# KimmiShi/TorchDistPackage

Measured on AMD Instinct MI355X. Metric: tokens_per_second, higher is better.
Workload: dtype bf16; 1 GPU; model=gpt2_1.3b, global_batch=16, seq_len=1024, parallelism=dp1_pp1_tp1

## Files before the change

torchdistpackage_amd/ops/__init__.py:

```python

from __future__ import annotations

import contextlib
import math
import os
from typing import Optional

import torch

_EXT = None
_EXT_ERR: Optional[str] = None


def _load_extension():
    global _EXT, _EXT_ERR
    if _EXT is not None or _EXT_ERR is not None:
        return _EXT
    import glob
    import importlib.util
    here = os.path.dirname(os.path.abspath(__file__))
    cands = glob.glob(os.path.join(here, "_tdpa_hip*.so"))
    if not cands:
        _EXT_ERR = (f"in-tree HIP extension not found under {here}; "
                    "run `python -m torchdistpackage_amd.ops.build` "
                    "(or __graft_entry__.build())")
        return None
    spec = importlib.util.spec_from_file_location("_tdpa_hip", cands[0])
    mod = importlib.util.module_from_spec(spec)
    try:
        spec.loader.exec_module(mod)
    except Exception as e:
        _EXT_ERR = f"failed to load {cands[0]}: {e}"
        return None
    _EXT = mod
    return _EXT


def ext(required_for: str = "op"):
    m = _load_extension()
    if m is None:
        raise RuntimeError(
            f"HIP extension required for {required_for} on GPU but "
            f"unavailable: {_EXT_ERR}")
    return m


def extension_available() -> bool:
    return _load_extension() is not None



class _RMSNormFn(torch.autograd.Function):
    @staticmethod
    def forward(ctx, x, weight, eps):
        if x.is_cuda:
            y, rstd = ext("rms_norm").rmsnorm_fwd(x.contiguous(), weight, eps)
        else:
            xf = x.float()
            rstd = torch.rsqrt(xf.pow(2).mean(-1, keepdim=True) + eps)
            y = (xf * rstd * weight.float()).to(x.dtype)
            rstd = rstd.squeeze(-1)
        ctx.save_for_backward(x, weight, rstd)
        ctx.eps = eps
        return y

    @staticmethod
    def backward(ctx, dy):
        x, weight, rstd = ctx.saved_tensors
        if x.is_cuda:
            dx, dw = ext("rms_norm").rmsnorm_bwd(
                dy.contiguous(), x.contiguous(), weight, rstd)
        else:
            xf, dyf, wf = x.float(), dy.float(), weight.float()
            r = rstd.unsqueeze(-1)
            xhat = xf * r
            wdy = dyf * wf
            m = (wdy * xhat).mean(-1, keepdim=True)
            dx = (r * (wdy - xhat * m)).to(x.dtype)
            dw = (dyf * xhat).reshape(-1, x.shape[-1]).sum(0).to(weight.dtype)
        return dx, dw, None


def rms_norm(x: torch.Tensor, weight: torch.Tensor, eps: float = 1e-6):
    return _RMSNormFn.apply(x, weight, eps)


class RMSNorm(torch.nn.Module):
    def __init__(self, dim: int, eps: float = 1e-6, device=None, dtype=None):
        super().__init__()
        self.eps = eps
        self.weight = torch.nn.Parameter(
            torch.ones(dim, device=device, dtype=dtype))

    def forward(self, x):
        return rms_norm(x, self.weight, self.eps)



class _LayerNormFn(torch.autograd.Function):
    @staticmethod
    def forward(ctx, x, weight, bias, eps):
        if x.is_cuda:
            y, mean, rstd = ext("layer_norm").layernorm_fwd(
                x.contiguous(), weight, bias, eps)
        else:
            xf = x.float()
            mean = xf.mean(-1, keepdim=True)
            var = xf.var(-1, unbiased=False, keepdim=True)
            off = ~(mean * mean <= var)
            if off.any():
                mean2 = mean + (xf - mean).mean(-1, keepdim=True)
                var2 = (xf - mean2).pow(2).mean(-1, keepdim=True)
                mean = torch.where(off, mean2, mean)
                var = torch.where(off, var2, var)
            rstd = torch.rsqrt(var + eps)
            y = ((xf - mean) * rstd * weight.float() + bias.float()).to(x.dtype)
            mean, rstd = mean.squeeze(-1), rstd.squeeze(-1)
        ctx.save_for_backward(x, weight, mean, rstd)
        return y

    @staticmethod
    def backward(ctx, dy):
        x, weight, mean, rstd = ctx.saved_tensors
        if x.is_cuda:
            dx, dw, db = ext("layer_norm").layernorm_bwd(
                dy.contiguous(), x.contiguous(), weight, mean, rstd)
        else:
            xf, dyf, wf = x.float(), dy.float(), weight.float()
            mu, r = mean.unsqueeze(-1), rstd.unsqueeze(-1)
            xhat = (xf - mu) * r
            wdy = dyf * wf
            m1 = wdy.mean(-1, keepdim=True)
            m2 = (wdy * xhat).mean(-1, keepdim=True)
            dx = (r * (wdy - m1 - xhat * m2)).to(x.dtype)
            dw = (dyf * xhat).reshape(-1, x.shape[-1]).sum(0).to(weight.dtype)
            db = dyf.reshape(-1, x.shape[-1]).sum(0).to(weight.dtype)
        return dx, dw, db, None


def layer_norm(x, weight, bias, eps: float = 1e-5):
    return _LayerNormFn.apply(x, weight, bias, eps)


class LayerNorm(torch.nn.Module):
    def __init__(self, dim: int, eps: float = 1e-5, device=None, dtype=None):
        super().__init__()
        self.eps = eps
        kw = {"device": device, "dtype": dtype}
        self.weight = torch.nn.Parameter(torch.ones(dim, **kw))
        self.bias = torch.nn.Parameter(torch.zeros(dim, **kw))

    def forward(self, x):
        return layer_norm(x, self.weight, self.bias, self.eps)



_GELU_C = math.sqrt(2.0 / math.pi)


def _gelu_tanh(u):
    return 0.5 * u * (1.0 + torch.tanh(_GELU_C * (u + 0.044715 * u.pow(3))))


class _BiasGeluFn(torch.autograd.Function):
    @staticmethod
    def forward(ctx, x, bias):
        ctx.has_bias = bias is not None
        if x.is_cuda:
            y = ext("bias_gelu").bias_gelu_fwd(
                x.contiguous(),
                bias if bias is not None else torch.empty(
                    0, dtype=x.dtype, device=x.device))
            ctx.save_for_backward(x, bias if bias is not None else
                                  torch.empty(0, dtype=x.dtype, device=x.device))
        else:
            u = x.float() + (bias.float() if bias is not None else 0.0)
            y = _gelu_tanh(u).to(x.dtype)
            ctx.save_for_backward(x, bias if bias is not None else
                                  torch.empty(0, dtype=x.dtype))
        return y

    @staticmethod
    def backward(ctx, dy):
        x, bias = ctx.saved_tensors
        if x.is_cuda:
            dx = ext("bias_gelu").bias_gelu_bwd(dy.contiguous(),
                                                x.contiguous(), bias)
        else:
            u = x.float() + (bias.float() if ctx.has_bias else 0.0)
            t = torch.tanh(_GELU_C * (u + 0.044715 * u.pow(3)))
            du = 0.5 * (1 + t) + 0.5 * u * (1 - t * t) * _GELU_C * \
                (1 + 3 * 0.044715 * u.pow(2))
            dx = (dy.float() * du).to(x.dtype)
        dbias = None
        if ctx.has_bias:
            dbias = dx.reshape(-1, x.shape[-1]).sum(0).to(x.dtype)
        return dx, dbias


def bias_gelu(x, bias=None):
    return _BiasGeluFn.apply(x, bias)



class _FlashAttentionFn(torch.autograd.Function):

    @staticmethod
    def forward(ctx, q, k, v, causal, scale):
        if scale is None:
            scale = 1.0 / math.sqrt(q.shape[-1])
        rep = q.shape[1] // k.shape[1]
        if q.is_cuda:
            o = torch.empty(q.shape, dtype=q.dtype, device=q.device)
            o, lse = ext("flash_attention").attn_fwd(
                q, k, v, o, bool(causal), float(scale))
        else:
            kf = k.float() if rep == 1 else \
                k.float().repeat_interleave(rep, 1)
            vf = v.float() if rep == 1 else \
                v.float().repeat_interleave(rep, 1)
            qf = q.float()
            s = torch.matmul(qf, kf.transpose(-1, -2)) * scale
            if causal:
                S = q.shape[-2]
                mask = torch.ones(S, k.shape[-2], dtype=torch.bool,
                                  device=q.device).tril_()
                s = s.masked_fill(~mask, float("-inf"))
            lse = torch.logsumexp(s, dim=-1)
            p = torch.softmax(s, dim=-1)
            o = torch.matmul(p, vf).to(q.dtype)
        ctx.save_for_backward(q, k, v, o, lse)
        ctx.causal = causal
        ctx.scale = scale
        return o

    @staticmethod
    def backward(ctx, do):
        q, k, v, o, lse = ctx.saved_tensors
        H, Hkv = q.shape[1], k.shape[1]
        rep = H // Hkv
        if q.is_cuda:
            dq = torch.empty(q.shape, dtype=q.dtype, device=q.device)
            dk = torch.empty(q.shape, dtype=k.dtype, device=k.device)
            dv = torch.empty(q.shape, dtype=v.dtype, device=v.device)
            dq, dk, dv = ext("flash_attention").attn_bwd(
                do.contiguous(), q, k, v, o, lse, dq, dk, dv,
                ctx.causal, ctx.scale)
            if rep > 1:
                B, _, S, D = q.shape
                dk = dk.view(B, Hkv, rep, S, D).sum(2).to(k.dtype)
                dv = dv.view(B, Hkv, rep, S, D).sum(2).to(v.dtype)
        else:
            qf = q.float()
            kf = k.float() if rep == 1 else \
                k.float().repeat_interleave(rep, 1)
            vf = v.float() if rep == 1 else \
                v.float().repeat_interleave(rep, 1)
            dof = do.float()
            s = torch.matmul(qf, kf.transpose(-1, -2)) * ctx.scale
            if ctx.causal:
                S = q.shape[-2]
                mask = torch.ones(S, k.shape[-2], dtype=torch.bool,
                                  device=q.device).tril_()
                s = s.masked_fill(~mask, float("-inf"))
            p = torch.softmax(s, dim=-1)
            dv = torch.matmul(p.transpose(-1, -2), dof)
            dp = torch.matmul(dof, vf.transpose(-1, -2))
            d = (dp * p).sum(-1, keepdim=True)
            ds = p * (dp - d) * ctx.scale
            dq = torch.matmul(ds, kf)
            dk = torch.matmul(ds.transpose(-1, -2), qf)
            if rep > 1:
                B, _, S, D = q.shape
                dk = dk.view(B, Hkv, rep, S, D).sum(2)
                dv = dv.view(B, Hkv, rep, S, D).sum(2)
            dq, dk, dv = dq.to(q.dtype), dk.to(k.dtype), dv.to(v.dtype)
        return dq, dk, dv, None, None


_ATTN_KNOBS = ("dq_recompute", "no_tr16", "pstore", "force_v1",
               "max_ds_bytes")


def attention_knobs() -> dict:
    return dict(zip(_ATTN_KNOBS, ext("attention_knobs").attn_knobs()))


@contextlib.contextmanager
def attention_route(**knobs):
    unknown = set(knobs) - set(_ATTN_KNOBS)
    if unknown:
        raise TypeError(f"unknown attention knob(s) {sorted(unknown)}; "
                        f"known: {_ATTN_KNOBS}")
    e = ext("attention_knobs")
    cur = attention_knobs()
    cur.update(knobs)
    prev = e.attn_set_knobs(*(cur[n] for n in _ATTN_KNOBS))
    try:
        yield
    finally:
        e.attn_set_knobs(*prev)


_warned_hd = set()


def flash_attention(q, k, v, causal: bool = True, scale: float = None):
    D = q.shape[-1]
    if q.is_cuda and D not in (64, 128):
        if D not in _warned_hd:
            _warned_hd.add(D)
            print(f"[tdpa.ops] flash_attention: head_dim {D} has no HIP "
                  f"kernel (64/128 do); using composite SDPA for it")
        rep = q.shape[1] // k.shape[1]
        kk = k if rep == 1 else k.repeat_interleave(rep, 1)
        vv = v if rep == 1 else v.repeat_interleave(rep, 1)
        if scale is None:
            scale = 1.0 / math.sqrt(D)
        return torch.nn.functional.scaled_dot_product_attention(
            q, kk, vv, is_causal=causal, scale=scale)
    return _FlashAttentionFn.apply(q, k, v, causal, scale)



def fused_adamw_(param: torch.Tensor, grad: torch.Tensor,
                 exp_avg: torch.Tensor, exp_avg_sq: torch.Tensor,
                 step: int, lr: float, beta1: float, beta2: float,
                 eps: float, weight_decay: float):
    if param.is_cuda:
        ext("fused_adamw").adamw_step(param, grad, exp_avg, exp_avg_sq,
                                      step, lr, beta1, beta2, eps,
                                      weight_decay)
        return
    bc1 = 1 - beta1 ** step
    bc2 = 1 - beta2 ** step
    param.mul_(1 - lr * weight_decay)
    exp_avg.mul_(beta1).add_(grad, alpha=1 - beta1)
    exp_avg_sq.mul_(beta2).addcmul_(grad, grad, value=1 - beta2)
    denom = (exp_avg_sq / bc2).sqrt_().add_(eps)
    param.addcdiv_(exp_avg, denom, value=-lr / bc1)


def ema_update_(ema: torch.Tensor, param: torch.Tensor, decay: float):
    if ema.is_cuda:
        ext("ema_update").ema_update(ema, param.contiguous(), decay)
        return
    ema.lerp_(param.to(ema.dtype), 1.0 - decay)


def l2norm_sq(t: torch.Tensor) -> torch.Tensor:
    if t.is_cuda:
        return ext("l2norm").l2norm_sq(t)
    return t.float().pow(2).sum()


def scale_(t: torch.Tensor, scale: float):
    if t.is_cuda:
        ext("scale").scale_inplace(t, scale)
        return
    t.mul_(scale)


class _FusedQKVAttentionFn(torch.autograd.Function):

    @staticmethod
    def forward(ctx, qkv, n_head, causal, scale):
        S, B, three_d = qkv.shape
        d_local = three_d // 3
        hd = d_local // n_head
        if scale is None:
            scale = 1.0 / math.sqrt(hd)

        def view4(t, off):
            return t.narrow(-1, off, d_local) \
                .view(S, B, n_head, hd).permute(1, 2, 0, 3)

        q, k, v = view4(qkv, 0), view4(qkv, d_local), view4(qkv, 2 * d_local)
        if qkv.is_cuda:
            o_buf = torch.empty(S, B, d_local, dtype=qkv.dtype,
                                device=qkv.device)
            o4 = o_buf.view(S, B, n_head, hd).permute(1, 2, 0, 3)
            _, lse = ext("flash_attention").attn_fwd(
                q, k, v, o4, bool(causal), float(scale))
        else:
            qf = q.contiguous().float()
            kf = k.contiguous().float()
            vf = v.contiguous().float()
            sc = torch.matmul(qf, kf.transpose(-1, -2)) * scale
            if causal:
                mask = torch.ones(S, S, dtype=torch.bool).tril_()
                sc = sc.masked_fill(~mask, float("-inf"))
            lse = torch.logsumexp(sc, dim=-1)
            o4 = torch.matmul(torch.softmax(sc, -1), vf).to(qkv.dtype)
            o_buf = o4.permute(2, 0, 1, 3).reshape(S, B, d_local)
        ctx.save_for_backward(qkv, o_buf, lse)
        ctx.meta = (n_head, causal, scale)
        return o_buf

    @staticmethod
    def backward(ctx, do):
        qkv, o_buf, lse = ctx.saved_tensors
        n_head, causal, scale = ctx.meta
        S, B, three_d = qkv.shape
        d_local = three_d // 3
        hd = d_local // n_head

        def view4(t, off, width):
            return t.narrow(-1, off, width) \
                .view(S, B, n_head, hd).permute(1, 2, 0, 3)

        q = view4(qkv, 0, d_local)
        k = view4(qkv, d_local, d_local)
        v = view4(qkv, 2 * d_local, d_local)
        o4 = o_buf.view(S, B, n_head, hd).permute(1, 2, 0, 3)
        do = do.contiguous()
        do4 = do.view(S, B, n_head, hd).permute(1, 2, 0, 3)
        if qkv.is_cuda:
            dqkv = torch.empty_like(qkv)
            dq = view4(dqkv, 0, d_local)
            dk = view4(dqkv, d_local, d_local)
            dv = view4(dqkv, 2 * d_local, d_local)
            ext("flash_attention").attn_bwd(
                do4, q, k, v, o4, lse, dq, dk, dv, causal, scale)
        else:
            qc, kc, vc = q.contiguous(), k.contiguous(), v.contiguous()
            with torch.enable_grad():
                qf = qc.float().requires_grad_(True)
                kf = kc.float().requires_grad_(True)
                vf = vc.float().requires_grad_(True)
                s = torch.matmul(qf, kf.transpose(-1, -2)) * scale
                if causal:
                    Sq = q.shape[-2]
                    mask = torch.ones(Sq, Sq, dtype=torch.bool).tril_()
                    s = s.masked_fill(~mask, float("-inf"))
                ref = torch.matmul(torch.softmax(s, -1), vf)
                ref.backward(do4.float())
            dqkv = torch.cat([
                g.to(qkv.dtype).permute(2, 0, 1, 3).reshape(S, B, d_local)
                for g in (qf.grad, kf.grad, vf.grad)], dim=-1)
        return dqkv, None, None, None



def fused_qkv_attention(qkv, n_head: int, causal: bool = True,
                        scale: float = None):
    return _FusedQKVAttentionFn.apply(qkv, n_head, causal, scale)


class _GqaAttentionFn(torch.autograd.Function):

    @staticmethod
    def forward(ctx, q, k, v, causal, scale):
        B, H, S, D = q.shape
        o_buf = torch.empty(S, B, H * D, dtype=q.dtype, device=q.device)
        o4 = o_buf.view(S, B, H, D).permute(1, 2, 0, 3)
        _, lse = ext("flash_attention").attn_fwd(
            q, k, v, o4, bool(causal), float(scale))
        ctx.save_for_backward(q, k, v, o_buf, lse)
        ctx.meta = (causal, scale)
        return o_buf

    @staticmethod
    def backward(ctx, do):
        q, k, v, o_buf, lse = ctx.saved_tensors
        causal, scale = ctx.meta
        B, H, S, D = q.shape
        Hkv = k.shape[1]
        rep = H // Hkv
        o4 = o_buf.view(S, B, H, D).permute(1, 2, 0, 3)
        do = do.contiguous()
        do4 = do.view(S, B, H, D).permute(1, 2, 0, 3)
        dq_buf = torch.empty(S, B, H * D, dtype=q.dtype, device=q.device)
        dq = dq_buf.view(S, B, H, D).permute(1, 2, 0, 3)
        dk = torch.empty(B, H, S, D, dtype=k.dtype, device=k.device)
        dv = torch.empty(B, H, S, D, dtype=v.dtype, device=v.device)
        ext("flash_attention").attn_bwd(do4, q, k, v, o4, lse, dq, dk, dv,
                                        causal, scale)
        if rep > 1:
            dk = dk.view(B, Hkv, rep, S, D).sum(2)
            dv = dv.view(B, Hkv, rep, S, D).sum(2)
        return dq, dk, dv, None, None


def gqa_attention(q, k, v, causal: bool = True, scale: float = None):
    if scale is None:
        scale = 1.0 / math.sqrt(q.shape[-1])
    if q.is_cuda and q.dtype == torch.bfloat16 and q.shape[-1] in (64, 128):
        return _GqaAttentionFn.apply(q, k, v, causal, scale)
    o = flash_attention(q, k, v, causal=causal, scale=scale)
    B, H, S, D = q.shape
    return o.permute(2, 0, 1, 3).reshape(S, B, H * D)



_DECODE_MAX_ROWS = 16


def resolve_decode_attn_impl(attn_impl: Optional[str] = None) -> str:
    if attn_impl is None:
        attn_impl = "hip" if os.environ.get("TDPA_DECODE_ATTN", "0") == "1" \
            else "sdpa"
    if attn_impl not in ("sdpa", "hip"):
        raise ValueError(f"attn_impl must be 'sdpa' or 'hip', got "
                         f"{attn_impl!r}")
    return attn_impl


def _decode_attention_ref(q, k_cache, v_cache, pos0, scale):
    B, Hq, Sq, D = q.shape
    Hkv, Smax = k_cache.shape[1], k_cache.shape[2]
    G = Hq // Hkv
    if torch.is_tensor(pos0):
        pos = pos0.reshape(-1).to(device=q.device, dtype=torch.long)
        pos = pos.expand(B) if pos.numel() == 1 else pos
    else:
        if pos0 < 0 or pos0 + Sq > Smax:
            raise ValueError(f"decode_attention: pos0={pos0} with Sq={Sq} "
                             f"outside the cache (Smax={Smax})")
        pos = torch.full((B,), int(pos0), dtype=torch.long, device=q.device)
    pos = pos.clamp(0, Smax - Sq)
    L = int(pos.max()) + Sq
    kf = k_cache[:, :, :L].float()
    vf = v_cache[:, :, :L].float()
    j = torch.arange(L, device=q.device)
    live = j[None, :] < (pos[:, None] + Sq)
    vf = torch.where(live[:, None, :, None], vf, torch.zeros_like(vf))
    qf = q.float().reshape(B, Hkv, G * Sq, D)
    s = torch.matmul(qf, kf.transpose(-1, -2)) * scale
    row = torch.arange(G * Sq, device=q.device) % Sq
    vis = j[None, None, :] <= (pos[:, None, None] + row[None, :, None])
    s = s.masked_fill(~vis[:, None], float("-inf"))
    o = torch.matmul(torch.softmax(s, dim=-1), vf)
    return o.reshape(B, Hq, Sq, D).to(q.dtype)


def decode_attention(q: torch.Tensor, k_cache: torch.Tensor,
                     v_cache: torch.Tensor, pos0, scale: float = None,
                     split_kv: Optional[int] = None) -> torch.Tensor:
    B, Hq, Sq, D = q.shape
    Hkv = k_cache.shape[1]
    if Hq % Hkv != 0:
        raise ValueError(f"decode_attention: Hq={Hq} not a multiple of "
                         f"Hkv={Hkv}")
    if scale is None:
        scale = 1.0 / math.sqrt(D)
    if not q.is_cuda:
        o = _decode_attention_ref(q, k_cache, v_cache, pos0, scale)
        o_buf = o.permute(2, 0, 1, 3).contiguous()
        return o_buf.permute(1, 2, 0, 3)
    if q.dtype != torch.bfloat16:
        raise TypeError("decode_attention: the GPU kernel is bf16-only, got "
                        f"{q.dtype}")
    if D not in (64, 128):
        raise ValueError("decode_attention: the GPU kernel covers head dim "
                         f"64 and 128, got {D}")
    G = Hq // Hkv
    if G > _DECODE_MAX_ROWS:
        raise ValueError(f"decode_attention: Hq/Hkv={G} exceeds the "
                         f"kernel's {_DECODE_MAX_ROWS} rows per kv head")
    e = ext("decode_attention")
    o_buf = torch.empty(Sq, B, Hq * D, dtype=q.dtype, device=q.device)
    o4 = o_buf.view(Sq, B, Hq, D).permute(1, 2, 0, 3)
    skv = int(split_kv or 0)
    if torch.is_tensor(pos0):
        if G * Sq > _DECODE_MAX_ROWS:
            raise ValueError(
                f"decode_attention: (Hq/Hkv)*Sq={G * Sq} exceeds "
                f"{_DECODE_MAX_ROWS} rows per kv head; with a tensor pos0 "
                "the call cannot be split on the host — pass an int pos0 "
                "or fewer query rows")
        e.decode_attention(q, k_cache, v_cache, o4, pos0, 0, float(scale),
                           skv)
        return o4
    pos0 = int(pos0)
    rows = _DECODE_MAX_ROWS // G
    for r0 in range(0, Sq, rows):
        r1 = min(r0 + rows, Sq)
        e.decode_attention(q[:, :, r0:r1], k_cache, v_cache,
                           o4[:, :, r0:r1], None, pos0 + r0, float(scale),
                           skv)
    return o4


class _CrossEntropyFn(torch.autograd.Function):

    @staticmethod
    def forward(ctx, logits2d, targets):
        loss_vec, lse = ext("cross_entropy").ce_fwd(logits2d, targets)
        ctx.save_for_backward(logits2d, targets, lse)
        return loss_vec.mean()

    @staticmethod
    def backward(ctx, g):
        logits2d, targets, lse = ctx.saved_tensors
        dlogits = ext("cross_entropy").ce_bwd(
            logits2d, targets, lse, g.reshape(1).float().contiguous())
        return dlogits, None


def cross_entropy_loss(logits: torch.Tensor, targets: torch.Tensor):
    l2 = logits.reshape(-1, logits.size(-1))
    t = targets.reshape(-1)
    if l2.is_cuda and l2.dtype == torch.bfloat16:
        return _CrossEntropyFn.apply(l2.contiguous(), t)
    import torch.nn.functional as F
    return F.cross_entropy(l2.float(), t)



class _BatchedBiasGeluFn(torch.autograd.Function):

    @staticmethod
    def forward(ctx, x, bias):
        ctx.save_for_backward(x, bias)
        if x.is_cuda and x.dtype == torch.bfloat16:
            return ext("bgelu_b").bgelu_b_fwd(x.contiguous(),
                                              bias.contiguous())
        u = x.float() + bias.float().unsqueeze(1)
        return _gelu_tanh(u).to(x.dtype)

    @staticmethod
    def backward(ctx, dy):
        x, bias = ctx.saved_tensors
        if x.is_cuda and x.dtype == torch.bfloat16:
            dx = ext("bgelu_b").bgelu_b_bwd(dy.contiguous(), x.contiguous(),
                                            bias.contiguous())
        else:
            u = x.float() + bias.float().unsqueeze(1)
            t = torch.tanh(_GELU_C * (u + 0.044715 * u.pow(3)))
            du = 0.5 * (1 + t) + 0.5 * u * (1 - t * t) * _GELU_C * \
                (1 + 3 * 0.044715 * u.pow(2))
            dx = (dy.float() * du).to(x.dtype)
        dbias = dx.float().sum(1).to(bias.dtype)
        return dx, dbias


def batched_bias_gelu(x, bias):
    return _BatchedBiasGeluFn.apply(x, bias)


def _rope_rows(cos, sin, pos0, S):
    if cos.shape != sin.shape:
        raise ValueError("rope: sin must have the shape of cos")
    if pos0 < 0 or pos0 + S > cos.shape[0]:
        raise ValueError(f"rope: pos0={pos0} with S={S} outside the cos/sin "
                         f"table ({cos.shape[0]} rows)")
    return cos[pos0:pos0 + S].float(), sin[pos0:pos0 + S].float()


class _RopeFn(torch.autograd.Function):

    @staticmethod
    def forward(ctx, x, cos, sin, pos0):
        ctx.save_for_backward(cos, sin)
        ctx.pos0 = pos0
        if x.is_cuda and x.dtype == torch.bfloat16:
            return ext("rope").rope_apply(x, cos, sin, pos0, True)
        c, s = _rope_rows(cos, sin, pos0, x.shape[-2])
        hd = x.shape[-1]
        xf = x.float()
        x1, x2 = xf[..., :hd // 2], xf[..., hd // 2:]
        return torch.cat([x1 * c - x2 * s, x2 * c + x1 * s],
                         dim=-1).to(x.dtype)

    @staticmethod
    def backward(ctx, dy):
        cos, sin = ctx.saved_tensors
        if dy.is_cuda and dy.dtype == torch.bfloat16:
            if dy.stride(-1) != 1:
                dy = dy.contiguous()
            return (ext("rope").rope_apply(dy, cos, sin,
                                           ctx.pos0, False),
                    None, None, None)
        c, s = _rope_rows(cos, sin, ctx.pos0, dy.shape[-2])
        hd = dy.shape[-1]
        df = dy.float()
        d1, d2 = df[..., :hd // 2], df[..., hd // 2:]
        return (torch.cat([d1 * c + d2 * s, d2 * c - d1 * s],
                          dim=-1).to(dy.dtype),
                None, None, None)


def rope_rotate_half(x: torch.Tensor, cos: torch.Tensor, sin: torch.Tensor,
                     pos0=0) -> torch.Tensor:
    if torch.is_tensor(pos0):
        assert not torch.is_grad_enabled(), \
            "tensor pos0 is the no-grad decode path"
        if x.is_cuda and x.dtype == torch.bfloat16:
            return ext("rope").rope_apply_pos(x, cos, sin, pos0, True)
        return _RopeFn.apply(x, cos, sin, int(pos0.item()))
    return _RopeFn.apply(x, cos, sin, pos0)


class _SwiGluFn(torch.autograd.Function):
    @staticmethod
    def forward(ctx, a, b):
        ctx.save_for_backward(a, b)
        if a.is_cuda and a.dtype == torch.bfloat16:
            return ext("swiglu").swiglu_fwd(a.contiguous(), b.contiguous())
        af = a.float()
        return (af * torch.sigmoid(af) * b.float()).to(a.dtype)

    @staticmethod
    def backward(ctx, dy):
        a, b = ctx.saved_tensors
        if a.is_cuda and a.dtype == torch.bfloat16:
            da, db = ext("swiglu").swiglu_bwd(dy.contiguous(),
                                              a.contiguous(), b.contiguous())
            return da, db
        af, bf, dyf = a.float(), b.float(), dy.float()
        sig = torch.sigmoid(af)
        silu = af * sig
        da = dyf * bf * (sig + silu * (1 - sig))
        db = dyf * silu
        return da.to(a.dtype), db.to(b.dtype)


def swiglu(a: torch.Tensor, b: torch.Tensor) -> torch.Tensor:
    return _SwiGluFn.apply(a, b)



from .grouped import (GROUPED_GEMM_BM, grouped_gemm_eligible,
                      grouped_linear)
```

torchdistpackage_amd/ops/csrc/attention.hip:

```cpp

#include <torch/extension.h>
#include <ATen/hip/HIPContext.h>
#include "common.h"
#include "attn_knobs.h"
#include <cstdlib>
#include <string>
#include <tuple>

namespace {

typedef __attribute__((ext_vector_type(8))) __bf16 bf16x8_v;
typedef __attribute__((ext_vector_type(4))) float f32x4;

constexpr int WQ = 16;
constexpr int KT = 32;
constexpr int NW_FWD = 16;
constexpr int NW_DQ = 8;
constexpr int NW_DKDV = 8;

struct Strides {
  long b, h, s;
};

DEVINL bf16x8_v pack8(const unsigned short* p) {
  return *(const bf16x8_v*)p;
}

template <int D>
DEVINL int swzD(int row, int col) {
  return row * D + (col ^ ((row & (D / 8 - 1)) << 3));
}

DEVINL int swz32(int row, int col) {
  return row * KT + (col ^ (((row >> 2) & 3) << 3));
}


template <int D, bool CAUSAL, int NW>
__launch_bounds__(NW * 64)
__global__ void attn_fwd_kernel(const unsigned short* __restrict__ q,
                                const unsigned short* __restrict__ k,
                                const unsigned short* __restrict__ v,
                                unsigned short* __restrict__ o,
                                float* __restrict__ lse,
                                Strides qs, Strides ks, Strides vs, Strides os,
                                int B, int H, int S, float scale,
                                int q_per_kv) {
  constexpr int KC = D / 32;
  constexpr int DC = D / 16;
  __shared__ __attribute__((aligned(16))) unsigned short k_lds[KT * D];
  __shared__ __attribute__((aligned(16))) unsigned short vt_lds[D * KT];
  __shared__ __attribute__((aligned(16))) unsigned short p_lds[NW * 16 * KT];

  constexpr int QT = NW * WQ;
  const int bh = blockIdx.y;
  const int bb = bh / H, hh = bh % H;
  const int qbase = blockIdx.x * QT;
  if (qbase >= S) return;
  const int tid = threadIdx.x;
  const int wid = tid / WAVE;
  const int lane = tid % WAVE;
  const int l15 = lane & 15;
  const int lg = lane >> 4;

  const int hkv = hh / q_per_kv;
  const unsigned short* qp = q + bb * qs.b + hh * qs.h;
  const unsigned short* kp = k + bb * ks.b + hkv * ks.h;
  const unsigned short* vp = v + bb * vs.b + hkv * vs.h;

  const int qrow0 = qbase + wid * WQ;
  bf16x8_v a_q[KC];
  {
    int r = qrow0 + l15;
    long rr = (r < S ? r : S - 1) * qs.s;
#pragma unroll
    for (int c = 0; c < KC; ++c)
      a_q[c] = pack8(qp + rr + c * 32 + lg * 8);
  }

  float m_run[4], l_run[4];
#pragma unroll
  for (int i = 0; i < 4; ++i) { m_run[i] = -1e30f; l_run[i] = 0.f; }
  f32x4 acc_o[DC];
#pragma unroll
  for (int d = 0; d < DC; ++d) acc_o[d] = (f32x4)(0.f);

  const int kv_end = CAUSAL ? min(S, qbase + QT) : S;

  const int st_idx = tid * 8;
  const int st_key = st_idx / D;
  const int st_col = st_idx % D;
  const bool st_own = st_idx < KT * D;
  bf16x8_v k_reg, v_reg;

  auto stage_load = [&](int kt0) {
    if (!st_own) return;
    int gkey = kt0 + st_key;
    if (gkey < S) {
      k_reg = pack8(kp + (long)gkey * ks.s + st_col);
      v_reg = pack8(vp + (long)gkey * vs.s + st_col);
    } else {
      k_reg = (bf16x8_v)(__bf16)0.f;
      v_reg = (bf16x8_v)(__bf16)0.f;
    }
  };

  stage_load(0);

  for (int kt0 = 0; kt0 < kv_end; kt0 += KT) {
    __syncthreads();
    if (st_own) {
      *(bf16x8_v*)&k_lds[swzD<D>(st_key, st_col)] = k_reg;
      const unsigned short* vsrc = (const unsigned short*)&v_reg;
#pragma unroll
      for (int j = 0; j < 8; ++j)
        vt_lds[swz32(st_col + j, st_key)] = vsrc[j];
    }
    __syncthreads();
    if (kt0 + KT < kv_end) stage_load(kt0 + KT);

    f32x4 s_acc[KT / 16];
#pragma unroll
    for (int kg = 0; kg < KT / 16; ++kg) {
      s_acc[kg] = (f32x4)(0.f);
#pragma unroll
      for (int c = 0; c < KC; ++c) {
        bf16x8_v b_k = pack8(&k_lds[swzD<D>(kg * 16 + l15, c * 32 + lg * 8)]);
        s_acc[kg] = __builtin_amdgcn_mfma_f32_16x16x32_bf16(
            a_q[c], b_k, s_acc[kg], 0, 0, 0);
      }
    }

    float p_val[KT / 16][4];
    float alpha[4];
    {
      float tile_max[4];
#pragma unroll
      for (int rr = 0; rr < 4; ++rr) tile_max[rr] = -1e30f;
#pragma unroll
      for (int kg = 0; kg < KT / 16; ++kg) {
#pragma unroll
        for (int rr = 0; rr < 4; ++rr) {
          int qrow = qrow0 + lg * 4 + rr;
          int key = kt0 + kg * 16 + l15;
          float sv = s_acc[kg][rr] * scale;
          bool valid = key < S && (!CAUSAL || key <= qrow);
          sv = valid ? sv : -1e30f;
          s_acc[kg][rr] = sv;
          tile_max[rr] = fmaxf(tile_max[rr], sv);
        }
      }
#pragma unroll
      for (int rr = 0; rr < 4; ++rr) {
        tile_max[rr] = group16_max(tile_max[rr]);
        float m_new = fmaxf(m_run[rr], tile_max[rr]);
        alpha[rr] = __expf(m_run[rr] - m_new);
        m_run[rr] = m_new;
        float psum = 0.f;
#pragma unroll
        for (int kg = 0; kg < KT / 16; ++kg) {
          float pv = __expf(s_acc[kg][rr] - m_new);
          p_val[kg][rr] = pv;
          psum += pv;
        }
        psum = group16_sum(psum);
        l_run[rr] = l_run[rr] * alpha[rr] + psum;
      }
    }

#pragma unroll
    for (int d = 0; d < DC; ++d)
#pragma unroll
      for (int rr = 0; rr < 4; ++rr) acc_o[d][rr] *= alpha[rr];

    unsigned short* pw = &p_lds[wid * 16 * KT];
#pragma unroll
    for (int kg = 0; kg < KT / 16; ++kg)
#pragma unroll
      for (int rr = 0; rr < 4; ++rr)
        pw[swz32(lg * 4 + rr, kg * 16 + l15)] = f2bf(p_val[kg][rr]);

    bf16x8_v a_p = pack8(&pw[swz32(l15, lg * 8)]);
#pragma unroll
    for (int d = 0; d < DC; ++d) {
      bf16x8_v b_v = pack8(&vt_lds[swz32(d * 16 + l15, lg * 8)]);
      acc_o[d] = __builtin_amdgcn_mfma_f32_16x16x32_bf16(
          a_p, b_v, acc_o[d], 0, 0, 0);
    }
  }

  unsigned short* op = o + bb * os.b + hh * os.h;
  float* lsep = lse + ((long)bh) * S;
#pragma unroll
  for (int rr = 0; rr < 4; ++rr) {
    int qrow = qrow0 + lg * 4 + rr;
    if (qrow >= S) continue;
    float inv_l = l_run[rr] > 0.f ? 1.f / l_run[rr] : 0.f;
#pragma unroll
    for (int d = 0; d < DC; ++d)
      op[(long)qrow * os.s + d * 16 + l15] = f2bf(acc_o[d][rr] * inv_l);
    if (l15 == 0)
      lsep[qrow] = m_run[rr] + __logf(l_run[rr] > 0.f ? l_run[rr] : 1.f);
  }
}


__global__ void attn_delta_kernel(const unsigned short* __restrict__ o,
                                  const unsigned short* __restrict__ dout,
                                  float* __restrict__ delta,
                                  Strides os, Strides ds,
                                  int B, int H, int S, int D) {
  const long rows = (long)B * H * S;
  const int wpb = blockDim.x / WAVE;
  const int lane = threadIdx.x % WAVE;
  const long stride = (long)gridDim.x * wpb;
  for (long row = (long)blockIdx.x * wpb + threadIdx.x / WAVE; row < rows;
       row += stride) {
    int s = row % S;
    int h = (row / S) % H;
    int b = row / ((long)S * H);
    const unsigned short* orow = o + b * os.b + h * os.h + (long)s * os.s;
    const unsigned short* drow = dout + b * ds.b + h * ds.h + (long)s * ds.s;
    float acc = 0.f;
    for (int i = lane * 8; i < D; i += WAVE * 8) {
      bf16x8_v ov = pack8(orow + i);
      bf16x8_v dv = pack8(drow + i);
      const unsigned short* op = (const unsigned short*)&ov;
      const unsigned short* dp = (const unsigned short*)&dv;
#pragma unroll
      for (int j = 0; j < 8; ++j) acc += bf2f(op[j]) * bf2f(dp[j]);
    }
    acc = wave_sum(acc);
    if (lane == 0) delta[row] = acc;
  }
}

template <int D, bool CAUSAL, int NW>
__launch_bounds__(NW * 64)
__global__ void attn_bwd_dq_kernel(const unsigned short* __restrict__ q,
                                   const unsigned short* __restrict__ k,
                                   const unsigned short* __restrict__ v,
                                   const unsigned short* __restrict__ dout,
                                   const float* __restrict__ lse,
                                   const float* __restrict__ delta,
                                   unsigned short* __restrict__ dq,
                                   Strides qs, Strides ks, Strides vs,
                                   Strides dos, Strides dqs,
                                   int B, int H, int S, float scale,
                                   int q_per_kv) {
  constexpr int KC = D / 32;
  constexpr int DC = D / 16;
  __shared__ __attribute__((aligned(16))) unsigned short k_lds[KT * D];
  __shared__ __attribute__((aligned(16))) unsigned short kt_lds[D * KT];
  __shared__ __attribute__((aligned(16))) unsigned short v_lds[KT * D];
  __shared__ __attribute__((aligned(16))) unsigned short ds_lds[NW * 16 * KT];

  constexpr int QT = NW * WQ;
  const int bh = blockIdx.y;
  const int bb = bh / H, hh = bh % H;
  const int qbase = blockIdx.x * QT;
  if (qbase >= S) return;
  const int tid = threadIdx.x;
  const int wid = tid / WAVE;
  const int lane = tid % WAVE;
  const int l15 = lane & 15;
  const int lg = lane >> 4;

  const int hkv = hh / q_per_kv;
  const unsigned short* qp = q + bb * qs.b + hh * qs.h;
  const unsigned short* kp = k + bb * ks.b + hkv * ks.h;
  const unsigned short* vp = v + bb * vs.b + hkv * vs.h;
  const unsigned short* dop = dout + bb * dos.b + hh * dos.h;
  const float* lsep = lse + (long)bh * S;
  const float* delp = delta + (long)bh * S;

  const int qrow0 = qbase + wid * WQ;
  bf16x8_v a_q[KC], a_do[KC];
  float my_lse[4], my_delta[4];
  {
    int r = qrow0 + l15;
    int rc = r < S ? r : S - 1;
#pragma unroll
    for (int c = 0; c < KC; ++c) {
      a_q[c] = pack8(qp + (long)rc * qs.s + c * 32 + lg * 8);
      a_do[c] = pack8(dop + (long)rc * dos.s + c * 32 + lg * 8);
    }
#pragma unroll
    for (int rr4 = 0; rr4 < 4; ++rr4) {
      int row = qrow0 + lg * 4 + rr4;
      my_lse[rr4] = row < S ? lsep[row] : 0.f;
      my_delta[rr4] = row < S ? delp[row] : 0.f;
    }
  }

  f32x4 acc_dq[DC];
#pragma unroll
  for (int d = 0; d < DC; ++d) acc_dq[d] = (f32x4)(0.f);

  const int kv_end = CAUSAL ? min(S, qbase + QT) : S;

  const int st_idx = tid * 8;
  const int st_key = st_idx / D;
  const int st_col = st_idx % D;
  const bool st_own = st_idx < KT * D;
  bf16x8_v k_reg, v_reg;

  auto stage_load = [&](int kt0) {
    if (!st_own) return;
    int gkey = kt0 + st_key;
    if (gkey < S) {
      k_reg = pack8(kp + (long)gkey * ks.s + st_col);
      v_reg = pack8(vp + (long)gkey * vs.s + st_col);
    } else {
      k_reg = (bf16x8_v)(__bf16)0.f;
      v_reg = (bf16x8_v)(__bf16)0.f;
    }
  };

  stage_load(0);

  for (int kt0 = 0; kt0 < kv_end; kt0 += KT) {
    __syncthreads();
    if (st_own) {
      *(bf16x8_v*)&k_lds[swzD<D>(st_key, st_col)] = k_reg;
      *(bf16x8_v*)&v_lds[swzD<D>(st_key, st_col)] = v_reg;
      const unsigned short* ksrc = (const unsigned short*)&k_reg;
#pragma unroll
      for (int j = 0; j < 8; ++j)
        kt_lds[swz32(st_col + j, st_key)] = ksrc[j];
    }
    __syncthreads();
    if (kt0 + KT < kv_end) stage_load(kt0 + KT);

    f32x4 s_acc[KT / 16], dp_acc[KT / 16];
#pragma unroll
    for (int kg = 0; kg < KT / 16; ++kg) {
      s_acc[kg] = (f32x4)(0.f);
      dp_acc[kg] = (f32x4)(0.f);
#pragma unroll
      for (int c = 0; c < KC; ++c) {
        bf16x8_v b_k = pack8(&k_lds[swzD<D>(kg * 16 + l15, c * 32 + lg * 8)]);
        s_acc[kg] = __builtin_amdgcn_mfma_f32_16x16x32_bf16(
            a_q[c], b_k, s_acc[kg], 0, 0, 0);
        bf16x8_v b_v = pack8(&v_lds[swzD<D>(kg * 16 + l15, c * 32 + lg * 8)]);
        dp_acc[kg] = __builtin_amdgcn_mfma_f32_16x16x32_bf16(
            a_do[c], b_v, dp_acc[kg], 0, 0, 0);
      }
    }

    unsigned short* dsw = &ds_lds[wid * 16 * KT];
#pragma unroll
    for (int kg = 0; kg < KT / 16; ++kg) {
#pragma unroll
      for (int rr = 0; rr < 4; ++rr) {
        int qrow = qrow0 + lg * 4 + rr;
        int key = kt0 + kg * 16 + l15;
        bool valid = key < S && qrow < S && (!CAUSAL || key <= qrow);
        float p = valid ?
            __expf(s_acc[kg][rr] * scale - my_lse[rr]) : 0.f;
        float ds = p * (dp_acc[kg][rr] - my_delta[rr]) * scale;
        dsw[swz32(lg * 4 + rr, kg * 16 + l15)] = f2bf(ds);
      }
    }

    bf16x8_v a_ds = pack8(&dsw[swz32(l15, lg * 8)]);
#pragma unroll
    for (int d = 0; d < DC; ++d) {
      bf16x8_v b_kt = pack8(&kt_lds[swz32(d * 16 + l15, lg * 8)]);
      acc_dq[d] = __builtin_amdgcn_mfma_f32_16x16x32_bf16(
          a_ds, b_kt, acc_dq[d], 0, 0, 0);
    }
  }

  unsigned short* dqp = dq + bb * dqs.b + hh * dqs.h;
#pragma unroll
  for (int rr = 0; rr < 4; ++rr) {
    int qrow = qrow0 + lg * 4 + rr;
    if (qrow >= S) continue;
#pragma unroll
    for (int d = 0; d < DC; ++d)
      dqp[(long)qrow * dqs.s + d * 16 + l15] = f2bf(acc_dq[d][rr]);
  }
}

template <int D, bool CAUSAL, int NW>
__launch_bounds__(NW * 64)
__global__ void attn_bwd_dkdv_kernel(const unsigned short* __restrict__ q,
                                     const unsigned short* __restrict__ k,
                                     const unsigned short* __restrict__ v,
                                     const unsigned short* __restrict__ dout,
                                     const float* __restrict__ lse,
                                     const float* __restrict__ delta,
                                     unsigned short* __restrict__ dk,
                                     unsigned short* __restrict__ dv,
                                     Strides qs, Strides ks, Strides vs,
                                     Strides dos, Strides dks, Strides dvs,
                                     int B, int H, int S, float scale,
                                     int q_per_kv) {
  constexpr int KC = D / 32;
  constexpr int DC = D / 16;
  __shared__ __attribute__((aligned(16))) unsigned short q_lds[KT * D];
  __shared__ __attribute__((aligned(16))) unsigned short qt_lds[D * KT];
  __shared__ __attribute__((aligned(16))) unsigned short do_lds[KT * D];
  __shared__ __attribute__((aligned(16))) unsigned short dot_lds[D * KT];
  __shared__ __attribute__((aligned(16))) unsigned short st_lds[NW * 16 * KT];
  __shared__ __attribute__((aligned(16))) float lse_lds[KT];
  __shared__ __attribute__((aligned(16))) float del_lds[KT];

  constexpr int QT = NW * WQ;
  const int bh = blockIdx.y;
  const int bb = bh / H, hh = bh % H;
  const int kbase = blockIdx.x * QT;
  if (kbase >= S) return;
  const int tid = threadIdx.x;
  const int wid = tid / WAVE;
  const int lane = tid % WAVE;
  const int l15 = lane & 15;
  const int lg = lane >> 4;

  const int hkv = hh / q_per_kv;
  const unsigned short* qp = q + bb * qs.b + hh * qs.h;
  const unsigned short* kp = k + bb * ks.b + hkv * ks.h;
  const unsigned short* vp = v + bb * vs.b + hkv * vs.h;
  const unsigned short* dop = dout + bb * dos.b + hh * dos.h;
  const float* lsep = lse + (long)bh * S;
  const float* delp = delta + (long)bh * S;

  const int key0 = kbase + wid * WQ;
  bf16x8_v a_k[KC], a_v[KC];
  {
    int r = key0 + l15;
    long rc = (long)(r < S ? r : S - 1);
#pragma unroll
    for (int c = 0; c < KC; ++c) {
      a_k[c] = pack8(kp + rc * ks.s + c * 32 + lg * 8);
      a_v[c] = pack8(vp + rc * vs.s + c * 32 + lg * 8);
    }
  }

  f32x4 acc_dk[DC], acc_dv[DC];
#pragma unroll
  for (int d = 0; d < DC; ++d) {
    acc_dk[d] = (f32x4)(0.f);
    acc_dv[d] = (f32x4)(0.f);
  }

  const int qt_start = CAUSAL ? kbase : 0;

  const int st_idx = tid * 8;
  const int st_row = st_idx / D;
  const int st_col = st_idx % D;
  const bool st_own = st_idx < KT * D;
  bf16x8_v q_reg, do_reg;
  float lse_reg = 0.f, del_reg = 0.f;

  auto stage_load = [&](int qt0) {
    if (st_own) {
      int grow = qt0 + st_row;
      if (grow < S) {
        q_reg = pack8(qp + (long)grow * qs.s + st_col);
        do_reg = pack8(dop + (long)grow * dos.s + st_col);
      } else {
        q_reg = (bf16x8_v)(__bf16)0.f;
        do_reg = (bf16x8_v)(__bf16)0.f;
      }
    }
    if (tid < KT) {
      int grow = qt0 + tid;
      lse_reg = grow < S ? lsep[grow] : 0.f;
      del_reg = grow < S ? delp[grow] : 0.f;
    }
  };

  stage_load(qt_start);

  for (int qt0 = qt_start; qt0 < S; qt0 += KT) {
    __syncthreads();
    if (st_own) {
      *(bf16x8_v*)&q_lds[swzD<D>(st_row, st_col)] = q_reg;
      *(bf16x8_v*)&do_lds[swzD<D>(st_row, st_col)] = do_reg;
      const unsigned short* qsrc = (const unsigned short*)&q_reg;
      const unsigned short* dsrc = (const unsigned short*)&do_reg;
#pragma unroll
      for (int j = 0; j < 8; ++j) {
        qt_lds[swz32(st_col + j, st_row)] = qsrc[j];
        dot_lds[swz32(st_col + j, st_row)] = dsrc[j];
      }
    }
    if (tid < KT) {
      lse_lds[tid] = lse_reg;
      del_lds[tid] = del_reg;
    }
    __syncthreads();
    if (qt0 + KT < S) stage_load(qt0 + KT);

    f32x4 st_acc[KT / 16], dpt_acc[KT / 16];
#pragma unroll
    for (int qg = 0; qg < KT / 16; ++qg) {
      st_acc[qg] = (f32x4)(0.f);
      dpt_acc[qg] = (f32x4)(0.f);
#pragma unroll
      for (int c = 0; c < KC; ++c) {
        bf16x8_v b_q = pack8(&q_lds[swzD<D>(qg * 16 + l15, c * 32 + lg * 8)]);
        st_acc[qg] = __builtin_amdgcn_mfma_f32_16x16x32_bf16(
            a_k[c], b_q, st_acc[qg], 0, 0, 0);
        bf16x8_v b_do = pack8(&do_lds[swzD<D>(qg * 16 + l15, c * 32 + lg * 8)]);
        dpt_acc[qg] = __builtin_amdgcn_mfma_f32_16x16x32_bf16(
            a_v[c], b_do, dpt_acc[qg], 0, 0, 0);
      }
    }

    unsigned short* stw = &st_lds[wid * 16 * KT];
#pragma unroll
    for (int qg = 0; qg < KT / 16; ++qg) {
#pragma unroll
      for (int rr = 0; rr < 4; ++rr) {
        int key = key0 + lg * 4 + rr;
        int qrow = qt0 + qg * 16 + l15;
        bool valid = key < S && qrow < S && (!CAUSAL || key <= qrow);
        float p = valid ?
            __expf(st_acc[qg][rr] * scale - lse_lds[qg * 16 + l15]) : 0.f;
        st_acc[qg][rr] = p;
        stw[swz32(lg * 4 + rr, qg * 16 + l15)] =
            f2bf(p < kAttnPFlush ? 0.f : p);
      }
    }

    bf16x8_v a_pt = pack8(&stw[swz32(l15, lg * 8)]);
#pragma unroll
    for (int d = 0; d < DC; ++d) {
      bf16x8_v b_dot = pack8(&dot_lds[swz32(d * 16 + l15, lg * 8)]);
      acc_dv[d] = __builtin_amdgcn_mfma_f32_16x16x32_bf16(
          a_pt, b_dot, acc_dv[d], 0, 0, 0);
    }

#pragma unroll
    for (int qg = 0; qg < KT / 16; ++qg) {
#pragma unroll
      for (int rr = 0; rr < 4; ++rr) {
        float ds = st_acc[qg][rr] *
            (dpt_acc[qg][rr] - del_lds[qg * 16 + l15]) * scale;
        stw[swz32(lg * 4 + rr, qg * 16 + l15)] = f2bf(ds);
      }
    }

    bf16x8_v a_dst = pack8(&stw[swz32(l15, lg * 8)]);
#pragma unroll
    for (int d = 0; d < DC; ++d) {
      bf16x8_v b_qt = pack8(&qt_lds[swz32(d * 16 + l15, lg * 8)]);
      acc_dk[d] = __builtin_amdgcn_mfma_f32_16x16x32_bf16(
          a_dst, b_qt, acc_dk[d], 0, 0, 0);
    }
  }

  unsigned short* dkp = dk + bb * dks.b + hh * dks.h;
  unsigned short* dvp = dv + bb * dvs.b + hh * dvs.h;
#pragma unroll
  for (int rr = 0; rr < 4; ++rr) {
    int key = key0 + lg * 4 + rr;
    if (key >= S) continue;
#pragma unroll
    for (int d = 0; d < DC; ++d) {
      dkp[(long)key * dks.s + d * 16 + l15] = f2bf(acc_dk[d][rr]);
      dvp[(long)key * dvs.s + d * 16 + l15] = f2bf(acc_dv[d][rr]);
    }
  }
}

Strides get_strides(const torch::Tensor& t) {
  TORCH_CHECK(t.dim() == 4 && t.stride(3) == 1,
              "attention tensors must be 4D (B,H,S,D) with contiguous D");
  return Strides{t.stride(0), t.stride(1), t.stride(2)};
}

void check_operand(const char* fn, const char* name, const torch::Tensor& t,
                   const torch::Tensor& q, int64_t B, int64_t Hh, int64_t S,
                   int64_t D) {
  TORCH_CHECK(t.is_cuda() && t.device() == q.device(), fn, ": ", name,
              " must be on q's device ", q.device(), ", got ", t.device());
  TORCH_CHECK(t.scalar_type() == torch::kBFloat16, fn, ": ", name,
              " must be bf16, got ", t.scalar_type());
  TORCH_CHECK(t.dim() == 4 && t.size(0) == B && t.size(1) == Hh &&
                  t.size(2) == S && t.size(3) == D,
              fn, ": ", name, " must be (", B, ", ", Hh, ", ", S, ", ", D,
              "), got ", t.sizes());
  TORCH_CHECK(t.stride(3) == 1, fn, ": ", name,
              " must have a contiguous last dim, got stride ", t.stride(3));
  for (int d = 0; d < 3; ++d)
    TORCH_CHECK(t.size(d) == 1 || t.stride(d) % 8 == 0, fn, ": ", name,
                " stride ", t.stride(d), " of dim ", d, " is not a multiple "
                "of 8 elements: the kernels use 16-byte vector accesses");
  TORCH_CHECK(reinterpret_cast<uintptr_t>(t.data_ptr()) % 16 == 0, fn, ": ",
              name, " is not 16-byte aligned: the kernels use 16-byte vector "
              "accesses");
}

std::tuple<int64_t, int64_t, int64_t, int64_t, int64_t> check_qkv(
    const char* fn, const torch::Tensor& q, const torch::Tensor& k,
    const torch::Tensor& v) {
  TORCH_CHECK(q.is_cuda() && q.scalar_type() == torch::kBFloat16, fn,
              ": bf16 CUDA tensors required");
  TORCH_CHECK(q.dim() == 4, fn, ": q must be (B, H, S, D), got ", q.sizes());
  const int64_t B = q.size(0), H = q.size(1), S = q.size(2), D = q.size(3);
  TORCH_CHECK(D == 64 || D == 128, fn, ": head_dim must be 64 or 128, got ",
              D);
  TORCH_CHECK(B >= 1 && H >= 1 && S >= 1, fn,
              ": empty problem (S = 0?), q is ", q.sizes());
  TORCH_CHECK(k.dim() == 4 && v.dim() == 4, fn,
              ": k and v must be (B, Hkv, S, D), got ", k.sizes(), " and ",
              v.sizes());
  const int64_t Hkv = k.size(1);
  TORCH_CHECK(Hkv >= 1 && H % Hkv == 0, fn,
              ": n_head must be a multiple of n_kv_head, got ", H, " and ",
              Hkv);
  TORCH_CHECK(k.size(2) == S, fn,
              ": cross-attention S_kv != S_q not supported yet (k has ",
              k.size(2), " keys, q ", S, " rows)");
  check_operand(fn, "q", q, q, B, H, S, D);
  check_operand(fn, "k", k, q, B, Hkv, S, D);
  check_operand(fn, "v", v, q, B, Hkv, S, D);
  return {B, H, Hkv, S, D};
}

}

AttnKnobs& attn_knobs_ref() {
  static AttnKnobs k{
      std::getenv("TDPA_DQ_RECOMPUTE") != nullptr,
      std::getenv("TDPA_NO_TR16") != nullptr,
      std::getenv("TDPA_PSTORE") != nullptr,
      std::getenv("TDPA_ATTN_V1") != nullptr,
      (int64_t)4 << 30};
  return k;
}

using KnobTuple = std::tuple<bool, bool, bool, bool, int64_t>;

KnobTuple attn_knobs() {
  const AttnKnobs& k = attn_knobs_ref();
  return {k.dq_recompute, k.no_tr16, k.pstore, k.force_v1, k.max_ds_bytes};
}

KnobTuple attn_set_knobs(bool dq_recompute, bool no_tr16, bool pstore,
                         bool force_v1, int64_t max_ds_bytes) {
  KnobTuple prev = attn_knobs();
  attn_knobs_ref() =
      AttnKnobs{dq_recompute, no_tr16, pstore, force_v1, max_ds_bytes};
  return prev;
}

std::string attn_bwd_route(int64_t B, int64_t H, int64_t S, int64_t D) {
  const AttnBwdRoute r = attn_bwd_select(attn_knobs_ref(), B, H, S, D);
  if (r.v1) return "v1";
  if (r.recompute) return "v2_recompute";
  std::string name = "v2_workspace";
  if (r.pstore) name += "+pstore";
  if (r.no_tr16) name += "+no_tr16";
  return name;
}

void attn_fwd_v2(torch::Tensor q, torch::Tensor k, torch::Tensor v,
                 torch::Tensor o, torch::Tensor lse, bool causal,
                 double scale);
void attn_bwd_dq_v2(torch::Tensor dout, torch::Tensor q, torch::Tensor k,
                    torch::Tensor v, torch::Tensor lse, torch::Tensor delta,
                    torch::Tensor dq, bool causal, double scale);
void attn_bwd_v2_all(torch::Tensor dout, torch::Tensor q, torch::Tensor k,
                     torch::Tensor v, torch::Tensor lse, torch::Tensor delta,
                     torch::Tensor dq, torch::Tensor dk, torch::Tensor dv,
                     bool causal, double scale, const AttnBwdRoute& route);
void attn_bwd_dkdv_v2(torch::Tensor dout, torch::Tensor q, torch::Tensor k,
                      torch::Tensor v, torch::Tensor lse, torch::Tensor delta,
                      torch::Tensor dk, torch::Tensor dv, bool causal,
                      double scale);

std::vector<torch::Tensor> attn_fwd(torch::Tensor q, torch::Tensor k,
                                    torch::Tensor v, torch::Tensor o,
                                    bool causal, double scale) {
  auto [B_, H_, Hkv_, S_, D_] = check_qkv("attn_fwd", q, k, v);
  check_operand("attn_fwd", "o", o, q, B_, H_, S_, D_);
  const int B = B_, H = H_, S = S_, D = D_, Hkv = Hkv_;
  const int q_per_kv = H / Hkv;
  auto lse = torch::empty({B, H, S}, q.options().dtype(torch::kFloat));
  const bool force_v1 = attn_knobs_ref().force_v1;
  if (D == 128 && !force_v1) {
    attn_fwd_v2(q, k, v, o, lse, causal, scale);
    return {o, lse};
  }
  auto stream = at::cuda::getCurrentHIPStream();
  constexpr int QT = NW_FWD * WQ;
  dim3 grid((S + QT - 1) / QT, B * H), block(NW_FWD * 64);
  Strides qs = get_strides(q), ks = get_strides(k), vs = get_strides(v),
          os = get_strides(o);
  const unsigned short* qp = (const unsigned short*)q.data_ptr();
  const unsigned short* kp = (const unsigned short*)k.data_ptr();
  const unsigned short* vp = (const unsigned short*)v.data_ptr();
  unsigned short* op = (unsigned short*)o.data_ptr();
  float* lp = lse.data_ptr<float>();
#define LAUNCH(DD, CC)                                                        \
  hipLaunchKernelGGL((attn_fwd_kernel<DD, CC, NW_FWD>), grid, block, 0,       \
                     stream, qp, kp, vp, op, lp, qs, ks, vs, os, B, H, S,     \
                     (float)scale, q_per_kv)
  if (D == 128) { if (causal) LAUNCH(128, true); else LAUNCH(128, false); }
  else          { if (causal) LAUNCH(64, true);  else LAUNCH(64, false);  }
#undef LAUNCH
  HIP_CHECK_LAST();
  return {o, lse};
}

std::vector<torch::Tensor> attn_bwd(torch::Tensor dout, torch::Tensor q,
                                    torch::Tensor k, torch::Tensor v,
                                    torch::Tensor o, torch::Tensor lse,
                                    torch::Tensor dq, torch::Tensor dk,
                                    torch::Tensor dv,
                                    bool causal, double scale) {
  auto [B_, H_, Hkv_, S_, D_] = check_qkv("attn_bwd", q, k, v);
  const int B = B_, H = H_, S = S_, D = D_, Hkv = Hkv_;
  const int q_per_kv = H / Hkv;
  check_operand("attn_bwd", "dout", dout, q, B, H, S, D);
  check_operand("attn_bwd", "o", o, q, B, H, S, D);
  check_operand("attn_bwd", "dq", dq, q, B, H, S, D);
  TORCH_CHECK(dk.dim() == 4 && dv.dim() == 4 && dk.size(1) == H &&
                  dv.size(1) == H,
              "attn_bwd: dk/dv must be expanded to H q-heads for GQA, got ",
              dk.sizes(), " and ", dv.sizes(), " for H = ", H);
  check_operand("attn_bwd", "dk", dk, q, B, H, S, D);
  check_operand("attn_bwd", "dv", dv, q, B, H, S, D);
  TORCH_CHECK(lse.is_cuda() && lse.device() == q.device() &&
                  lse.scalar_type() == torch::kFloat && lse.dim() == 3 &&
                  lse.size(0) == B && lse.size(1) == H && lse.size(2) == S &&
                  lse.is_contiguous(),
              "attn_bwd: lse must be a contiguous fp32 (", B, ", ", H, ", ",
              S, ") tensor on q's device, got ", lse.scalar_type(), " ",
              lse.sizes(), " strides ", lse.strides(), " on ", lse.device());
  auto delta = torch::empty({B, H, S}, q.options().dtype(torch::kFloat));
  auto stream = at::cuda::getCurrentHIPStream();
  Strides qs = get_strides(q), ks = get_strides(k), vs = get_strides(v),
          os = get_strides(o), dos = get_strides(dout),
          dqs = get_strides(dq), dks = get_strides(dk), dvs = get_strides(dv);

  {
    long rows = (long)B * H * S;
    long blocks = (rows + 3) / 4;
    if (blocks > 2048) blocks = 2048;
    hipLaunchKernelGGL(attn_delta_kernel, dim3((unsigned)blocks), dim3(256),
                       0, stream, (const unsigned short*)o.data_ptr(),
                       (const unsigned short*)dout.data_ptr(),
                       delta.data_ptr<float>(), os, dos, B, H, S, D);
  }

  const AttnBwdRoute route = attn_bwd_select(attn_knobs_ref(), B, H, S, D);
  if (!route.v1) {
    attn_bwd_v2_all(dout, q, k, v, lse, delta, dq, dk, dv, causal, scale,
                    route);
    HIP_CHECK_LAST();
    return {dq, dk, dv};
  }
  constexpr int QT_DQ = NW_DQ * WQ;
  constexpr int QT_KV = NW_DKDV * WQ;
  dim3 grid_dq((S + QT_DQ - 1) / QT_DQ, B * H), block_dq(NW_DQ * 64);
  dim3 grid_kv((S + QT_KV - 1) / QT_KV, B * H), block_kv(NW_DKDV * 64);
  const unsigned short* qp = (const unsigned short*)q.data_ptr();
  const unsigned short* kp = (const unsigned short*)k.data_ptr();
  const unsigned short* vp = (const unsigned short*)v.data_ptr();
  const unsigned short* dop = (const unsigned short*)dout.data_ptr();
  const float* lp = lse.data_ptr<float>();
  const float* delp = delta.data_ptr<float>();
#define LAUNCH_BWD(DD, CC)                                                    \
  do {                                                                        \
    hipLaunchKernelGGL((attn_bwd_dq_kernel<DD, CC, NW_DQ>), grid_dq,         \
                       block_dq, 0, stream, qp, kp, vp, dop, lp, delp,        \
                       (unsigned short*)dq.data_ptr(), qs, ks, vs, dos, dqs,  \
                       B, H, S, (float)scale, q_per_kv);                      \
    hipLaunchKernelGGL((attn_bwd_dkdv_kernel<DD, CC, NW_DKDV>), grid_kv,      \
                       block_kv, 0, stream, qp, kp, vp, dop, lp, delp,        \
                       (unsigned short*)dk.data_ptr(),                        \
                       (unsigned short*)dv.data_ptr(), qs, ks, vs, dos,       \
                       dks, dvs, B, H, S, (float)scale, q_per_kv);            \
  } while (0)
  if (D == 128) { if (causal) LAUNCH_BWD(128, true); else LAUNCH_BWD(128, false); }
  else          { if (causal) LAUNCH_BWD(64, true);  else LAUNCH_BWD(64, false);  }
#undef LAUNCH_BWD
  HIP_CHECK_LAST();
  return {dq, dk, dv};
}
```

torchdistpackage_amd/ops/csrc/bindings.cpp:

```cpp
#include <torch/extension.h>

#include "grouped_gemm_plan.h"

std::vector<torch::Tensor> rmsnorm_fwd(torch::Tensor x, torch::Tensor w,
                                       double eps);
std::vector<torch::Tensor> rmsnorm_bwd(torch::Tensor dy, torch::Tensor x,
                                       torch::Tensor w, torch::Tensor rstd);
std::vector<torch::Tensor> layernorm_fwd(torch::Tensor x, torch::Tensor w,
                                         torch::Tensor b, double eps);
std::vector<torch::Tensor> layernorm_bwd(torch::Tensor dy, torch::Tensor x,
                                         torch::Tensor w, torch::Tensor mean,
                                         torch::Tensor rstd);
torch::Tensor bias_gelu_fwd(torch::Tensor x, torch::Tensor bias);
torch::Tensor bias_gelu_bwd(torch::Tensor dy, torch::Tensor x,
                            torch::Tensor bias);
void adamw_step(torch::Tensor p, torch::Tensor g, torch::Tensor m,
                torch::Tensor v, long step, double lr, double beta1,
                double beta2, double eps, double wd);
void multi_adamw_step(torch::Tensor cpid, torch::Tensor coff,
                      torch::Tensor pptrs, torch::Tensor gptrs,
                      torch::Tensor mptrs, torch::Tensor moffs,
                      torch::Tensor numels,
                      torch::Tensor m, torch::Tensor v,
                      long step, double lr, double beta1, double beta2,
                      double eps, double wd, bool param_bf16, bool grad_bf16);
void adamw_step_dev(torch::Tensor p, torch::Tensor g, torch::Tensor m,
                    torch::Tensor v, torch::Tensor coef, double beta1,
                    double beta2, double eps);
void adamw_prelude(torch::Tensor step, torch::Tensor hyp, torch::Tensor coef);
void multi_adamw_step_dev(torch::Tensor cpid, torch::Tensor coff,
                          torch::Tensor pptrs, torch::Tensor gptrs,
                          torch::Tensor mptrs, torch::Tensor moffs,
                          torch::Tensor numels,
                          torch::Tensor m, torch::Tensor v,
                          torch::Tensor coef, double beta1, double beta2,
                          double eps, bool param_bf16, bool grad_bf16);
void ema_update(torch::Tensor ema, torch::Tensor p, double decay);
torch::Tensor l2norm_sq(torch::Tensor x);
void scale_inplace(torch::Tensor x, double s);
std::vector<torch::Tensor> attn_fwd(torch::Tensor q, torch::Tensor k,
                                    torch::Tensor v, torch::Tensor o,
                                    bool causal, double scale);
std::vector<torch::Tensor> attn_bwd(torch::Tensor dout, torch::Tensor q,
                                    torch::Tensor k, torch::Tensor v,
                                    torch::Tensor o, torch::Tensor lse,
                                    torch::Tensor dq, torch::Tensor dk,
                                    torch::Tensor dv,
                                    bool causal, double scale);
std::tuple<bool, bool, bool, bool, int64_t> attn_knobs();
std::tuple<bool, bool, bool, bool, int64_t> attn_set_knobs(
    bool dq_recompute, bool no_tr16, bool pstore, bool force_v1,
    int64_t max_ds_bytes);
std::string attn_bwd_route(int64_t B, int64_t H, int64_t S, int64_t D);
torch::Tensor mfma_probe_16x16x32(torch::Tensor a, torch::Tensor b);
torch::Tensor mfma_probe_32x32x16(torch::Tensor a, torch::Tensor b);
torch::Tensor tr16_probe(long addr_mode);
std::vector<torch::Tensor> ce_fwd(torch::Tensor logits, torch::Tensor targets);
torch::Tensor gemm_fprop(torch::Tensor x, torch::Tensor w,
                         c10::optional<torch::Tensor> bias);
torch::Tensor rope_apply(torch::Tensor x, torch::Tensor cs, torch::Tensor sn,
                         long pos0, bool fwd);
torch::Tensor swiglu_fwd(torch::Tensor a, torch::Tensor b);
torch::Tensor bgelu_b_fwd(torch::Tensor x, torch::Tensor bias);
torch::Tensor bgelu_b_bwd(torch::Tensor dy, torch::Tensor x,
                          torch::Tensor bias);
std::vector<torch::Tensor> swiglu_bwd(torch::Tensor dy, torch::Tensor a,
                                      torch::Tensor b);
torch::Tensor gemm_dgrad(torch::Tensor dy, torch::Tensor w, bool kswz);
torch::Tensor gemm_wgrad(torch::Tensor dy, torch::Tensor x, long splitk,
                         bool kswz);
torch::Tensor ce_bwd(torch::Tensor logits, torch::Tensor targets,
                     torch::Tensor lse, torch::Tensor grad_out);
std::vector<torch::Tensor> ce_partial_fwd(torch::Tensor logits,
                                          torch::Tensor targets);
torch::Tensor gemv_bf16(torch::Tensor x, torch::Tensor W,
                        c10::optional<torch::Tensor> bias);
torch::Tensor rope_apply_pos(torch::Tensor x, torch::Tensor cs,
                             torch::Tensor sn, torch::Tensor pos, bool fwd);
torch::Tensor decode_attention(torch::Tensor q, torch::Tensor k_cache,
                               torch::Tensor v_cache, torch::Tensor out,
                               c10::optional<torch::Tensor> pos_t, long pos0,
                               double scale, long split_kv);
torch::Tensor grouped_gemm_fprop(torch::Tensor x, torch::Tensor w,
                                 torch::Tensor offs,
                                 c10::optional<torch::Tensor> bias);
torch::Tensor grouped_gemm_dgrad(torch::Tensor dy, torch::Tensor w,
                                 torch::Tensor offs);
std::tuple<torch::Tensor, c10::optional<torch::Tensor>> grouped_gemm_wgrad(
    torch::Tensor dy, torch::Tensor x, torch::Tensor offs,
    bool want_bias_grad);
torch::Tensor grouped_gemm_plan(torch::Tensor offs_cpu, int64_t T);

PYBIND11_MODULE(TORCH_EXTENSION_NAME, m) {
  m.def("rmsnorm_fwd", &rmsnorm_fwd);
  m.def("rmsnorm_bwd", &rmsnorm_bwd);
  m.def("layernorm_fwd", &layernorm_fwd);
  m.def("layernorm_bwd", &layernorm_bwd);
  m.def("bias_gelu_fwd", &bias_gelu_fwd);
  m.def("bias_gelu_bwd", &bias_gelu_bwd);
  m.def("adamw_step", &adamw_step);
  m.def("multi_adamw_step", &multi_adamw_step);
  m.def("adamw_step_dev", &adamw_step_dev);
  m.def("adamw_prelude", &adamw_prelude);
  m.def("multi_adamw_step_dev", &multi_adamw_step_dev);
  m.def("ema_update", &ema_update);
  m.def("l2norm_sq", &l2norm_sq);
  m.def("scale_inplace", &scale_inplace);
  m.def("attn_fwd", &attn_fwd);
  m.def("attn_bwd", &attn_bwd);
  m.def("attn_knobs", &attn_knobs,
        "(dq_recompute, no_tr16, pstore, force_v1, max_ds_bytes)");
  m.def("attn_set_knobs", &attn_set_knobs,
        "set the five attention knobs; returns the previous five");
  m.def("attn_bwd_route", &attn_bwd_route,
        "name of the backward route for (B, H, S, D) under the current knobs");
  m.def("mfma_probe_16x16x32", &mfma_probe_16x16x32);
  m.def("mfma_probe_32x32x16", &mfma_probe_32x32x16);
  m.def("tr16_probe", &tr16_probe);
  m.def("ce_fwd", &ce_fwd);
  m.def("gemm_fprop", &gemm_fprop);
  m.def("rope_apply", &rope_apply);
  m.def("swiglu_fwd", &swiglu_fwd);
  m.def("bgelu_b_fwd", &bgelu_b_fwd);
  m.def("bgelu_b_bwd", &bgelu_b_bwd);
  m.def("swiglu_bwd", &swiglu_bwd);
  m.def("gemm_dgrad", &gemm_dgrad);
  m.def("gemm_wgrad", &gemm_wgrad);
  m.def("ce_bwd", &ce_bwd);
  m.def("ce_partial_fwd", &ce_partial_fwd);
  m.def("gemv_bf16", &gemv_bf16);
  m.def("rope_apply_pos", &rope_apply_pos);
  m.def("decode_attention", &decode_attention);
  m.def("grouped_gemm_fprop", &grouped_gemm_fprop);
  m.def("grouped_gemm_dgrad", &grouped_gemm_dgrad);
  m.def("grouped_gemm_wgrad", &grouped_gemm_wgrad);
  m.def("grouped_gemm_plan", &grouped_gemm_plan,
        "(offs_cpu, T) -> (row-tile bound, 3) int64: (expert, first row, "
        "row count) per block, expert -1 = idle");
  m.attr("GROUPED_GEMM_BM") = GG_BM;
}
```

torchdistpackage_amd/ops/csrc/elementwise.hip:

```cpp

#include <torch/extension.h>
#include <ATen/hip/HIPContext.h>
#include "common.h"

namespace {

constexpr int BLOCK = 256;
constexpr float GELU_C = 0.7978845608028654f;
constexpr float GELU_A = 0.044715f;

DEVINL float tanh_fast(float x) {
  float e = __builtin_amdgcn_exp2f(x * 2.885390082f);
  return 1.f - 2.f / (e + 1.f);
}

DEVINL float gelu_f(float u) {
  float t = tanh_fast(GELU_C * (u + GELU_A * u * u * u));
  return 0.5f * u * (1.f + t);
}

DEVINL float gelu_df(float u) {
  float u2 = u * u;
  float t = tanh_fast(GELU_C * (u + GELU_A * u * u2));
  return 0.5f * (1.f + t) +
         0.5f * u * (1.f - t * t) * GELU_C * (1.f + 3.f * GELU_A * u2);
}


__global__ void bias_gelu_fwd_bf16(const unsigned short* __restrict__ x,
                                   const unsigned short* __restrict__ bias,
                                   unsigned short* __restrict__ y,
                                   long n, int D, int has_bias) {
  long i0 = ((long)blockIdx.x * BLOCK + threadIdx.x) * 8;
  long stride = (long)gridDim.x * BLOCK * 8;
  for (long i = i0; i < n; i += stride) {
    if (i + 8 <= n) {
      bf16x8 xv = *(const bf16x8*)(x + i);
      bf16x8 bv;
      if (has_bias) bv = *(const bf16x8*)(bias + (int)(i % D));
      const unsigned short* xs = (const unsigned short*)&xv;
      const unsigned short* bs = (const unsigned short*)&bv;
      bf16x8 out;
      unsigned short* os = (unsigned short*)&out;
#pragma unroll
      for (int j = 0; j < 8; ++j) {
        float b = has_bias ? bf2f(bs[j]) : 0.f;
        os[j] = f2bf(gelu_f(bf2f(xs[j]) + b));
      }
      *(bf16x8*)(y + i) = out;
    } else {
      for (long j = i; j < n; ++j) {
        float b = has_bias ? bf2f(bias[j % D]) : 0.f;
        y[j] = f2bf(gelu_f(bf2f(x[j]) + b));
      }
    }
  }
}

__global__ void bias_gelu_bwd_bf16(const unsigned short* __restrict__ dy,
                                   const unsigned short* __restrict__ x,
                                   const unsigned short* __restrict__ bias,
                                   unsigned short* __restrict__ dx,
                                   long n, int D, int has_bias) {
  long i0 = ((long)blockIdx.x * BLOCK + threadIdx.x) * 8;
  long stride = (long)gridDim.x * BLOCK * 8;
  for (long i = i0; i < n; i += stride) {
    if (i + 8 <= n) {
      bf16x8 xv = *(const bf16x8*)(x + i);
      bf16x8 gv = *(const bf16x8*)(dy + i);
      bf16x8 bv;
      if (has_bias) bv = *(const bf16x8*)(bias + (int)(i % D));
      const unsigned short* xs = (const unsigned short*)&xv;
      const unsigned short* gs = (const unsigned short*)&gv;
      const unsigned short* bs = (const unsigned short*)&bv;
      bf16x8 out;
      unsigned short* os = (unsigned short*)&out;
#pragma unroll
      for (int j = 0; j < 8; ++j) {
        float b = has_bias ? bf2f(bs[j]) : 0.f;
        os[j] = f2bf(bf2f(gs[j]) * gelu_df(bf2f(xs[j]) + b));
      }
      *(bf16x8*)(dx + i) = out;
    } else {
      for (long j = i; j < n; ++j) {
        float b = has_bias ? bf2f(bias[j % D]) : 0.f;
        dx[j] = f2bf(bf2f(dy[j]) * gelu_df(bf2f(x[j]) + b));
      }
    }
  }
}

__global__ void bias_gelu_fwd_f32(const float* __restrict__ x,
                                  const float* __restrict__ bias,
                                  float* __restrict__ y,
                                  long n, int D, int has_bias) {
  long i0 = (long)blockIdx.x * BLOCK + threadIdx.x;
  long stride = (long)gridDim.x * BLOCK;
  for (long i = i0; i < n; i += stride) {
    float b = has_bias ? bias[i % D] : 0.f;
    y[i] = gelu_f(x[i] + b);
  }
}

__global__ void bias_gelu_bwd_f32(const float* __restrict__ dy,
                                  const float* __restrict__ x,
                                  const float* __restrict__ bias,
                                  float* __restrict__ dx,
                                  long n, int D, int has_bias) {
  long i0 = (long)blockIdx.x * BLOCK + threadIdx.x;
  long stride = (long)gridDim.x * BLOCK;
  for (long i = i0; i < n; i += stride) {
    float b = has_bias ? bias[i % D] : 0.f;
    dx[i] = dy[i] * gelu_df(x[i] + b);
  }
}


struct AdamCoef {
  float omb1;
  float omb2;
  float bc2;
  float step_size;
  float decay;
};
constexpr int ADAM_NCOEF = 5;
constexpr int ADAM_NHYP = 4;

DEVINL AdamCoef adam_coef_load(AdamCoef c, const float* __restrict__ cdev) {
  if (cdev != nullptr) {
    c.omb1 = cdev[0];
    c.omb2 = cdev[1];
    c.bc2 = cdev[2];
    c.step_size = cdev[3];
    c.decay = cdev[4];
  }
  return c;
}

DEVINL void adam_elem(float& p, float& m, float& v, float g, float beta1,
                      float beta2, float eps, const AdamCoef& c) {
  float mi = m * beta1 + g * c.omb1;
  float vi = v * beta2 + g * g * c.omb2;
  m = mi;
  v = vi;
  p = p * c.decay - c.step_size * mi / (sqrtf(vi / c.bc2) + eps);
}

__global__ void adam_prelude_kernel(long* __restrict__ step,
                                    const double* __restrict__ hyp,
                                    float* __restrict__ coef, int ngroups) {
  const long t = *step + 1;
  __syncthreads();
  for (int g = threadIdx.x; g < ngroups; g += blockDim.x) {
    const double lr = hyp[g * ADAM_NHYP + 0];
    const double b1 = hyp[g * ADAM_NHYP + 1];
    const double b2 = hyp[g * ADAM_NHYP + 2];
    const double wd = hyp[g * ADAM_NHYP + 3];
    const double bc1 = 1.0 - pow(b1, (double)t);
    const double bc2 = 1.0 - pow(b2, (double)t);
    float* c = coef + g * ADAM_NCOEF;
    c[0] = (float)(1.0 - b1);
    c[1] = (float)(1.0 - b2);
    c[2] = (float)bc2;
    c[3] = (float)(lr / bc1);
    c[4] = (float)(1.0 - lr * wd);
  }
  if (threadIdx.x == 0) *step = t;
}

__global__ void adamw_kernel(float* __restrict__ p, const float* __restrict__ g,
                             float* __restrict__ m, float* __restrict__ v,
                             long n, float beta1, float beta2, float eps,
                             AdamCoef ch, const float* __restrict__ cdev) {
  const AdamCoef c = adam_coef_load(ch, cdev);
  long i0 = (long)blockIdx.x * BLOCK + threadIdx.x;
  long stride = (long)gridDim.x * BLOCK;
  for (long i = i0; i < n; i += stride) {
    float pi = p[i], mi = m[i], vi = v[i];
    adam_elem(pi, mi, vi, g[i], beta1, beta2, eps, c);
    m[i] = mi;
    v[i] = vi;
    p[i] = pi;
  }
}


__global__ void ema_kernel(float* __restrict__ ema, const float* __restrict__ p,
                           long n, float decay, float omd, int vec4) {
  const long n4 = vec4 ? (n >> 2) : 0;
  long i0 = (long)blockIdx.x * BLOCK + threadIdx.x;
  long stride = (long)gridDim.x * BLOCK;
  for (long i = i0; i < n4; i += stride) {
    float4 e = *(const float4*)(ema + i * 4);
    float4 v = *(const float4*)(p + i * 4);
    e.x = decay * e.x + omd * v.x;
    e.y = decay * e.y + omd * v.y;
    e.z = decay * e.z + omd * v.z;
    e.w = decay * e.w + omd * v.w;
    *(float4*)(ema + i * 4) = e;
  }
  for (long i = n4 * 4 + i0; i < n; i += stride)
    ema[i] = decay * ema[i] + omd * p[i];
}


template <typename T>
__global__ void l2norm_kernel(const T* __restrict__ x,
                              float* __restrict__ partial, long n) {
  __shared__ float lds[BLOCK / WAVE];
  long i0 = (long)blockIdx.x * BLOCK + threadIdx.x;
  long stride = (long)gridDim.x * BLOCK;
  float acc = 0.f;
  for (long i = i0; i < n; i += stride) {
    float v;
    if constexpr (sizeof(T) == 2) v = bf2f(((const unsigned short*)x)[i]);
    else v = ((const float*)x)[i];
    acc += v * v;
  }
  acc = block_sum<BLOCK>(acc, lds);
  if (threadIdx.x == 0) partial[blockIdx.x] = acc;
}

__global__ void l2norm_final_kernel(const float* __restrict__ partial,
                                    float* __restrict__ out, int nparts) {
  __shared__ float lds[BLOCK / WAVE];
  float acc = 0.f;
  for (int i = threadIdx.x; i < nparts; i += BLOCK) acc += partial[i];
  acc = block_sum<BLOCK>(acc, lds);
  if (threadIdx.x == 0) *out = acc;
}

template <typename T>
__global__ void scale_kernel(T* __restrict__ x, long n, float s) {
  long i0 = (long)blockIdx.x * BLOCK + threadIdx.x;
  long stride = (long)gridDim.x * BLOCK;
  for (long i = i0; i < n; i += stride) {
    if constexpr (sizeof(T) == 2) {
      unsigned short* p = (unsigned short*)x;
      p[i] = f2bf(bf2f(p[i]) * s);
    } else {
      ((float*)x)[i] *= s;
    }
  }
}

int ew_grid(long n, int per_thread = 1) {
  long blocks = (n + (long)BLOCK * per_thread - 1) / ((long)BLOCK * per_thread);
  return (int)(blocks > 2048 ? 2048 : (blocks > 0 ? blocks : 1));
}

AdamCoef adam_coef_host(long step, double lr, double beta1, double beta2,
                        double wd) {
  const double bc1 = 1.0 - std::pow(beta1, (double)step);
  const double bc2 = 1.0 - std::pow(beta2, (double)step);
  AdamCoef c;
  c.omb1 = (float)(1.0 - beta1);
  c.omb2 = (float)(1.0 - beta2);
  c.bc2 = (float)bc2;
  c.step_size = (float)(lr / bc1);
  c.decay = (float)(1.0 - lr * wd);
  return c;
}

void check_adamw_flat(const torch::Tensor& p, const torch::Tensor& g,
                      const torch::Tensor& m, const torch::Tensor& v) {
  const torch::Tensor* ts[4] = {&p, &g, &m, &v};
  const char* names[4] = {"p", "g", "m", "v"};
  for (int i = 0; i < 4; ++i) {
    TORCH_CHECK(ts[i]->is_cuda() && ts[i]->scalar_type() == torch::kFloat,
                "adamw_step: ", names[i], " must be an fp32 device tensor");
    TORCH_CHECK(ts[i]->is_contiguous(), "adamw_step: ", names[i],
                " must be contiguous");
    TORCH_CHECK(ts[i]->numel() == p.numel(), "adamw_step: ", names[i],
                " has ", ts[i]->numel(), " elements, p has ", p.numel());
    TORCH_CHECK(ts[i]->get_device() == p.get_device(), "adamw_step: ",
                names[i], " is on another device than p");
  }
}

void check_adam_coef(const torch::Tensor& coef, const torch::Tensor& like) {
  TORCH_CHECK(coef.is_cuda() && coef.scalar_type() == torch::kFloat &&
              coef.is_contiguous() && coef.numel() == ADAM_NCOEF &&
              coef.get_device() == like.get_device(),
              "adamw: coef must be ", ADAM_NCOEF,
              " contiguous fp32 values on the params' device");
}

}


torch::Tensor bias_gelu_fwd(torch::Tensor x, torch::Tensor bias) {
  TORCH_CHECK(x.is_cuda() && x.is_contiguous());
  auto y = torch::empty_like(x);
  long n = x.numel();
  int D = x.size(-1);
  int has_bias = bias.numel() > 0 ? 1 : 0;
  auto stream = at::cuda::getCurrentHIPStream();
  if (x.scalar_type() == torch::kBFloat16) {
    TORCH_CHECK(!has_bias || (D % 8 == 0), "D must be multiple of 8");
    hipLaunchKernelGGL(bias_gelu_fwd_bf16, dim3(ew_grid(n, 8)), dim3(BLOCK), 0,
                       stream, (const unsigned short*)x.data_ptr(),
                       (const unsigned short*)bias.data_ptr(),
                       (unsigned short*)y.data_ptr(), n, D, has_bias);
  } else {
    hipLaunchKernelGGL(bias_gelu_fwd_f32, dim3(ew_grid(n)), dim3(BLOCK), 0,
                       stream, x.data_ptr<float>(), bias.data_ptr<float>(),
                       y.data_ptr<float>(), n, D, has_bias);
  }
  HIP_CHECK_LAST();
  return y;
}

torch::Tensor bias_gelu_bwd(torch::Tensor dy, torch::Tensor x,
                            torch::Tensor bias) {
  auto dx = torch::empty_like(x);
  long n = x.numel();
  int D = x.size(-1);
  int has_bias = bias.numel() > 0 ? 1 : 0;
  auto stream = at::cuda::getCurrentHIPStream();
  if (x.scalar_type() == torch::kBFloat16) {
    TORCH_CHECK(!has_bias || (D % 8 == 0), "D must be multiple of 8");
    hipLaunchKernelGGL(bias_gelu_bwd_bf16, dim3(ew_grid(n, 8)), dim3(BLOCK), 0,
                       stream, (const unsigned short*)dy.data_ptr(),
                       (const unsigned short*)x.data_ptr(),
                       (const unsigned short*)bias.data_ptr(),
                       (unsigned short*)dx.data_ptr(), n, D, has_bias);
  } else {
    hipLaunchKernelGGL(bias_gelu_bwd_f32, dim3(ew_grid(n)), dim3(BLOCK), 0,
                       stream, dy.data_ptr<float>(), x.data_ptr<float>(),
                       bias.data_ptr<float>(), dx.data_ptr<float>(),
                       n, D, has_bias);
  }
  HIP_CHECK_LAST();
  return dx;
}

void adamw_step(torch::Tensor p, torch::Tensor g, torch::Tensor m,
                torch::Tensor v, long step, double lr, double beta1,
                double beta2, double eps, double wd) {
  check_adamw_flat(p, g, m, v);
  long n = p.numel();
  auto stream = at::cuda::getCurrentHIPStream();
  hipLaunchKernelGGL(adamw_kernel, dim3(ew_grid(n)), dim3(BLOCK), 0, stream,
                     p.data_ptr<float>(), g.data_ptr<float>(),
                     m.data_ptr<float>(), v.data_ptr<float>(), n,
                     (float)beta1, (float)beta2, (float)eps,
                     adam_coef_host(step, lr, beta1, beta2, wd),
                     (const float*)nullptr);
  HIP_CHECK_LAST();
}

void adamw_step_dev(torch::Tensor p, torch::Tensor g, torch::Tensor m,
                    torch::Tensor v, torch::Tensor coef, double beta1,
                    double beta2, double eps) {
  check_adamw_flat(p, g, m, v);
  check_adam_coef(coef, p);
  long n = p.numel();
  auto stream = at::cuda::getCurrentHIPStream();
  hipLaunchKernelGGL(adamw_kernel, dim3(ew_grid(n)), dim3(BLOCK), 0, stream,
                     p.data_ptr<float>(), g.data_ptr<float>(),
                     m.data_ptr<float>(), v.data_ptr<float>(), n,
                     (float)beta1, (float)beta2, (float)eps, AdamCoef{},
                     (const float*)coef.data_ptr<float>());
  HIP_CHECK_LAST();
}

void adamw_prelude(torch::Tensor step, torch::Tensor hyp, torch::Tensor coef) {
  TORCH_CHECK(step.is_cuda() && step.scalar_type() == torch::kLong &&
              step.numel() == 1, "adamw_prelude: step must be a device int64");
  TORCH_CHECK(hyp.is_cuda() && hyp.scalar_type() == torch::kDouble &&
              hyp.is_contiguous() && hyp.dim() == 2 &&
              hyp.size(1) == ADAM_NHYP,
              "adamw_prelude: hyp must be a contiguous device double (G, 4)");
  TORCH_CHECK(coef.is_cuda() && coef.scalar_type() == torch::kFloat &&
              coef.is_contiguous() && coef.dim() == 2 &&
              coef.size(0) == hyp.size(0) && coef.size(1) == ADAM_NCOEF,
              "adamw_prelude: coef must be a contiguous device float (G, 5)");
  TORCH_CHECK(step.get_device() == hyp.get_device() &&
              step.get_device() == coef.get_device());
  auto stream = at::cuda::getCurrentHIPStream();
  hipLaunchKernelGGL(adam_prelude_kernel, dim3(1), dim3(WAVE), 0, stream,
                     (long*)step.data_ptr<int64_t>(), hyp.data_ptr<double>(),
                     coef.data_ptr<float>(), (int)hyp.size(0));
  HIP_CHECK_LAST();
}

namespace {
__global__ void ema_bf16_kernel(float* __restrict__ ema,
                                const unsigned short* __restrict__ p, long n,
                                float decay, float omd, int vec4) {
  const long n4 = vec4 ? (n >> 2) : 0;
  const long i0 = (long)blockIdx.x * blockDim.x + threadIdx.x;
  const long stride = (long)gridDim.x * blockDim.x;
  for (long i = i0; i < n4; i += stride) {
    float4 e = *(const float4*)(ema + i * 4);
    ushort4 v = *(const ushort4*)(p + i * 4);
    e.x = decay * e.x + omd * bf2f(v.x);
    e.y = decay * e.y + omd * bf2f(v.y);
    e.z = decay * e.z + omd * bf2f(v.z);
    e.w = decay * e.w + omd * bf2f(v.w);
    *(float4*)(ema + i * 4) = e;
  }
  for (long i = n4 * 4 + i0; i < n; i += stride)
    ema[i] = decay * ema[i] + omd * bf2f(p[i]);
}
}

void ema_update(torch::Tensor ema, torch::Tensor p, double decay) {
  TORCH_CHECK(ema.is_cuda() && ema.scalar_type() == torch::kFloat);
  TORCH_CHECK(p.is_cuda() && p.get_device() == ema.get_device(),
              "ema_update: p must be on ema's device");
  TORCH_CHECK(p.scalar_type() == torch::kFloat ||
              p.scalar_type() == torch::kBFloat16,
              "ema_update: p must be fp32 or bf16");
  TORCH_CHECK(p.numel() == ema.numel(), "ema_update: p has ", p.numel(),
              " elements, ema has ", ema.numel());
  TORCH_CHECK(ema.is_contiguous() && p.is_contiguous(),
              "ema_update: ema and p must be contiguous");
  long n = ema.numel();
  const float omd = (float)(1.0 - decay);
  auto stream = at::cuda::getCurrentHIPStream();
  const int vec4 = (((unsigned long long)ema.data_ptr() & 15) == 0 &&
                    ((unsigned long long)p.data_ptr() &
                     (p.scalar_type() == torch::kBFloat16 ? 7 : 15)) == 0)
                   ? 1 : 0;
  if (p.scalar_type() == torch::kBFloat16) {
    hipLaunchKernelGGL(ema_bf16_kernel, dim3(ew_grid(n, 4)), dim3(BLOCK), 0,
                       stream, ema.data_ptr<float>(),
                       (const unsigned short*)p.data_ptr(), n, (float)decay,
                       omd, vec4);
  } else {
    hipLaunchKernelGGL(ema_kernel, dim3(ew_grid(n, 4)), dim3(BLOCK), 0,
                       stream, ema.data_ptr<float>(), p.data_ptr<float>(), n,
                       (float)decay, omd, vec4);
  }
  HIP_CHECK_LAST();
}

torch::Tensor l2norm_sq(torch::Tensor x) {
  TORCH_CHECK(x.is_cuda() && x.is_contiguous());
  auto out = torch::empty({}, x.options().dtype(torch::kFloat));
  long n = x.numel();
  const int grid = ew_grid(n);
  auto partial = grid == 1 ? out
      : torch::empty({grid}, x.options().dtype(torch::kFloat));
  auto stream = at::cuda::getCurrentHIPStream();
  if (x.scalar_type() == torch::kBFloat16) {
    hipLaunchKernelGGL(l2norm_kernel<bf16_t>, dim3(grid), dim3(BLOCK), 0,
                       stream, (const bf16_t*)x.data_ptr(),
                       partial.data_ptr<float>(), n);
  } else {
    hipLaunchKernelGGL(l2norm_kernel<float>, dim3(grid), dim3(BLOCK), 0,
                       stream, x.data_ptr<float>(), partial.data_ptr<float>(),
                       n);
  }
  HIP_CHECK_LAST();
  if (grid > 1) {
    hipLaunchKernelGGL(l2norm_final_kernel, dim3(1), dim3(BLOCK), 0, stream,
                       (const float*)partial.data_ptr<float>(),
                       out.data_ptr<float>(), grid);
    HIP_CHECK_LAST();
  }
  return out;
}

void scale_inplace(torch::Tensor x, double s) {
  TORCH_CHECK(x.is_cuda() && x.is_contiguous());
  long n = x.numel();
  auto stream = at::cuda::getCurrentHIPStream();
  if (x.scalar_type() == torch::kBFloat16) {
    hipLaunchKernelGGL(scale_kernel<bf16_t>, dim3(ew_grid(n)), dim3(BLOCK), 0,
                       stream, (bf16_t*)x.data_ptr(), n, (float)s);
  } else {
    hipLaunchKernelGGL(scale_kernel<float>, dim3(ew_grid(n)), dim3(BLOCK), 0,
                       stream, x.data_ptr<float>(), n, (float)s);
  }
  HIP_CHECK_LAST();
}


namespace {

constexpr long MT_CHUNK = 1 << 16;

__global__ void multi_adamw_kernel(const int* __restrict__ cpid,
                                   const long* __restrict__ coff,
                                   const long* __restrict__ pptrs,
                                   const long* __restrict__ gptrs,
                                   const long* __restrict__ mptrs,
                                   const long* __restrict__ moffs,
                                   const long* __restrict__ numels,
                                   int nchunks,
                                   float* __restrict__ m,
                                   float* __restrict__ v,
                                   float beta1, float beta2, float eps,
                                   AdamCoef ch,
                                   const float* __restrict__ cdev,
                                   int param_bf16, int grad_bf16) {
  const int c = blockIdx.x;
  if (c >= nchunks) return;
  const AdamCoef cf = adam_coef_load(ch, cdev);
  const int pid = cpid[c];
  const long off = coff[c];
  const long n = numels[pid];
  const long end = off + MT_CHUNK < n ? off + MT_CHUNK : n;
  const long mvbase = moffs[pid];
  float* master = (float*)mptrs[pid];
  void* pp = (void*)pptrs[pid];
  const void* gp = (const void*)gptrs[pid];
  if (gp == nullptr) return;
  const bool vec4 = ((off | mvbase) & 3) == 0 &&
      (((long)master | (long)pp | (long)gp) & 15) == 0;
  if (vec4) {
    const long nv = (end - off) >> 2;
    for (long g = threadIdx.x; g < nv; g += blockDim.x) {
      const long i = off + g * 4;
      const long k = mvbase + i;
      float4 gi4;
      if (gp == nullptr) gi4 = make_float4(0.f, 0.f, 0.f, 0.f);
      else if (grad_bf16) {
        ushort4 gu = *(const ushort4*)((const unsigned short*)gp + i);
        gi4 = make_float4(bf2f(gu.x), bf2f(gu.y), bf2f(gu.z), bf2f(gu.w));
      } else {
        gi4 = *(const float4*)((const float*)gp + i);
      }
      float4 p4 = *(const float4*)(master + i);
      float4 m4 = *(const float4*)(m + k);
      float4 v4 = *(const float4*)(v + k);
      float* pi = (float*)&p4;
      float* mi = (float*)&m4;
      float* vi = (float*)&v4;
      const float* gi = (const float*)&gi4;
      ushort4 pb;
      unsigned short* pbs = (unsigned short*)&pb;
#pragma unroll
      for (int j = 0; j < 4; ++j) {
        adam_elem(pi[j], mi[j], vi[j], gi[j], beta1, beta2, eps, cf);
        pbs[j] = f2bf(pi[j]);
      }
      *(float4*)(m + k) = m4;
      *(float4*)(v + k) = v4;
      *(float4*)(master + i) = p4;
      if (param_bf16) *(ushort4*)((unsigned short*)pp + i) = pb;
    }
    for (long i = off + nv * 4 + threadIdx.x; i < end; i += blockDim.x) {
      float gi;
      if (gp == nullptr) gi = 0.f;
      else if (grad_bf16) gi = bf2f(((const unsigned short*)gp)[i]);
      else gi = ((const float*)gp)[i];
      const long k = mvbase + i;
      float pi = master[i], mi = m[k], vi = v[k];
      adam_elem(pi, mi, vi, gi, beta1, beta2, eps, cf);
      m[k] = mi;
      v[k] = vi;
      master[i] = pi;
      if (param_bf16) ((unsigned short*)pp)[i] = f2bf(pi);
    }
    return;
  }
  for (long i = off + threadIdx.x; i < end; i += blockDim.x) {
    float gi;
    if (gp == nullptr) gi = 0.f;
    else if (grad_bf16) gi = bf2f(((const unsigned short*)gp)[i]);
    else gi = ((const float*)gp)[i];
    const long k = mvbase + i;
    float pi = master[i], mi = m[k], vi = v[k];
    adam_elem(pi, mi, vi, gi, beta1, beta2, eps, cf);
    m[k] = mi;
    v[k] = vi;
    master[i] = pi;
    if (param_bf16) ((unsigned short*)pp)[i] = f2bf(pi);
  }
}

}

namespace {
void launch_multi_adamw(const torch::Tensor& cpid, const torch::Tensor& coff,
                        const torch::Tensor& pptrs, const torch::Tensor& gptrs,
                        const torch::Tensor& mptrs, const torch::Tensor& moffs,
                        const torch::Tensor& numels, const torch::Tensor& m,
                        const torch::Tensor& v, double beta1, double beta2,
                        double eps, AdamCoef ch, const float* cdev,
                        bool param_bf16, bool grad_bf16) {
  TORCH_CHECK(m.is_cuda() && m.scalar_type() == torch::kFloat);
  int nchunks = cpid.numel();
  auto stream = at::cuda::getCurrentHIPStream();
  hipLaunchKernelGGL(multi_adamw_kernel, dim3(nchunks), dim3(BLOCK), 0,
                     stream, cpid.data_ptr<int>(), coff.data_ptr<long>(),
                     pptrs.data_ptr<long>(), gptrs.data_ptr<long>(),
                     mptrs.data_ptr<long>(), moffs.data_ptr<long>(),
                     numels.data_ptr<long>(),
                     nchunks, m.data_ptr<float>(),
                     v.data_ptr<float>(), (float)beta1, (float)beta2,
                     (float)eps, ch, cdev,
                     param_bf16 ? 1 : 0, grad_bf16 ? 1 : 0);
  HIP_CHECK_LAST();
}
}

void multi_adamw_step(torch::Tensor cpid, torch::Tensor coff,
                      torch::Tensor pptrs, torch::Tensor gptrs,
                      torch::Tensor mptrs, torch::Tensor moffs,
                      torch::Tensor numels,
                      torch::Tensor m, torch::Tensor v,
                      long step, double lr, double beta1, double beta2,
                      double eps, double wd, bool param_bf16,
                      bool grad_bf16) {
  launch_multi_adamw(cpid, coff, pptrs, gptrs, mptrs, moffs, numels, m, v,
                     beta1, beta2, eps,
                     adam_coef_host(step, lr, beta1, beta2, wd), nullptr,
                     param_bf16, grad_bf16);
}

void multi_adamw_step_dev(torch::Tensor cpid, torch::Tensor coff,
                          torch::Tensor pptrs, torch::Tensor gptrs,
                          torch::Tensor mptrs, torch::Tensor moffs,
                          torch::Tensor numels,
                          torch::Tensor m, torch::Tensor v,
                          torch::Tensor coef, double beta1, double beta2,
                          double eps, bool param_bf16, bool grad_bf16) {
  check_adam_coef(coef, m);
  launch_multi_adamw(cpid, coff, pptrs, gptrs, mptrs, moffs, numels, m, v,
                     beta1, beta2, eps, AdamCoef{}, coef.data_ptr<float>(),
                     param_bf16, grad_bf16);
}
```

torchdistpackage_amd/ops/csrc/norms.hip:

```cpp

#include <torch/extension.h>
#include <ATen/hip/HIPContext.h>
#include "common.h"

namespace {

constexpr int BLOCK = 256;
constexpr int MAX_D = 16384;


template <typename T>
DEVINL float load_as_f32(const T* p, int i);
template <> DEVINL float load_as_f32<bf16_t>(const bf16_t* p, int i) {
  return bf2f(((const unsigned short*)p)[i]);
}
template <> DEVINL float load_as_f32<float>(const float* p, int i) {
  return p[i];
}
template <typename T>
DEVINL void store_from_f32(T* p, int i, float v);
template <> DEVINL void store_from_f32<bf16_t>(bf16_t* p, int i, float v) {
  ((unsigned short*)p)[i] = f2bf(v);
}
template <> DEVINL void store_from_f32<float>(float* p, int i, float v) {
  p[i] = v;
}

template <typename T>
__global__ void rmsnorm_fwd_kernel(const T* __restrict__ x,
                                   const T* __restrict__ w,
                                   T* __restrict__ y,
                                   float* __restrict__ rstd,
                                   int rows, int D, float eps) {
  __shared__ float lds[BLOCK / WAVE];
  for (int row = blockIdx.x; row < rows; row += gridDim.x) {
    const T* xr = x + (long)row * D;
    T* yr = y + (long)row * D;
    float ss = 0.f;
    for (int i = threadIdx.x; i < D; i += BLOCK) {
      float v = load_as_f32(xr, i);
      ss += v * v;
    }
    ss = block_sum<BLOCK>(ss, lds);
    float r = rsqrtf(ss / D + eps);
    if (threadIdx.x == 0) rstd[row] = r;
    for (int i = threadIdx.x; i < D; i += BLOCK) {
      float v = load_as_f32(xr, i);
      float wv = load_as_f32(w, i);
      store_from_f32(yr, i, v * r * wv);
    }
    __syncthreads();
  }
}

template <typename T>
__global__ void rmsnorm_bwd_kernel(const T* __restrict__ dy,
                                   const T* __restrict__ x,
                                   const T* __restrict__ w,
                                   const float* __restrict__ rstd,
                                   T* __restrict__ dx,
                                   int rows, int D) {
  __shared__ float scratch[BLOCK / WAVE];
  for (int row = blockIdx.x; row < rows; row += gridDim.x) {
    const T* dyr = dy + (long)row * D;
    const T* xr = x + (long)row * D;
    T* dxr = dx + (long)row * D;
    float r = rstd[row];
    float dot = 0.f;
    for (int i = threadIdx.x; i < D; i += BLOCK) {
      float xhat = load_as_f32(xr, i) * r;
      float wdy = load_as_f32(w, i) * load_as_f32(dyr, i);
      dot += wdy * xhat;
    }
    dot = block_sum<BLOCK>(dot, scratch) / D;
    for (int i = threadIdx.x; i < D; i += BLOCK) {
      float xhat = load_as_f32(xr, i) * r;
      float dyv = load_as_f32(dyr, i);
      float wdy = load_as_f32(w, i) * dyv;
      store_from_f32(dxr, i, r * (wdy - xhat * dot));
    }
    __syncthreads();
  }
}

constexpr int DW_COLS = 16;
constexpr int DW_LANES = BLOCK / DW_COLS;

template <typename T, bool MEAN>
__global__ void norm_bwd_dwdb_kernel(const T* __restrict__ dy,
                                     const T* __restrict__ x,
                                     const float* __restrict__ mean,
                                     const float* __restrict__ rstd,
                                     float* __restrict__ dw,
                                     float* __restrict__ db,
                                     int rows, int D) {
  __shared__ float lds_w[DW_LANES][DW_COLS];
  __shared__ float lds_b[DW_LANES][DW_COLS];
  const int c = threadIdx.x % DW_COLS;
  const int lane = threadIdx.x / DW_COLS;
  const int col = blockIdx.x * DW_COLS + c;
  float aw = 0.f, ab = 0.f;
  if (col < D) {
    for (int row = lane; row < rows; row += DW_LANES) {
      const long off = (long)row * D;
      float xv = load_as_f32(x + off, col);
      float dyv = load_as_f32(dy + off, col);
      float xhat = MEAN ? (xv - mean[row]) * rstd[row] : xv * rstd[row];
      aw += dyv * xhat;
      ab += dyv;
    }
  }
  lds_w[lane][c] = aw;
  lds_b[lane][c] = ab;
  __syncthreads();
  if (lane == 0 && col < D) {
    float sw = 0.f, sb = 0.f;
    for (int l = 0; l < DW_LANES; ++l) {
      sw += lds_w[l][c];
      sb += lds_b[l][c];
    }
    dw[col] = sw;
    if (MEAN) db[col] = sb;
  }
}


DEVINL bool ln_one_pass_ok(float mu, float var) { return mu * mu <= var; }

DEVINL void ln_finish_stats(float mu0, float d1, float d2, int D, float eps,
                            float& mu, float& r) {
  const float c = d1 / D;
  mu = mu0 + c;
  const float var = fmaxf(d2 / D - c * c, 0.f);
  r = rsqrtf(var + eps);
}

template <typename T>
__global__ void layernorm_fwd_kernel(const T* __restrict__ x,
                                     const T* __restrict__ w,
                                     const T* __restrict__ b,
                                     T* __restrict__ y,
                                     float* __restrict__ mean,
                                     float* __restrict__ rstd,
                                     int rows, int D, float eps) {
  __shared__ float lds[3 * BLOCK / WAVE];
  for (int row = blockIdx.x; row < rows; row += gridDim.x) {
    const T* xr = x + (long)row * D;
    T* yr = y + (long)row * D;
    float s = 0.f, ss = 0.f;
    for (int i = threadIdx.x; i < D; i += BLOCK) {
      float v = load_as_f32(xr, i);
      s += v;
      ss += v * v;
    }
    s = block_sum<BLOCK>(s, lds);
    __syncthreads();
    ss = block_sum<BLOCK>(ss, lds);
    float mu = s / D;
    float var = ss / D - mu * mu;
    float r = rsqrtf(var + eps);
    if (!ln_one_pass_ok(mu, var)) {
      const float mu0 = mu;
      float d1 = 0.f, d2 = 0.f;
      for (int i = threadIdx.x; i < D; i += BLOCK) {
        float d = load_as_f32(xr, i) - mu0;
        d1 += d;
        d2 += d * d;
      }
      d1 = block_sum<BLOCK>(d1, lds + BLOCK / WAVE);
      d2 = block_sum<BLOCK>(d2, lds + 2 * BLOCK / WAVE);
      ln_finish_stats(mu0, d1, d2, D, eps, mu, r);
    }
    if (threadIdx.x == 0) { mean[row] = mu; rstd[row] = r; }
    for (int i = threadIdx.x; i < D; i += BLOCK) {
      float v = load_as_f32(xr, i);
      float wv = load_as_f32(w, i);
      float bv = load_as_f32(b, i);
      store_from_f32(yr, i, (v - mu) * r * wv + bv);
    }
    __syncthreads();
  }
}

template <typename T>
__global__ void layernorm_bwd_kernel(const T* __restrict__ dy,
                                     const T* __restrict__ x,
                                     const T* __restrict__ w,
                                     const float* __restrict__ mean,
                                     const float* __restrict__ rstd,
                                     T* __restrict__ dx,
                                     int rows, int D) {
  __shared__ float scratch[BLOCK / WAVE];
  for (int row = blockIdx.x; row < rows; row += gridDim.x) {
    const T* dyr = dy + (long)row * D;
    const T* xr = x + (long)row * D;
    T* dxr = dx + (long)row * D;
    float mu = mean[row], r = rstd[row];
    float m1 = 0.f, m2 = 0.f;
    for (int i = threadIdx.x; i < D; i += BLOCK) {
      float xhat = (load_as_f32(xr, i) - mu) * r;
      float wdy = load_as_f32(w, i) * load_as_f32(dyr, i);
      m1 += wdy;
      m2 += wdy * xhat;
    }
    m1 = block_sum<BLOCK>(m1, scratch);
    __syncthreads();
    m2 = block_sum<BLOCK>(m2, scratch);
    m1 /= D;
    m2 /= D;
    for (int i = threadIdx.x; i < D; i += BLOCK) {
      float xhat = (load_as_f32(xr, i) - mu) * r;
      float dyv = load_as_f32(dyr, i);
      float wdy = load_as_f32(w, i) * dyv;
      store_from_f32(dxr, i, r * (wdy - m1 - xhat * m2));
    }
    __syncthreads();
  }
}

int pick_grid(long rows) {
  long g = rows < 2048 ? rows : 2048;
  return (int)(g > 0 ? g : 1);
}


typedef ushort4 u4;
struct f8 { float v[8]; };

DEVINL f8 load8f(const unsigned short* p) {
  u4 a = *(const u4*)p;
  u4 b = *(const u4*)(p + 4);
  f8 r;
  r.v[0] = bf2f(a.x); r.v[1] = bf2f(a.y); r.v[2] = bf2f(a.z); r.v[3] = bf2f(a.w);
  r.v[4] = bf2f(b.x); r.v[5] = bf2f(b.y); r.v[6] = bf2f(b.z); r.v[7] = bf2f(b.w);
  return r;
}

DEVINL void store8f(unsigned short* p, const f8& r) {
  u4 a, b;
  a.x = f2bf(r.v[0]); a.y = f2bf(r.v[1]); a.z = f2bf(r.v[2]); a.w = f2bf(r.v[3]);
  b.x = f2bf(r.v[4]); b.y = f2bf(r.v[5]); b.z = f2bf(r.v[6]); b.w = f2bf(r.v[7]);
  *(u4*)p = a;
  *(u4*)(p + 4) = b;
}

__global__ void rmsnorm_fwd_bf16v8(const unsigned short* __restrict__ x,
                                   const unsigned short* __restrict__ w,
                                   unsigned short* __restrict__ y,
                                   float* __restrict__ rstd,
                                   int rows, int D, float eps) {
  __shared__ float lds[BLOCK / WAVE];
  for (int row = blockIdx.x; row < rows; row += gridDim.x) {
    const unsigned short* xr = x + (long)row * D;
    unsigned short* yr = y + (long)row * D;
    float ss = 0.f;
    for (int i = threadIdx.x * 8; i < D; i += BLOCK * 8) {
      f8 v = load8f(xr + i);
#pragma unroll
      for (int j = 0; j < 8; ++j) ss += v.v[j] * v.v[j];
    }
    ss = block_sum<BLOCK>(ss, lds);
    float r = rsqrtf(ss / D + eps);
    if (threadIdx.x == 0) rstd[row] = r;
    for (int i = threadIdx.x * 8; i < D; i += BLOCK * 8) {
      f8 v = load8f(xr + i);
      f8 wv = load8f(w + i);
      f8 out;
#pragma unroll
      for (int j = 0; j < 8; ++j) out.v[j] = v.v[j] * r * wv.v[j];
      store8f(yr + i, out);
    }
    __syncthreads();
  }
}

__global__ void rmsnorm_bwd_bf16v8(const unsigned short* __restrict__ dy,
                                   const unsigned short* __restrict__ x,
                                   const unsigned short* __restrict__ w,
                                   const float* __restrict__ rstd,
                                   unsigned short* __restrict__ dx,
                                   int rows, int D) {
  __shared__ float scratch[BLOCK / WAVE];
  for (int row = blockIdx.x; row < rows; row += gridDim.x) {
    const unsigned short* dyr = dy + (long)row * D;
    const unsigned short* xr = x + (long)row * D;
    unsigned short* dxr = dx + (long)row * D;
    float r = rstd[row];
    float dot = 0.f;
    for (int i = threadIdx.x * 8; i < D; i += BLOCK * 8) {
      f8 xv = load8f(xr + i), dyv = load8f(dyr + i), wv = load8f(w + i);
#pragma unroll
      for (int j = 0; j < 8; ++j)
        dot += wv.v[j] * dyv.v[j] * xv.v[j] * r;
    }
    dot = block_sum<BLOCK>(dot, scratch) / D;
    for (int i = threadIdx.x * 8; i < D; i += BLOCK * 8) {
      f8 xv = load8f(xr + i), dyv = load8f(dyr + i), wv = load8f(w + i);
      f8 out;
#pragma unroll
      for (int j = 0; j < 8; ++j) {
        float xhat = xv.v[j] * r;
        out.v[j] = r * (wv.v[j] * dyv.v[j] - xhat * dot);
      }
      store8f(dxr + i, out);
    }
    __syncthreads();
  }
}

template <int NC>
__global__ void __launch_bounds__(BLOCK)
layernorm_fwd_bf16v8(const unsigned short* __restrict__ x,
                     const unsigned short* __restrict__ w,
                     const unsigned short* __restrict__ b,
                     unsigned short* __restrict__ y,
                     float* __restrict__ mean,
                     float* __restrict__ rstd,
                     int rows, int D, float eps) {
  __shared__ float lds[4 * BLOCK / WAVE];
  const int wid = threadIdx.x / WAVE;
  for (int row = blockIdx.x; row < rows; row += gridDim.x) {
    const unsigned short* xr = x + (long)row * D;
    unsigned short* yr = y + (long)row * D;
    f8 xv[NC];
    float s = 0.f, ss = 0.f;
#pragma unroll
    for (int c = 0; c < NC; ++c) {
      int i = threadIdx.x * 8 + c * BLOCK * 8;
      if (i < D) {
        xv[c] = load8f(xr + i);
#pragma unroll
        for (int j = 0; j < 8; ++j) {
          s += xv[c].v[j];
          ss += xv[c].v[j] * xv[c].v[j];
        }
      }
    }
    {
      float sw = wave_sum(s), ssw = wave_sum(ss);
      if ((threadIdx.x & (WAVE - 1)) == 0) {
        lds[wid] = sw;
        lds[BLOCK / WAVE + wid] = ssw;
      }
      __syncthreads();
      s = 0.f; ss = 0.f;
#pragma unroll
      for (int i = 0; i < BLOCK / WAVE; ++i) {
        s += lds[i];
        ss += lds[BLOCK / WAVE + i];
      }
    }
    float mu = s / D;
    float var = ss / D - mu * mu;
    float r = rsqrtf(var + eps);
    if (!ln_one_pass_ok(mu, var)) {
      const float mu0 = mu;
      float d1 = 0.f, d2 = 0.f;
#pragma unroll
      for (int c = 0; c < NC; ++c) {
        int i = threadIdx.x * 8 + c * BLOCK * 8;
        if (i < D) {
#pragma unroll
          for (int j = 0; j < 8; ++j) {
            float d = xv[c].v[j] - mu0;
            d1 += d;
            d2 += d * d;
          }
        }
      }
      float a = wave_sum(d1), q = wave_sum(d2);
      if ((threadIdx.x & (WAVE - 1)) == 0) {
        lds[2 * BLOCK / WAVE + wid] = a;
        lds[3 * BLOCK / WAVE + wid] = q;
      }
      __syncthreads();
      d1 = 0.f; d2 = 0.f;
#pragma unroll
      for (int i = 0; i < BLOCK / WAVE; ++i) {
        d1 += lds[2 * BLOCK / WAVE + i];
        d2 += lds[3 * BLOCK / WAVE + i];
      }
      ln_finish_stats(mu0, d1, d2, D, eps, mu, r);
    }
    if (threadIdx.x == 0) { mean[row] = mu; rstd[row] = r; }
#pragma unroll
    for (int c = 0; c < NC; ++c) {
      int i = threadIdx.x * 8 + c * BLOCK * 8;
      if (i < D) {
        f8 wv = load8f(w + i), bv = load8f(b + i);
        f8 out;
#pragma unroll
        for (int j = 0; j < 8; ++j)
          out.v[j] = (xv[c].v[j] - mu) * r * wv.v[j] + bv.v[j];
        store8f(yr + i, out);
      }
    }
    __syncthreads();
  }
}

__global__ void layernorm_bwd_bf16v8(const unsigned short* __restrict__ dy,
                                     const unsigned short* __restrict__ x,
                                     const unsigned short* __restrict__ w,
                                     const float* __restrict__ mean,
                                     const float* __restrict__ rstd,
                                     unsigned short* __restrict__ dx,
                                     int rows, int D) {
  __shared__ float scratch[2 * BLOCK / WAVE];
  for (int row = blockIdx.x; row < rows; row += gridDim.x) {
    const unsigned short* dyr = dy + (long)row * D;
    const unsigned short* xr = x + (long)row * D;
    unsigned short* dxr = dx + (long)row * D;
    float mu = mean[row], r = rstd[row];
    float m1 = 0.f, m2 = 0.f;
    for (int i = threadIdx.x * 8; i < D; i += BLOCK * 8) {
      f8 xv = load8f(xr + i), dyv = load8f(dyr + i), wv = load8f(w + i);
#pragma unroll
      for (int j = 0; j < 8; ++j) {
        float xhat = (xv.v[j] - mu) * r;
        float wdy = wv.v[j] * dyv.v[j];
        m1 += wdy;
        m2 += wdy * xhat;
      }
    }
    {
      const int wid = threadIdx.x / WAVE;
      float a = wave_sum(m1), c = wave_sum(m2);
      if ((threadIdx.x & (WAVE - 1)) == 0) {
        scratch[wid] = a;
        scratch[BLOCK / WAVE + wid] = c;
      }
      __syncthreads();
      m1 = 0.f; m2 = 0.f;
#pragma unroll
      for (int i = 0; i < BLOCK / WAVE; ++i) {
        m1 += scratch[i];
        m2 += scratch[BLOCK / WAVE + i];
      }
    }
    m1 /= D;
    m2 /= D;
    for (int i = threadIdx.x * 8; i < D; i += BLOCK * 8) {
      f8 xv = load8f(xr + i), dyv = load8f(dyr + i), wv = load8f(w + i);
      f8 out;
#pragma unroll
      for (int j = 0; j < 8; ++j) {
        float xhat = (xv.v[j] - mu) * r;
        out.v[j] = r * (wv.v[j] * dyv.v[j] - m1 - xhat * m2);
      }
      store8f(dxr + i, out);
    }
    __syncthreads();
  }
}

template <int NC>
__global__ void rmsnorm_bwd_bf16_reg(const unsigned short* __restrict__ dy,
                                     const unsigned short* __restrict__ x,
                                     const unsigned short* __restrict__ w,
                                     const float* __restrict__ rstd,
                                     unsigned short* __restrict__ dx,
                                     float* __restrict__ dw_partial,
                                     int rows, int D) {
  __shared__ float scratch[BLOCK / WAVE];
  float acc_dw[NC][8];
#pragma unroll
  for (int c = 0; c < NC; ++c)
#pragma unroll
    for (int j = 0; j < 8; ++j) acc_dw[c][j] = 0.f;

  for (int row = blockIdx.x; row < rows; row += gridDim.x) {
    const unsigned short* dyr = dy + (long)row * D;
    const unsigned short* xr = x + (long)row * D;
    unsigned short* dxr = dx + (long)row * D;
    float r = rstd[row];
    float dot = 0.f;
    f8 xv[NC], dyv[NC], wv[NC];
#pragma unroll
    for (int c = 0; c < NC; ++c) {
      int i = threadIdx.x * 8 + c * BLOCK * 8;
      if (i < D) {
        xv[c] = load8f(xr + i);
        dyv[c] = load8f(dyr + i);
        wv[c] = load8f(w + i);
#pragma unroll
        for (int j = 0; j < 8; ++j)
          dot += wv[c].v[j] * dyv[c].v[j] * xv[c].v[j] * r;
      }
    }
    dot = block_sum<BLOCK>(dot, scratch) / D;
#pragma unroll
    for (int c = 0; c < NC; ++c) {
      int i = threadIdx.x * 8 + c * BLOCK * 8;
      if (i < D) {
        f8 out;
#pragma unroll
        for (int j = 0; j < 8; ++j) {
          float xhat = xv[c].v[j] * r;
          out.v[j] = r * (wv[c].v[j] * dyv[c].v[j] - xhat * dot);
          acc_dw[c][j] += dyv[c].v[j] * xhat;
        }
        store8f(dxr + i, out);
      }
    }
    __syncthreads();
  }
  float* dwp = dw_partial + (long)blockIdx.x * D;
#pragma unroll
  for (int c = 0; c < NC; ++c) {
    int i = threadIdx.x * 8 + c * BLOCK * 8;
    if (i < D)
#pragma unroll
      for (int j = 0; j < 8; ++j) dwp[i + j] = acc_dw[c][j];
  }
}

template <int NC>
__global__ void layernorm_bwd_bf16_reg(const unsigned short* __restrict__ dy,
                                       const unsigned short* __restrict__ x,
                                       const unsigned short* __restrict__ w,
                                       const float* __restrict__ mean,
                                       const float* __restrict__ rstd,
                                       unsigned short* __restrict__ dx,
                                       float* __restrict__ dw_partial,
                                       float* __restrict__ db_partial,
                                       int rows, int D) {
  __shared__ float scratch[2 * BLOCK / WAVE];
  float acc_dw[NC][8], acc_db[NC][8];
#pragma unroll
  for (int c = 0; c < NC; ++c)
#pragma unroll
    for (int j = 0; j < 8; ++j) { acc_dw[c][j] = 0.f; acc_db[c][j] = 0.f; }

  for (int row = blockIdx.x; row < rows; row += gridDim.x) {
    const unsigned short* dyr = dy + (long)row * D;
    const unsigned short* xr = x + (long)row * D;
    unsigned short* dxr = dx + (long)row * D;
    float mu = mean[row], r = rstd[row];
    float m1 = 0.f, m2 = 0.f;
    f8 xv[NC], dyv[NC], wv[NC];
#pragma unroll
    for (int c = 0; c < NC; ++c) {
      int i = threadIdx.x * 8 + c * BLOCK * 8;
      if (i < D) {
        xv[c] = load8f(xr + i);
        dyv[c] = load8f(dyr + i);
        wv[c] = load8f(w + i);
#pragma unroll
        for (int j = 0; j < 8; ++j) {
          float xhat = (xv[c].v[j] - mu) * r;
          float wdy = wv[c].v[j] * dyv[c].v[j];
          m1 += wdy;
          m2 += wdy * xhat;
        }
      }
    }
    {
      const int wid = threadIdx.x / WAVE;
      float a = wave_sum(m1), cgr = wave_sum(m2);
      if ((threadIdx.x & (WAVE - 1)) == 0) {
        scratch[wid] = a;
        scratch[BLOCK / WAVE + wid] = cgr;
      }
      __syncthreads();
      m1 = 0.f; m2 = 0.f;
#pragma unroll
      for (int i = 0; i < BLOCK / WAVE; ++i) {
        m1 += scratch[i];
        m2 += scratch[BLOCK / WAVE + i];
      }
    }
    m1 /= D;
    m2 /= D;
#pragma unroll
    for (int c = 0; c < NC; ++c) {
      int i = threadIdx.x * 8 + c * BLOCK * 8;
      if (i < D) {
        f8 out;
#pragma unroll
        for (int j = 0; j < 8; ++j) {
          float xhat = (xv[c].v[j] - mu) * r;
          out.v[j] = r * (wv[c].v[j] * dyv[c].v[j] - m1 - xhat * m2);
          acc_dw[c][j] += dyv[c].v[j] * xhat;
          acc_db[c][j] += dyv[c].v[j];
        }
        store8f(dxr + i, out);
      }
    }
    __syncthreads();
  }
  float* dwp = dw_partial + (long)blockIdx.x * D;
  float* dbp = db_partial + (long)blockIdx.x * D;
#pragma unroll
  for (int c = 0; c < NC; ++c) {
    int i = threadIdx.x * 8 + c * BLOCK * 8;
    if (i < D)
#pragma unroll
      for (int j = 0; j < 8; ++j) {
        dwp[i + j] = acc_dw[c][j];
        dbp[i + j] = acc_db[c][j];
      }
  }
}

}


std::vector<torch::Tensor> rmsnorm_fwd(torch::Tensor x, torch::Tensor w,
                                       double eps) {
  TORCH_CHECK(x.is_cuda() && x.is_contiguous());
  const int D = x.size(-1);
  TORCH_CHECK(D <= MAX_D, "D too large");
  const long rows = x.numel() / D;
  auto y = torch::empty_like(x);
  auto rstd = torch::empty({rows}, x.options().dtype(torch::kFloat));
  auto stream = at::cuda::getCurrentHIPStream();
  dim3 grid(pick_grid(rows)), block(BLOCK);
  if (x.scalar_type() == torch::kBFloat16 && D % 8 == 0) {
    hipLaunchKernelGGL(rmsnorm_fwd_bf16v8, grid, block, 0, stream,
                       (const unsigned short*)x.data_ptr(),
                       (const unsigned short*)w.data_ptr(),
                       (unsigned short*)y.data_ptr(), rstd.data_ptr<float>(),
                       (int)rows, D, (float)eps);
  } else if (x.scalar_type() == torch::kBFloat16) {
    hipLaunchKernelGGL(rmsnorm_fwd_kernel<bf16_t>, grid, block, 0, stream,
                       (const bf16_t*)x.data_ptr(), (const bf16_t*)w.data_ptr(),
                       (bf16_t*)y.data_ptr(), rstd.data_ptr<float>(),
                       (int)rows, D, (float)eps);
  } else {
    TORCH_CHECK(x.scalar_type() == torch::kFloat, "bf16/f32 only");
    hipLaunchKernelGGL(rmsnorm_fwd_kernel<float>, grid, block, 0, stream,
                       x.data_ptr<float>(), w.data_ptr<float>(),
                       y.data_ptr<float>(), rstd.data_ptr<float>(),
                       (int)rows, D, (float)eps);
  }
  HIP_CHECK_LAST();
  return {y, rstd};
}

std::vector<torch::Tensor> rmsnorm_bwd(torch::Tensor dy, torch::Tensor x,
                                       torch::Tensor w, torch::Tensor rstd) {
  const int D = x.size(-1);
  const long rows = x.numel() / D;
  auto dx = torch::empty_like(x);
  auto stream = at::cuda::getCurrentHIPStream();
  dim3 grid(pick_grid(rows)), block(BLOCK);
  const bool reg_path = x.scalar_type() == torch::kBFloat16 &&
      D % 8 == 0 && D <= 4 * BLOCK * 8;
  if (reg_path) {
    auto dw_partial = torch::empty({(long)grid.x, (long)D},
                                   x.options().dtype(torch::kFloat));
    int nc = (D + BLOCK * 8 - 1) / (BLOCK * 8);
#define RMS_REG(NC)                                                          \
    hipLaunchKernelGGL(rmsnorm_bwd_bf16_reg<NC>, grid, block, 0, stream,     \
                       (const unsigned short*)dy.data_ptr(),                 \
                       (const unsigned short*)x.data_ptr(),                  \
                       (const unsigned short*)w.data_ptr(),                  \
                       rstd.data_ptr<float>(),                               \
                       (unsigned short*)dx.data_ptr(),                       \
                       dw_partial.data_ptr<float>(), (int)rows, D)
    if (nc == 1) RMS_REG(1); else if (nc == 2) RMS_REG(2);
    else if (nc == 3) RMS_REG(3); else RMS_REG(4);
#undef RMS_REG
    HIP_CHECK_LAST();
    return {dx, dw_partial.sum(0).to(w.scalar_type())};
  }
  auto dw = torch::empty({D}, x.options().dtype(torch::kFloat));
  dim3 grid_dw((D + DW_COLS - 1) / DW_COLS);
  if (x.scalar_type() == torch::kBFloat16) {
    if (D % 8 == 0) {
      hipLaunchKernelGGL(rmsnorm_bwd_bf16v8, grid, block, 0, stream,
                         (const unsigned short*)dy.data_ptr(),
                         (const unsigned short*)x.data_ptr(),
                         (const unsigned short*)w.data_ptr(),
                         rstd.data_ptr<float>(),
                         (unsigned short*)dx.data_ptr(), (int)rows, D);
    } else {
      hipLaunchKernelGGL(rmsnorm_bwd_kernel<bf16_t>, grid, block, 0, stream,
                         (const bf16_t*)dy.data_ptr(),
                         (const bf16_t*)x.data_ptr(),
                         (const bf16_t*)w.data_ptr(), rstd.data_ptr<float>(),
                         (bf16_t*)dx.data_ptr(), (int)rows, D);
    }
    hipLaunchKernelGGL((norm_bwd_dwdb_kernel<bf16_t, false>), grid_dw, block,
                       0, stream, (const bf16_t*)dy.data_ptr(),
                       (const bf16_t*)x.data_ptr(), (const float*)nullptr,
                       rstd.data_ptr<float>(), dw.data_ptr<float>(),
                       (float*)nullptr, (int)rows, D);
  } else {
    TORCH_CHECK(x.scalar_type() == torch::kFloat, "bf16/f32 only");
    hipLaunchKernelGGL(rmsnorm_bwd_kernel<float>, grid, block, 0, stream,
                       dy.data_ptr<float>(), x.data_ptr<float>(),
                       w.data_ptr<float>(), rstd.data_ptr<float>(),
                       dx.data_ptr<float>(), (int)rows, D);
    hipLaunchKernelGGL((norm_bwd_dwdb_kernel<float, false>), grid_dw, block,
                       0, stream, dy.data_ptr<float>(), x.data_ptr<float>(),
                       (const float*)nullptr, rstd.data_ptr<float>(),
                       dw.data_ptr<float>(), (float*)nullptr, (int)rows, D);
  }
  HIP_CHECK_LAST();
  return {dx, dw.to(w.scalar_type())};
}

std::vector<torch::Tensor> layernorm_fwd(torch::Tensor x, torch::Tensor w,
                                         torch::Tensor b, double eps) {
  TORCH_CHECK(x.is_cuda() && x.is_contiguous());
  const int D = x.size(-1);
  TORCH_CHECK(D <= MAX_D, "D too large");
  const long rows = x.numel() / D;
  auto y = torch::empty_like(x);
  auto mean = torch::empty({rows}, x.options().dtype(torch::kFloat));
  auto rstd = torch::empty({rows}, x.options().dtype(torch::kFloat));
  auto stream = at::cuda::getCurrentHIPStream();
  dim3 grid(pick_grid(rows)), block(BLOCK);
  if (x.scalar_type() == torch::kBFloat16 && D % 8 == 0) {
    const int nc = (D + BLOCK * 8 - 1) / (BLOCK * 8);
#define LN_FWD(NC)                                                           \
    hipLaunchKernelGGL(layernorm_fwd_bf16v8<NC>, grid, block, 0, stream,     \
                       (const unsigned short*)x.data_ptr(),                  \
                       (const unsigned short*)w.data_ptr(),                  \
                       (const unsigned short*)b.data_ptr(),                  \
                       (unsigned short*)y.data_ptr(),                        \
                       mean.data_ptr<float>(), rstd.data_ptr<float>(),       \
                       (int)rows, D, (float)eps)
    if (nc == 1) LN_FWD(1); else if (nc == 2) LN_FWD(2);
    else if (nc <= 4) LN_FWD(4); else LN_FWD(8);
#undef LN_FWD
  } else if (x.scalar_type() == torch::kBFloat16) {
    hipLaunchKernelGGL(layernorm_fwd_kernel<bf16_t>, grid, block, 0, stream,
                       (const bf16_t*)x.data_ptr(), (const bf16_t*)w.data_ptr(),
                       (const bf16_t*)b.data_ptr(), (bf16_t*)y.data_ptr(),
                       mean.data_ptr<float>(), rstd.data_ptr<float>(),
                       (int)rows, D, (float)eps);
  } else {
    TORCH_CHECK(x.scalar_type() == torch::kFloat, "bf16/f32 only");
    hipLaunchKernelGGL(layernorm_fwd_kernel<float>, grid, block, 0, stream,
                       x.data_ptr<float>(), w.data_ptr<float>(),
                       b.data_ptr<float>(), y.data_ptr<float>(),
                       mean.data_ptr<float>(), rstd.data_ptr<float>(),
                       (int)rows, D, (float)eps);
  }
  HIP_CHECK_LAST();
  return {y, mean, rstd};
}

std::vector<torch::Tensor> layernorm_bwd(torch::Tensor dy, torch::Tensor x,
                                         torch::Tensor w, torch::Tensor mean,
                                         torch::Tensor rstd) {
  const int D = x.size(-1);
  const long rows = x.numel() / D;
  auto dx = torch::empty_like(x);
  auto stream = at::cuda::getCurrentHIPStream();
  dim3 grid(pick_grid(rows)), block(BLOCK);
  const bool reg_path = x.scalar_type() == torch::kBFloat16 &&
      D % 8 == 0 && D <= 4 * BLOCK * 8;
  if (reg_path) {
    auto dw_partial = torch::empty({(long)grid.x, (long)D},
                                   x.options().dtype(torch::kFloat));
    auto db_partial = torch::empty({(long)grid.x, (long)D},
                                   x.options().dtype(torch::kFloat));
    int nc = (D + BLOCK * 8 - 1) / (BLOCK * 8);
#define LN_REG(NC)                                                           \
    hipLaunchKernelGGL(layernorm_bwd_bf16_reg<NC>, grid, block, 0, stream,   \
                       (const unsigned short*)dy.data_ptr(),                 \
                       (const unsigned short*)x.data_ptr(),                  \
                       (const unsigned short*)w.data_ptr(),                  \
                       mean.data_ptr<float>(), rstd.data_ptr<float>(),       \
                       (unsigned short*)dx.data_ptr(),                       \
                       dw_partial.data_ptr<float>(),                         \
                       db_partial.data_ptr<float>(), (int)rows, D)
    if (nc == 1) LN_REG(1); else if (nc == 2) LN_REG(2);
    else if (nc == 3) LN_REG(3); else LN_REG(4);
#undef LN_REG
    HIP_CHECK_LAST();
    return {dx, dw_partial.sum(0).to(w.scalar_type()),
            db_partial.sum(0).to(w.scalar_type())};
  }
  auto dw = torch::empty({D}, x.options().dtype(torch::kFloat));
  auto db = torch::empty({D}, x.options().dtype(torch::kFloat));
  dim3 grid_dw((D + DW_COLS - 1) / DW_COLS);
  if (x.scalar_type() == torch::kBFloat16) {
    if (D % 8 == 0) {
      hipLaunchKernelGGL(layernorm_bwd_bf16v8, grid, block, 0, stream,
                         (const unsigned short*)dy.data_ptr(),
                         (const unsigned short*)x.data_ptr(),
                         (const unsigned short*)w.data_ptr(),
                         mean.data_ptr<float>(), rstd.data_ptr<float>(),
                         (unsigned short*)dx.data_ptr(), (int)rows, D);
    } else {
      hipLaunchKernelGGL(layernorm_bwd_kernel<bf16_t>, grid, block, 0, stream,
                         (const bf16_t*)dy.data_ptr(),
                         (const bf16_t*)x.data_ptr(),
                         (const bf16_t*)w.data_ptr(), mean.data_ptr<float>(),
                         rstd.data_ptr<float>(), (bf16_t*)dx.data_ptr(),
                         (int)rows, D);
    }
    hipLaunchKernelGGL((norm_bwd_dwdb_kernel<bf16_t, true>), grid_dw, block,
                       0, stream, (const bf16_t*)dy.data_ptr(),
                       (const bf16_t*)x.data_ptr(), mean.data_ptr<float>(),
                       rstd.data_ptr<float>(), dw.data_ptr<float>(),
                       db.data_ptr<float>(), (int)rows, D);
  } else {
    TORCH_CHECK(x.scalar_type() == torch::kFloat, "bf16/f32 only");
    hipLaunchKernelGGL(layernorm_bwd_kernel<float>, grid, block, 0, stream,
                       dy.data_ptr<float>(), x.data_ptr<float>(),
                       w.data_ptr<float>(), mean.data_ptr<float>(),
                       rstd.data_ptr<float>(), dx.data_ptr<float>(),
                       (int)rows, D);
    hipLaunchKernelGGL((norm_bwd_dwdb_kernel<float, true>), grid_dw, block,
                       0, stream, dy.data_ptr<float>(), x.data_ptr<float>(),
                       mean.data_ptr<float>(), rstd.data_ptr<float>(),
                       dw.data_ptr<float>(), db.data_ptr<float>(),
                       (int)rows, D);
  }
  HIP_CHECK_LAST();
  return {dx, dw.to(w.scalar_type()), db.to(w.scalar_type())};
}
```

torchdistpackage_amd/parallel/tensor/attn.py:

```python

from __future__ import annotations

from typing import Optional

import torch
import torch.nn as nn
import torch.nn.functional as F

from ...ops import (decode_attention, fused_qkv_attention,
                    resolve_decode_attn_impl)
from .tp_utils import (ColParallelLinear, RowParallelLinear, TpLinear,
                       copy_to_tp_region, gather_from_sequence_parallel_region,
                       get_tp_size, is_sequence_parallel)


def _cached_sdpa(q: torch.Tensor, k_cache: torch.Tensor,
                 v_cache: torch.Tensor, pos0: int,
                 causal: bool) -> torch.Tensor:
    S = q.shape[2]
    ka = k_cache[:, :, :pos0 + S]
    va = v_cache[:, :, :pos0 + S]
    if not causal or S == 1:
        return F.scaled_dot_product_attention(q, ka, va)
    if pos0 == 0:
        return F.scaled_dot_product_attention(q, ka, va, is_causal=True)
    mask = torch.arange(pos0 + S, device=q.device)[None, :] <= \
        (pos0 + torch.arange(S, device=q.device))[:, None]
    return F.scaled_dot_product_attention(q, ka, va, attn_mask=mask)


def _sdpa(x_qkv: torch.Tensor, n_head: int, causal: bool) -> torch.Tensor:
    return fused_qkv_attention(x_qkv.contiguous(), n_head, causal=causal)


class Attention(nn.Module):

    def __init__(self, dim: int, n_head: int, bias: bool = True,
                 causal: bool = True, device=None, dtype=None):
        super().__init__()
        assert dim % n_head == 0
        self.n_head = n_head
        self.causal = causal
        self.qkv = TpLinear(dim, 3 * dim, bias=bias, device=device, dtype=dtype)
        self.proj = TpLinear(dim, dim, bias=bias, device=device, dtype=dtype)

    def forward(self, x):
        return self.proj(_sdpa(self.qkv(x), self.n_head, self.causal))


class TpAttention(nn.Module):

    def __init__(self, dim: int, n_head: int, bias: bool = True,
                 causal: bool = True, sequence_parallel: bool = False,
                 device=None, dtype=None):
        super().__init__()
        tp = get_tp_size()
        assert dim % n_head == 0 and n_head % tp == 0, (dim, n_head, tp)
        self.n_head = n_head
        self.n_head_local = n_head // tp
        self.causal = causal
        self.qkv = ColParallelLinear(dim, 3 * dim, bias=bias,
                                     device=device, dtype=dtype)
        self.proj = RowParallelLinear(dim, dim, bias=bias,
                                      sequence_parallel=sequence_parallel,
                                      device=device, dtype=dtype)

    def forward(self, x):
        if is_sequence_parallel(x):
            x = gather_from_sequence_parallel_region(x)
        else:
            x = copy_to_tp_region(x)
        from ...ops.gemm import linear as fast_linear
        qkv = fast_linear(x, self.qkv.weight, self.qkv.bias)
        o = _sdpa(qkv, self.n_head_local, self.causal)
        return self.proj(o)

    @torch.no_grad()
    def decode_step(self, x: torch.Tensor, k_cache: torch.Tensor,
                    v_cache: torch.Tensor, pos0: int,
                    attn_impl: Optional[str] = None) -> torch.Tensor:
        from ...ops.gemm import linear as fast_linear
        S, B, D = x.shape
        hl = self.n_head_local
        hd = D // self.n_head
        qkv = fast_linear(x, self.qkv.weight, self.qkv.bias)
        q, k, v = qkv.split(hl * hd, dim=-1)

        def v4(t):
            return t.reshape(S, B, hl, hd).permute(1, 2, 0, 3)

        q, k, v = v4(q), v4(k), v4(v)
        k_cache[:, :, pos0:pos0 + S] = k
        v_cache[:, :, pos0:pos0 + S] = v
        if resolve_decode_attn_impl(attn_impl) == "hip":
            assert self.causal or S == 1, \
                "decode_attention is causal over the new rows"
            o = decode_attention(q, k_cache, v_cache, pos0)
        else:
            o = _cached_sdpa(q, k_cache, v_cache, pos0, self.causal)
        o = o.permute(2, 0, 1, 3).reshape(S, B, hl * hd)
        return self.proj(o)

    @torch.no_grad()
    def init_from_full(self, full_attn: Attention):
        self.qkv.init_qkv_weight_from_full(full_attn.qkv.weight,
                                           full_attn.qkv.bias, num_splits=3)
        self.proj.init_weight_from_full(full_attn.proj.weight,
                                        full_attn.proj.bias)
```

torchdistpackage_amd/parallel/tensor/mlp.py:

```python

from __future__ import annotations

import torch
import torch.nn as nn
import torch.nn.functional as F

from .tp_utils import (ColParallelLinear, RowParallelLinear, TpLinear,
                       get_tp_size, is_sequence_parallel,
                       maybe_gather_for_sequence_parallel)
from ...ops import bias_gelu


class Mlp(nn.Module):

    def __init__(self, dim: int, hidden_mult: int = 4, bias: bool = True,
                 device=None, dtype=None):
        super().__init__()
        self.fc1 = TpLinear(dim, dim * hidden_mult, bias=bias,
                            device=device, dtype=dtype)
        self.fc2 = TpLinear(dim * hidden_mult, dim, bias=bias,
                            device=device, dtype=dtype)

    def forward(self, x):
        return self.fc2(F.gelu(self.fc1(x), approximate="tanh"))


class TpMlp(nn.Module):

    def __init__(self, dim: int, hidden_mult: int = 4, bias: bool = True,
                 dropout: float = 0.0, sequence_parallel: bool = False,
                 device=None, dtype=None):
        super().__init__()
        self.dropout = dropout
        self.fc1 = ColParallelLinear(dim, dim * hidden_mult, bias=bias,
                                     device=device, dtype=dtype)
        self.fc2 = RowParallelLinear(dim * hidden_mult, dim, bias=bias,
                                     sequence_parallel=sequence_parallel,
                                     device=device, dtype=dtype)

    def forward(self, x):
        from .tp_utils import copy_to_tp_region, \
            gather_from_sequence_parallel_region
        if is_sequence_parallel(x):
            x = gather_from_sequence_parallel_region(x)
        else:
            x = copy_to_tp_region(x)
        from ...ops.gemm import linear as fast_linear
        h = fast_linear(x, self.fc1.weight)
        h = bias_gelu(h, self.fc1.bias)
        if self.dropout > 0 and self.training:
            h = F.dropout(h, p=self.dropout)
        return self.fc2(h)

    @torch.no_grad()
    def init_weight_from_full(self, full_mlp: Mlp):
        self.fc1.init_weight_from_full(full_mlp.fc1.weight,
                                       full_mlp.fc1.bias)
        self.fc2.init_weight_from_full(full_mlp.fc2.weight,
                                       full_mlp.fc2.bias)
```

torchdistpackage_amd/parallel/tensor/tp_utils.py:

```python

from __future__ import annotations

from typing import Optional

import torch
import torch.distributed as dist
import torch.nn as nn
import torch.nn.functional as F

from ...ops.gemm import linear as fast_linear

_TP_GROUP: Optional[dist.ProcessGroup] = None


def set_tp_group(group: Optional[dist.ProcessGroup]):
    global _TP_GROUP
    _TP_GROUP = group


def get_tp_group() -> Optional[dist.ProcessGroup]:
    global _TP_GROUP
    if _TP_GROUP is None:
        try:
            from ...dist.topo import tpc
            if tpc.is_mode_inited("tensor"):
                _TP_GROUP = tpc.get_group("tensor")
        except Exception:
            pass
    return _TP_GROUP


def get_tp_size() -> int:
    g = get_tp_group()
    return dist.get_world_size(g) if (g is not None and dist.is_initialized()) else 1


def get_tp_rank() -> int:
    g = get_tp_group()
    return dist.get_rank(g) if (g is not None and dist.is_initialized()) else 0


def _backend_is_gloo(group) -> bool:
    try:
        return dist.get_backend(group) == "gloo"
    except Exception:
        return False



def _all_gather_first_dim(x: torch.Tensor) -> torch.Tensor:
    tp = get_tp_size()
    if tp == 1:
        return x
    group = get_tp_group()
    out_shape = list(x.shape)
    out_shape[0] *= tp
    out = torch.empty(out_shape, dtype=x.dtype, device=x.device)
    dist.all_gather_into_tensor(out, x.contiguous(), group=group)
    return out


def _reduce_scatter_first_dim(x: torch.Tensor) -> torch.Tensor:
    tp = get_tp_size()
    if tp == 1:
        return x
    group = get_tp_group()
    assert x.shape[0] % tp == 0, \
        f"first dim {x.shape[0]} not divisible by tp {tp}"
    out_shape = list(x.shape)
    out_shape[0] //= tp
    x = x.contiguous()
    if _backend_is_gloo(group):
        x = x.clone()
        dist.all_reduce(x, group=group)
        r = dist.get_rank(group)
        return x.narrow(0, r * out_shape[0], out_shape[0]).clone()
    out = torch.empty(out_shape, dtype=x.dtype, device=x.device)
    dist.reduce_scatter_tensor(out, x, group=group)
    return out


def _split_first_dim(x: torch.Tensor) -> torch.Tensor:
    tp = get_tp_size()
    if tp == 1:
        return x
    r = get_tp_rank()
    n = x.shape[0] // tp
    return x.narrow(0, r * n, n).contiguous()


def _all_reduce(x: torch.Tensor) -> torch.Tensor:
    if get_tp_size() == 1:
        return x
    dist.all_reduce(x, group=get_tp_group())
    return x



class _ReduceFromTp(torch.autograd.Function):

    @staticmethod
    def forward(ctx, x):
        return _all_reduce(x.clone())

    @staticmethod
    def backward(ctx, grad):
        return grad


class _CopyToTp(torch.autograd.Function):

    @staticmethod
    def forward(ctx, x):
        return x

    @staticmethod
    def backward(ctx, grad):
        return _all_reduce(grad.contiguous().clone())


class _ReduceScatterToSp(torch.autograd.Function):

    @staticmethod
    def forward(ctx, x):
        return _reduce_scatter_first_dim(x)

    @staticmethod
    def backward(ctx, grad):
        return _all_gather_first_dim(grad.contiguous())


class _GatherFromSp(torch.autograd.Function):

    @staticmethod
    def forward(ctx, x, bwd_mode: str = "reduce_scatter"):
        ctx.bwd_mode = bwd_mode
        return _all_gather_first_dim(x)

    @staticmethod
    def backward(ctx, grad):
        grad = grad.contiguous()
        if ctx.bwd_mode == "split":
            return _split_first_dim(grad), None
        return _reduce_scatter_first_dim(grad), None


def reduce_from_tp_region(x):
    return _ReduceFromTp.apply(x)


def copy_to_tp_region(x):
    return _CopyToTp.apply(x)


def reduce_scatter_to_sequence_parallel_region(x):
    out = _ReduceScatterToSp.apply(x)
    set_sequence_parallel_attr(out)
    return out


def gather_from_sequence_parallel_region(x, bwd_mode: str = "reduce_scatter"):
    return _GatherFromSp.apply(x, bwd_mode)



def set_sequence_parallel_attr(t: torch.Tensor):
    t.sequence_parallel = True


def is_sequence_parallel(t: torch.Tensor) -> bool:
    return getattr(t, "sequence_parallel", False)


def maybe_gather_for_sequence_parallel(t: torch.Tensor) -> torch.Tensor:
    if is_sequence_parallel(t):
        return gather_from_sequence_parallel_region(t)
    return t


def maybe_split_into_sequence_parallel(t: torch.Tensor) -> torch.Tensor:
    if get_tp_size() == 1 or is_sequence_parallel(t):
        return t
    out = _SplitToSp.apply(t)
    set_sequence_parallel_attr(out)
    return out


class _SplitToSp(torch.autograd.Function):
    @staticmethod
    def forward(ctx, x):
        return _split_first_dim(x)

    @staticmethod
    def backward(ctx, grad):
        return _all_gather_first_dim(grad.contiguous())


class _GatherLastDim(torch.autograd.Function):

    @staticmethod
    def forward(ctx, x):
        tp = get_tp_size()
        if tp == 1:
            return x
        xs = [torch.empty_like(x) for _ in range(tp)]
        dist.all_gather(xs, x.contiguous(), group=get_tp_group())
        return torch.cat(xs, dim=-1)

    @staticmethod
    def backward(ctx, grad):
        tp = get_tp_size()
        if tp == 1:
            return grad
        n = grad.shape[-1] // tp
        return grad.narrow(-1, get_tp_rank() * n, n).contiguous()



class TpLinear(nn.Module):

    def __init__(self, in_features: int, out_features: int, bias: bool = True,
                 device=None, dtype=None):
        super().__init__()
        kw = {"device": device, "dtype": dtype}
        self.in_features = in_features
        self.out_features = out_features
        self.weight = nn.Parameter(torch.empty(out_features, in_features, **kw))
        self.bias = nn.Parameter(torch.empty(out_features, **kw)) if bias \
            else None
        self.reset_parameters()

    def reset_parameters(self):
        nn.init.normal_(self.weight, std=0.02)
        if self.bias is not None:
            nn.init.zeros_(self.bias)

    def forward(self, x):
        return fast_linear(x, self.weight, self.bias)


class ColParallelLinear(TpLinear):

    def __init__(self, in_features: int, out_features: int, bias: bool = True,
                 gather_output: bool = False, device=None, dtype=None):
        tp = get_tp_size()
        assert out_features % tp == 0, (out_features, tp)
        self.full_out_features = out_features
        self.gather_output = gather_output
        super().__init__(in_features, out_features // tp, bias=bias,
                         device=device, dtype=dtype)

    def forward(self, x):
        x = copy_to_tp_region(x)
        out = fast_linear(x, self.weight, self.bias)
        if self.gather_output and get_tp_size() > 1:
            out = _GatherLastDim.apply(out)
        return out

    @torch.no_grad()
    def init_weight_from_full(self, full_weight: torch.Tensor,
                              full_bias: Optional[torch.Tensor] = None):
        tp, r = get_tp_size(), get_tp_rank()
        shard = full_weight.chunk(tp, dim=0)[r]
        self.weight.copy_(shard)
        if full_bias is not None and self.bias is not None:
            self.bias.copy_(full_bias.chunk(tp, dim=0)[r])

    @torch.no_grad()
    def init_qkv_weight_from_full(self, full_weight: torch.Tensor,
                                  full_bias: Optional[torch.Tensor] = None,
                                  num_splits: int = 3):
        tp, r = get_tp_size(), get_tp_rank()
        chunks = full_weight.chunk(num_splits, dim=0)
        mine = torch.cat([c.chunk(tp, dim=0)[r] for c in chunks], dim=0)
        self.weight.copy_(mine)
        if full_bias is not None and self.bias is not None:
            bchunks = full_bias.chunk(num_splits, dim=0)
            self.bias.copy_(
                torch.cat([c.chunk(tp, dim=0)[r] for c in bchunks], dim=0))


class RowParallelLinear(TpLinear):

    def __init__(self, in_features: int, out_features: int, bias: bool = True,
                 sequence_parallel: bool = False, device=None, dtype=None):
        tp = get_tp_size()
        assert in_features % tp == 0, (in_features, tp)
        self.full_in_features = in_features
        self.sequence_parallel = sequence_parallel
        super().__init__(in_features // tp, out_features, bias=bias,
                         device=device, dtype=dtype)

    def forward(self, x):
        out = fast_linear(x, self.weight)
        if self.sequence_parallel and get_tp_size() > 1:
            out = reduce_scatter_to_sequence_parallel_region(out)
        else:
            out = reduce_from_tp_region(out)
        if self.bias is not None:
            out = out + self.bias
        return out

    @torch.no_grad()
    def init_weight_from_full(self, full_weight: torch.Tensor,
                              full_bias: Optional[torch.Tensor] = None):
        tp, r = get_tp_size(), get_tp_rank()
        shard = full_weight.chunk(tp, dim=1)[r]
        self.weight.copy_(shard)
        if full_bias is not None and self.bias is not None:
            self.bias.copy_(full_bias)


def mark_sequence_parallel_params(module: "nn.Module"):
    for p in module.parameters():
        p.sequence_parallel_param = True


def allreduce_sequence_parallel_grads(module: "nn.Module"):
    if get_tp_size() == 1:
        return
    group = get_tp_group()
    grads = [p.grad for p in module.parameters()
             if getattr(p, "sequence_parallel_param", False)
             and p.grad is not None]
    if not grads:
        return
    flat = torch.cat([g.reshape(-1) for g in grads])
    dist.all_reduce(flat, group=group)
    off = 0
    for g in grads:
        g.copy_(flat[off:off + g.numel()].view_as(g))
        off += g.numel()



get_tensor_model_parallel_world_size = get_tp_size
maybe_gather_from_sequence_parallel = maybe_gather_for_sequence_parallel
is_squence_parallel_tensor = is_sequence_parallel
```

torchdistpackage_amd/parallel/tensor/transformer.py:

```python

from __future__ import annotations

import torch
import torch.nn as nn

from ...ops import LayerNorm
from .attn import Attention, TpAttention
from .mlp import Mlp, TpMlp
from .tp_utils import (gather_from_sequence_parallel_region, get_tp_size,
                       is_sequence_parallel,
                       maybe_split_into_sequence_parallel,
                       set_sequence_parallel_attr)


class Block(nn.Module):

    def __init__(self, dim: int, n_head: int, hidden_mult: int = 4,
                 bias: bool = True, causal: bool = True,
                 device=None, dtype=None):
        super().__init__()
        kw = {"device": device, "dtype": dtype}
        self.ln_1 = LayerNorm(dim, **kw)
        self.attn = Attention(dim, n_head, bias=bias, causal=causal, **kw)
        self.ln_2 = LayerNorm(dim, **kw)
        self.mlp = Mlp(dim, hidden_mult, bias=bias, **kw)

    def forward(self, x):
        x = x + self.attn(self.ln_1(x))
        x = x + self.mlp(self.ln_2(x))
        return x


class ParallelBlock(nn.Module):

    def __init__(self, dim: int, n_head: int, hidden_mult: int = 4,
                 bias: bool = True, causal: bool = True, dropout: float = 0.0,
                 sequence_parallel: bool = True, device=None, dtype=None):
        super().__init__()
        kw = {"device": device, "dtype": dtype}
        self.sequence_parallel = sequence_parallel and get_tp_size() > 1
        self.dropout = dropout
        self.ln_1 = LayerNorm(dim, **kw)
        self.attn = TpAttention(dim, n_head, bias=bias, causal=causal,
                                sequence_parallel=self.sequence_parallel, **kw)
        self.ln_2 = LayerNorm(dim, **kw)
        self.mlp = TpMlp(dim, hidden_mult, bias=bias, dropout=dropout,
                         sequence_parallel=self.sequence_parallel, **kw)
        if self.sequence_parallel:
            from .tp_utils import mark_sequence_parallel_params
            mark_sequence_parallel_params(self.ln_1)
            mark_sequence_parallel_params(self.ln_2)

    def forward(self, x):
        if self.sequence_parallel:
            x = maybe_split_into_sequence_parallel(x)
        h = self.ln_1(x)
        if self.sequence_parallel:
            set_sequence_parallel_attr(h)
        a = self.attn(h)
        if self.dropout > 0 and self.training:
            import torch.nn.functional as F
            a = F.dropout(a, p=self.dropout)
        x = x + a
        h = self.ln_2(x)
        if self.sequence_parallel:
            set_sequence_parallel_attr(h)
        x = x + self.mlp(h)
        if self.sequence_parallel:
            set_sequence_parallel_attr(x)
        return x

    @torch.no_grad()
    def decode_step(self, x, k_cache, v_cache, pos0: int, attn_impl=None):
        x = x + self.attn.decode_step(self.ln_1(x), k_cache, v_cache, pos0,
                                      attn_impl)
        return x + self.mlp(self.ln_2(x))

    @torch.no_grad()
    def init_from_full(self, full: Block):
        self.ln_1.load_state_dict(full.ln_1.state_dict())
        self.ln_2.load_state_dict(full.ln_2.state_dict())
        self.attn.init_from_full(full.attn)
        self.mlp.init_weight_from_full(full.mlp)


class Transformer(nn.Module):

    def __init__(self, dim: int, n_head: int, depth: int,
                 hidden_mult: int = 4, parallel: bool = True,
                 causal: bool = True, sequence_parallel: bool = True,
                 device=None, dtype=None):
        super().__init__()
        cls = ParallelBlock if parallel else Block
        kw = dict(bias=True, causal=causal, device=device, dtype=dtype)
        if parallel:
            kw["sequence_parallel"] = sequence_parallel
        self.blocks = nn.ModuleList(
            [cls(dim, n_head, hidden_mult, **kw) for _ in range(depth)])

    def forward(self, x):
        for blk in self.blocks:
            x = blk(x)
        if is_sequence_parallel(x) and get_tp_size() > 1:
            x = gather_from_sequence_parallel_region(x, bwd_mode="split")
        return x
```

Measured before the change: 107,700 tokens/s.

## Fuse bias-add, residual-add and LayerNorm in transformer blocks, plus fused backward colsums

Adds fused HIP kernels that combine the output-projection bias, residual add and the next LayerNorm into one pass. The LayerNorm backward also absorbs the residual gradient and the bias column sums. The bias-GELU backward now emits per-block partial column sums, so the separate bias-gradient reduction is gone. The attention delta kernel packs several rows per wave instead of one row per wave. ParallelBlock routes through this path by default, which cuts elementwise kernel launches and HBM round-trips, at the cost of many new kernels and the numerical risk that comes with them.

```diff
diff --git a/torchdistpackage_amd/ops/__init__.py b/torchdistpackage_amd/ops/__init__.py
--- a/torchdistpackage_amd/ops/__init__.py
+++ b/torchdistpackage_amd/ops/__init__.py
@@ -155,6 +155,140 @@
 
 
 
+_FUSED_RESIDUAL = os.environ.get("TDPA_FUSED_RESIDUAL", "1") != "0"
+
+
+def fused_residual_enabled() -> bool:
+    return _FUSED_RESIDUAL
+
+
+def set_fused_residual(on: bool) -> bool:
+    global _FUSED_RESIDUAL
+    prev, _FUSED_RESIDUAL = _FUSED_RESIDUAL, bool(on)
+    return prev
+
+
+def _bf16_rows_ok(*ts) -> bool:
+    t0 = ts[0]
+    if t0.dim() < 1 or t0.numel() == 0 or t0.shape[-1] % 8 != 0:
+        return False
+    return all(t.is_cuda and t.dtype == torch.bfloat16 and t.is_contiguous()
+               and t.shape == t0.shape and t.device == t0.device
+               and t.data_ptr() % 16 == 0 for t in ts)
+
+
+def _bf16_vecs_ok(like, *vs) -> bool:
+    D = like.shape[-1]
+    return all(v is None or (
+        v.is_cuda and v.dtype == torch.bfloat16 and v.is_contiguous()
+        and v.numel() == D and v.device == like.device
+        and v.data_ptr() % 16 == 0) for v in vs)
+
+
+def _fused_ln_ok(x, weight, bias, *more_rows, vec=None) -> bool:
+    return (_FUSED_RESIDUAL and _bf16_rows_ok(x, *more_rows)
+            and x.shape[-1] <= ext("layer_norm").fused_ln_max_d()
+            and _bf16_vecs_ok(x, weight, bias, vec))
+
+
+def _ln_bwd_residual(dh, x, weight, mean, rstd, g_res, want_colsum):
+    g, partial = ext("layer_norm").layernorm_bwd_residual(
+        dh.contiguous(), x, weight, mean, rstd, g_res.contiguous(),
+        want_colsum)
+    sums = [partial[k].sum(0).to(weight.dtype)
+            for k in range(partial.shape[0])]
+    return g, sums[0], sums[1], (sums[2] if want_colsum else None)
+
+
+class _LayerNormForkFn(torch.autograd.Function):
+
+    @staticmethod
+    def forward(ctx, x, weight, bias, eps):
+        h, mean, rstd = ext("layer_norm").layernorm_fwd(x, weight, bias, eps)
+        ctx.save_for_backward(x, weight, mean, rstd)
+        ctx.set_materialize_grads(False)
+        return x, h
+
+    @staticmethod
+    def backward(ctx, gx, gh):
+        x, weight, mean, rstd = ctx.saved_tensors
+        if gh is None:
+            return gx, None, None, None
+        if gx is None:
+            dx, dw, db = ext("layer_norm").layernorm_bwd(
+                gh.contiguous(), x, weight, mean, rstd)
+            return dx, dw, db, None
+        g, dw, db, _ = _ln_bwd_residual(gh, x, weight, mean, rstd, gx, False)
+        return g, dw, db, None
+
+
+def layer_norm_fork(x, weight, bias, eps: float = 1e-5):
+    if _fused_ln_ok(x, weight, bias) and x.shape[-1] == weight.numel():
+        return _LayerNormForkFn.apply(x, weight, bias, eps)
+    return x, layer_norm(x, weight, bias, eps)
+
+
+class _BiasResidualLayerNormFn(torch.autograd.Function):
+    @staticmethod
+    def forward(ctx, y, lin_bias, x_res, weight, bias, eps):
+        x_new, h, mean, rstd = ext("layer_norm").bias_residual_layernorm_fwd(
+            y, lin_bias, x_res, weight, bias, eps)
+        ctx.save_for_backward(x_new, weight, mean, rstd)
+        ctx.has_lin_bias = lin_bias is not None
+        ctx.set_materialize_grads(False)
+        return x_new, h
+
+    @staticmethod
+    def backward(ctx, gx, gh):
+        x_new, weight, mean, rstd = ctx.saved_tensors
+        has_b = ctx.has_lin_bias and ctx.needs_input_grad[1]
+        D = x_new.shape[-1]
+        if gh is None:
+            if gx is None:
+                return None, None, None, None, None, None
+            dlb = gx.reshape(-1, D).sum(0) if has_b else None
+            return gx, dlb, gx, None, None, None
+        if gx is None:
+            g, dw, db = ext("layer_norm").layernorm_bwd(
+                gh.contiguous(), x_new, weight, mean, rstd)
+            dlb = g.reshape(-1, D).sum(0) if has_b else None
+            return g, dlb, g, dw, db, None
+        g, dw, db, dlb = _ln_bwd_residual(gh, x_new, weight, mean, rstd, gx,
+                                          has_b)
+        return g, dlb, g, dw, db, None
+
+
+def bias_residual_layer_norm(y, lin_bias, x_res, weight, bias,
+                             eps: float = 1e-5):
+    if _fused_ln_ok(x_res, weight, bias, y, vec=lin_bias) \
+            and x_res.shape[-1] == weight.numel():
+        return _BiasResidualLayerNormFn.apply(y, lin_bias, x_res, weight,
+                                              bias, eps)
+    x_new = x_res + (y if lin_bias is None else y + lin_bias)
+    return x_new, layer_norm(x_new, weight, bias, eps)
+
+
+class _BiasResidualAddFn(torch.autograd.Function):
+    @staticmethod
+    def forward(ctx, y, lin_bias, x_res):
+        ctx.has_lin_bias = lin_bias is not None
+        return ext("bias_residual_add").bias_residual_add(y, lin_bias, x_res)
+
+    @staticmethod
+    def backward(ctx, g):
+        dlb = g.reshape(-1, g.shape[-1]).sum(0) \
+            if ctx.has_lin_bias and ctx.needs_input_grad[1] else None
+        return g, dlb, g
+
+
+def bias_residual_add(y, lin_bias, x_res):
+    if _FUSED_RESIDUAL and _bf16_rows_ok(x_res, y) \
+            and _bf16_vecs_ok(x_res, lin_bias):
+        return _BiasResidualAddFn.apply(y, lin_bias, x_res)
+    return x_res + (y if lin_bias is None else y + lin_bias)
+
+
+
 _GELU_C = math.sqrt(2.0 / math.pi)
 
 
@@ -183,6 +317,13 @@
     @staticmethod
     def backward(ctx, dy):
         x, bias = ctx.saved_tensors
+        if x.is_cuda and ctx.has_bias:
+            dy, xc = dy.contiguous(), x.contiguous()
+            if _bf16_rows_ok(xc, dy) and _bf16_vecs_ok(xc, bias) and \
+                    ext("bias_gelu").bias_gelu_bwd_colsum_ok(x.shape[-1]):
+                dx, partial = ext("bias_gelu").bias_gelu_bwd_colsum(
+                    dy, xc, bias)
+                return dx, partial.sum(0).to(x.dtype)
         if x.is_cuda:
             dx = ext("bias_gelu").bias_gelu_bwd(dy.contiguous(),
                                                 x.contiguous(), bias)
diff --git a/torchdistpackage_amd/ops/csrc/attention.hip b/torchdistpackage_amd/ops/csrc/attention.hip
--- a/torchdistpackage_amd/ops/csrc/attention.hip
+++ b/torchdistpackage_amd/ops/csrc/attention.hip
@@ -205,34 +205,56 @@
 }
 
 
+template <int LPR>
 __global__ void attn_delta_kernel(const unsigned short* __restrict__ o,
                                   const unsigned short* __restrict__ dout,
                                   float* __restrict__ delta,
                                   Strides os, Strides ds,
-                                  int B, int H, int S, int D) {
+                                  int B, int H, int S) {
   const long rows = (long)B * H * S;
-  const int wpb = blockDim.x / WAVE;
   const int lane = threadIdx.x % WAVE;
-  const long stride = (long)gridDim.x * wpb;
-  for (long row = (long)blockIdx.x * wpb + threadIdx.x / WAVE; row < rows;
-       row += stride) {
-    int s = row % S;
-    int h = (row / S) % H;
-    int b = row / ((long)S * H);
-    const unsigned short* orow = o + b * os.b + h * os.h + (long)s * os.s;
-    const unsigned short* drow = dout + b * ds.b + h * ds.h + (long)s * ds.s;
+  const int sub = lane % LPR;
+  constexpr int RPW = WAVE / LPR;
+  const long wave = (long)blockIdx.x * (blockDim.x / WAVE) + threadIdx.x / WAVE;
+  const long stride = (long)gridDim.x * (blockDim.x / WAVE) * RPW;
+  for (long row0 = wave * RPW; row0 < rows; row0 += stride) {
+    const long row = row0 + lane / LPR;
     float acc = 0.f;
-    for (int i = lane * 8; i < D; i += WAVE * 8) {
-      bf16x8_v ov = pack8(orow + i);
-      bf16x8_v dv = pack8(drow + i);
+    if (row < rows) {
+      int s = row % S;
+      int h = (row / S) % H;
+      int b = row / ((long)S * H);
+      const unsigned short* orow = o + b * os.b + h * os.h + (long)s * os.s;
+      const unsigned short* drow = dout + b * ds.b + h * ds.h + (long)s * ds.s;
+      bf16x8_v ov = pack8(orow + sub * 8);
+      bf16x8_v dv = pack8(drow + sub * 8);
       const unsigned short* op = (const unsigned short*)&ov;
       const unsigned short* dp = (const unsigned short*)&dv;
 #pragma unroll
       for (int j = 0; j < 8; ++j) acc += bf2f(op[j]) * bf2f(dp[j]);
     }
-    acc = wave_sum(acc);
-    if (lane == 0) delta[row] = acc;
-  }
+#pragma unroll
+    for (int off = LPR / 2; off > 0; off >>= 1) acc += __shfl_xor(acc, off, 64);
+    if (sub == 0 && row < rows) delta[row] = acc;
+  }
+}
+
+void launch_attn_delta(const torch::Tensor& o, const torch::Tensor& dout,
+                       torch::Tensor& delta, Strides os, Strides dos, int B,
+                       int H, int S, int D, hipStream_t stream) {
+  const long rows = (long)B * H * S;
+  const int rpb = 4 * (WAVE / (D / 8));
+  long blocks = (rows + rpb - 1) / rpb;
+  if (blocks > 2048) blocks = 2048;
+  const unsigned short* op = (const unsigned short*)o.data_ptr();
+  const unsigned short* dp = (const unsigned short*)dout.data_ptr();
+  float* delp = delta.data_ptr<float>();
+  if (D == 128)
+    hipLaunchKernelGGL(attn_delta_kernel<16>, dim3((unsigned)blocks),
+                       dim3(256), 0, stream, op, dp, delp, os, dos, B, H, S);
+  else
+    hipLaunchKernelGGL(attn_delta_kernel<8>, dim3((unsigned)blocks),
+                       dim3(256), 0, stream, op, dp, delp, os, dos, B, H, S);
 }
 
 template <int D, bool CAUSAL, int NW>
@@ -739,15 +761,7 @@
           os = get_strides(o), dos = get_strides(dout),
           dqs = get_strides(dq), dks = get_strides(dk), dvs = get_strides(dv);
 
-  {
-    long rows = (long)B * H * S;
-    long blocks = (rows + 3) / 4;
-    if (blocks > 2048) blocks = 2048;
-    hipLaunchKernelGGL(attn_delta_kernel, dim3((unsigned)blocks), dim3(256),
-                       0, stream, (const unsigned short*)o.data_ptr(),
-                       (const unsigned short*)dout.data_ptr(),
-                       delta.data_ptr<float>(), os, dos, B, H, S, D);
-  }
+  launch_attn_delta(o, dout, delta, os, dos, B, H, S, D, stream);
 
   const AttnBwdRoute route = attn_bwd_select(attn_knobs_ref(), B, H, S, D);
   if (!route.v1) {
@@ -784,3 +798,21 @@
   HIP_CHECK_LAST();
   return {dq, dk, dv};
 }
+
+torch::Tensor attn_delta(torch::Tensor o, torch::Tensor dout) {
+  TORCH_CHECK(o.is_cuda() && o.scalar_type() == torch::kBFloat16 &&
+                  o.dim() == 4,
+              "attn_delta: o must be a (B, H, S, D) bf16 device tensor");
+  const int64_t B = o.size(0), H = o.size(1), S = o.size(2), D = o.size(3);
+  TORCH_CHECK(D == 64 || D == 128,
+              "attn_delta: head_dim must be 64 or 128, got ", D);
+  TORCH_CHECK(B >= 1 && H >= 1 && S >= 1, "attn_delta: empty problem, o is ",
+              o.sizes());
+  check_operand("attn_delta", "o", o, o, B, H, S, D);
+  check_operand("attn_delta", "dout", dout, o, B, H, S, D);
+  auto delta = torch::empty({B, H, S}, o.options().dtype(torch::kFloat));
+  launch_attn_delta(o, dout, delta, get_strides(o), get_strides(dout), (int)B,
+                    (int)H, (int)S, (int)D, at::cuda::getCurrentHIPStream());
+  HIP_CHECK_LAST();
+  return delta;
+}
diff --git a/torchdistpackage_amd/ops/csrc/bindings.cpp b/torchdistpackage_amd/ops/csrc/bindings.cpp
--- a/torchdistpackage_amd/ops/csrc/bindings.cpp
+++ b/torchdistpackage_amd/ops/csrc/bindings.cpp
@@ -90,6 +90,21 @@
     torch::Tensor dy, torch::Tensor x, torch::Tensor offs,
     bool want_bias_grad);
 torch::Tensor grouped_gemm_plan(torch::Tensor offs_cpu, int64_t T);
+std::vector<torch::Tensor> bias_residual_layernorm_fwd(
+    torch::Tensor y, c10::optional<torch::Tensor> bias, torch::Tensor x_res,
+    torch::Tensor ln_w, torch::Tensor ln_b, double eps);
+std::vector<torch::Tensor> layernorm_bwd_residual(
+    torch::Tensor dh, torch::Tensor x, torch::Tensor w, torch::Tensor mean,
+    torch::Tensor rstd, torch::Tensor g_res, bool want_colsum);
+std::vector<torch::Tensor> bias_gelu_bwd_colsum(torch::Tensor dy,
+                                                torch::Tensor x,
+                                                torch::Tensor bias);
+bool bias_gelu_bwd_colsum_ok(int64_t D);
+int64_t fused_ln_max_d();
+torch::Tensor bias_residual_add(torch::Tensor y,
+                                c10::optional<torch::Tensor> bias,
+                                torch::Tensor x_res);
+torch::Tensor attn_delta(torch::Tensor o, torch::Tensor dout);
 
 PYBIND11_MODULE(TORCH_EXTENSION_NAME, m) {
   m.def("rmsnorm_fwd", &rmsnorm_fwd);
@@ -138,4 +153,20 @@
         "(offs_cpu, T) -> (row-tile bound, 3) int64: (expert, first row, "
         "row count) per block, expert -1 = idle");
   m.attr("GROUPED_GEMM_BM") = GG_BM;
+  m.def("bias_residual_layernorm_fwd", &bias_residual_layernorm_fwd,
+        "(y, bias|None, x_res, ln_w, ln_b, eps) -> (x_new, h, mean, rstd)");
+  m.def("layernorm_bwd_residual", &layernorm_bwd_residual,
+        "(dh, x, w, mean, rstd, g_res, want_colsum) -> (g, partial): "
+        "fp32 (2|3, grid, D); partial[k].sum(0), one sum per slice, = dw, db"
+        "[, colsum(g)] (one sum(1) would change the bits of dw and db)");
+  m.def("bias_gelu_bwd_colsum", &bias_gelu_bwd_colsum,
+        "(dy, x, bias) -> (dx, partial): partial.sum(0) = colsum(dx) in fp32");
+  m.def("fused_ln_max_d", &fused_ln_max_d,
+        "widest last dim of the fused LayerNorm kernels");
+  m.def("bias_gelu_bwd_colsum_ok", &bias_gelu_bwd_colsum_ok,
+        "whether bias_gelu_bwd_colsum covers last dim D");
+  m.def("bias_residual_add", &bias_residual_add,
+        "(y, bias|None, x_res) -> bf16(x_res + bf16(y + bias))");
+  m.def("attn_delta", &attn_delta,
+        "(o, dout) (B, H, S, D) bf16 -> rowsum(o * dout) (B, H, S) fp32");
 }
diff --git a/torchdistpackage_amd/ops/csrc/elementwise.hip b/torchdistpackage_amd/ops/csrc/elementwise.hip
--- a/torchdistpackage_amd/ops/csrc/elementwise.hip
+++ b/torchdistpackage_amd/ops/csrc/elementwise.hip
@@ -2,6 +2,7 @@
 #include <torch/extension.h>
 #include <ATen/hip/HIPContext.h>
 #include "common.h"
+#include "fused_checks.h"
 
 namespace {
 
@@ -24,6 +25,15 @@
   float t = tanh_fast(GELU_C * (u + GELU_A * u * u2));
   return 0.5f * (1.f + t) +
          0.5f * u * (1.f - t * t) * GELU_C * (1.f + 3.f * GELU_A * u2);
+}
+
+DEVINL float gelu_df_pinned(float u) {
+#pragma clang fp contract(off)
+  float u2 = u * u;
+  float t = tanh_fast(GELU_C * fmaf(GELU_A * u, u2, u));
+  float k = fmaf(u2, 3.f * GELU_A, 1.f);
+  float m = 0.5f * u * fmaf(-t, t, 1.f) * GELU_C * k;
+  return fmaf(1.f + t, 0.5f, m);
 }
 
 
@@ -57,13 +67,20 @@
   }
 }
 
+template <bool COLSUM>
 __global__ void bias_gelu_bwd_bf16(const unsigned short* __restrict__ dy,
                                    const unsigned short* __restrict__ x,
                                    const unsigned short* __restrict__ bias,
                                    unsigned short* __restrict__ dx,
+                                   float* __restrict__ partial,
                                    long n, int D, int has_bias) {
   long i0 = ((long)blockIdx.x * BLOCK + threadIdx.x) * 8;
   long stride = (long)gridDim.x * BLOCK * 8;
+  float acc[8];
+  if constexpr (COLSUM) {
+#pragma unroll
+    for (int j = 0; j < 8; ++j) acc[j] = 0.f;
+  }
   for (long i = i0; i < n; i += stride) {
     if (i + 8 <= n) {
       bf16x8 xv = *(const bf16x8*)(x + i);
@@ -78,15 +95,21 @@
 #pragma unroll
       for (int j = 0; j < 8; ++j) {
         float b = has_bias ? bf2f(bs[j]) : 0.f;
-        os[j] = f2bf(bf2f(gs[j]) * gelu_df(bf2f(xs[j]) + b));
+        os[j] = f2bf(bf2f(gs[j]) * gelu_df_pinned(bf2f(xs[j]) + b));
+        if constexpr (COLSUM) acc[j] += bf2f(os[j]);
       }
       *(bf16x8*)(dx + i) = out;
     } else {
       for (long j = i; j < n; ++j) {
         float b = has_bias ? bf2f(bias[j % D]) : 0.f;
-        dx[j] = f2bf(bf2f(dy[j]) * gelu_df(bf2f(x[j]) + b));
+        dx[j] = f2bf(bf2f(dy[j]) * gelu_df_pinned(bf2f(x[j]) + b));
       }
     }
+  }
+  if constexpr (COLSUM) {
+    *(float4*)(partial + i0) = make_float4(acc[0], acc[1], acc[2], acc[3]);
+    *(float4*)(partial + i0 + 4) =
+        make_float4(acc[4], acc[5], acc[6], acc[7]);
   }
 }
 
@@ -112,6 +135,33 @@
   for (long i = i0; i < n; i += stride) {
     float b = has_bias ? bias[i % D] : 0.f;
     dx[i] = dy[i] * gelu_df(x[i] + b);
+  }
+}
+
+__global__ void bias_residual_add_bf16(const unsigned short* __restrict__ y,
+                                       const unsigned short* __restrict__ bias,
+                                       const unsigned short* __restrict__ x,
+                                       unsigned short* __restrict__ out,
+                                       long n, int D) {
+  long i0 = ((long)blockIdx.x * BLOCK + threadIdx.x) * 8;
+  long stride = (long)gridDim.x * BLOCK * 8;
+  for (long i = i0; i < n; i += stride) {
+    bf16x8 yv = *(const bf16x8*)(y + i);
+    bf16x8 xv = *(const bf16x8*)(x + i);
+    bf16x8 bv;
+    if (bias != nullptr) bv = *(const bf16x8*)(bias + (int)(i % D));
+    const unsigned short* ys = (const unsigned short*)&yv;
+    const unsigned short* xs = (const unsigned short*)&xv;
+    const unsigned short* bs = (const unsigned short*)&bv;
+    bf16x8 ov;
+    unsigned short* os = (unsigned short*)&ov;
+#pragma unroll
+    for (int j = 0; j < 8; ++j) {
+      float t = bf2f(ys[j]);
+      if (bias != nullptr) t = bf2f(f2bf(t + bf2f(bs[j])));
+      os[j] = f2bf(bf2f(xs[j]) + t);
+    }
+    *(bf16x8*)(out + i) = ov;
   }
 }
 
@@ -320,11 +370,13 @@
   auto stream = at::cuda::getCurrentHIPStream();
   if (x.scalar_type() == torch::kBFloat16) {
     TORCH_CHECK(!has_bias || (D % 8 == 0), "D must be multiple of 8");
-    hipLaunchKernelGGL(bias_gelu_bwd_bf16, dim3(ew_grid(n, 8)), dim3(BLOCK), 0,
-                       stream, (const unsigned short*)dy.data_ptr(),
+    hipLaunchKernelGGL(bias_gelu_bwd_bf16<false>, dim3(ew_grid(n, 8)),
+                       dim3(BLOCK), 0, stream,
+                       (const unsigned short*)dy.data_ptr(),
                        (const unsigned short*)x.data_ptr(),
                        (const unsigned short*)bias.data_ptr(),
-                       (unsigned short*)dx.data_ptr(), n, D, has_bias);
+                       (unsigned short*)dx.data_ptr(), (float*)nullptr, n, D,
+                       has_bias);
   } else {
     hipLaunchKernelGGL(bias_gelu_bwd_f32, dim3(ew_grid(n)), dim3(BLOCK), 0,
                        stream, dy.data_ptr<float>(), x.data_ptr<float>(),
@@ -333,6 +385,81 @@
   }
   HIP_CHECK_LAST();
   return dx;
+}
+
+namespace {
+long colsum_grid(long n, int D) {
+  long a = D, b = (long)BLOCK * 8;
+  while (b) { long t = a % b; a = b; b = t; }
+  const long q = D / a;
+  if (q > 2048) return 0;
+  const long want = ew_grid(n, 8);
+  return want < q ? q : want / q * q;
+}
+}
+
+std::vector<torch::Tensor> bias_gelu_bwd_colsum(torch::Tensor dy,
+                                                torch::Tensor x,
+                                                torch::Tensor bias) {
+  const char* fn = "bias_gelu_bwd_colsum";
+  TORCH_CHECK(x.is_cuda() && x.scalar_type() == torch::kBFloat16 &&
+                  x.is_contiguous() && x.dim() >= 1 && aligned16(x),
+              fn, ": x must be a contiguous, 16-byte aligned bf16 device "
+              "tensor");
+  const int D = x.size(-1);
+  TORCH_CHECK(D > 0 && D % 8 == 0, fn, ": D must be a multiple of 8, got ", D);
+  check_bf16_rows(fn, "dy", dy, x);
+  check_bf16_vec(fn, "bias", bias, x, D);
+  const long rows = x.numel() / D;
+  auto dx = torch::empty_like(x);
+  auto opts = x.options().dtype(torch::kFloat);
+  if (rows == 0) return {dx, torch::zeros({1, (long)D}, opts)};
+  const long grid = colsum_grid(x.numel(), D);
+  TORCH_CHECK(grid > 0, fn, ": no grid of at most 2048 blocks has a stride "
+              "that is a multiple of D = ", D);
+  auto partial = torch::empty({grid * BLOCK * 8 / D, (long)D}, opts);
+  auto stream = at::cuda::getCurrentHIPStream();
+  hipLaunchKernelGGL(bias_gelu_bwd_bf16<true>, dim3((unsigned)grid),
+                     dim3(BLOCK), 0, stream,
+                     (const unsigned short*)dy.data_ptr(),
+                     (const unsigned short*)x.data_ptr(),
+                     (const unsigned short*)bias.data_ptr(),
+                     (unsigned short*)dx.data_ptr(),
+                     partial.data_ptr<float>(), x.numel(), D, 1);
+  HIP_CHECK_LAST();
+  return {dx, partial};
+}
+
+bool bias_gelu_bwd_colsum_ok(int64_t D) {
+  return D > 0 && D % 8 == 0 && colsum_grid(1, (int)D) > 0;
+}
+
+torch::Tensor bias_residual_add(torch::Tensor y,
+                                c10::optional<torch::Tensor> bias,
+                                torch::Tensor x_res) {
+  const char* fn = "bias_residual_add";
+  TORCH_CHECK(x_res.is_cuda() && x_res.scalar_type() == torch::kBFloat16 &&
+                  x_res.is_contiguous() && x_res.dim() >= 1 &&
+                  aligned16(x_res),
+              fn, ": x_res must be a contiguous, 16-byte aligned bf16 device "
+              "tensor");
+  const int D = x_res.size(-1);
+  TORCH_CHECK(D > 0 && D % 8 == 0, fn, ": D must be a multiple of 8, got ", D);
+  check_bf16_rows(fn, "y", y, x_res);
+  const bool has_bias = bias.has_value() && bias->defined();
+  if (has_bias) check_bf16_vec(fn, "bias", *bias, x_res, D);
+  auto out = torch::empty_like(x_res);
+  const long n = x_res.numel();
+  if (n == 0) return out;
+  auto stream = at::cuda::getCurrentHIPStream();
+  hipLaunchKernelGGL(bias_residual_add_bf16, dim3(ew_grid(n, 8)), dim3(BLOCK),
+                     0, stream, (const unsigned short*)y.data_ptr(),
+                     has_bias ? (const unsigned short*)bias->data_ptr()
+                              : (const unsigned short*)nullptr,
+                     (const unsigned short*)x_res.data_ptr(),
+                     (unsigned short*)out.data_ptr(), n, D);
+  HIP_CHECK_LAST();
+  return out;
 }
 
 void adamw_step(torch::Tensor p, torch::Tensor g, torch::Tensor m,
diff --git a/torchdistpackage_amd/ops/csrc/fused_checks.h b/torchdistpackage_amd/ops/csrc/fused_checks.h
--- /dev/null
+++ b/torchdistpackage_amd/ops/csrc/fused_checks.h
@@ -0,0 +1,30 @@
+#pragma once
+
+#include <torch/extension.h>
+
+inline bool aligned16(const torch::Tensor& t) {
+  return ((unsigned long long)t.data_ptr() & 15) == 0;
+}
+
+inline void check_bf16_rows(const char* fn, const char* name,
+                            const torch::Tensor& t,
+                            const torch::Tensor& like) {
+  TORCH_CHECK(t.is_cuda() && t.device() == like.device() &&
+                  t.scalar_type() == torch::kBFloat16 && t.is_contiguous() &&
+                  t.sizes() == like.sizes() && aligned16(t),
+              fn, ": ", name,
+              " must be a contiguous, 16-byte aligned bf16 tensor of shape ",
+              like.sizes(), " on ", like.device(), ", got ", t.scalar_type(),
+              " ", t.sizes(), " on ", t.device());
+}
+
+inline void check_bf16_vec(const char* fn, const char* name,
+                           const torch::Tensor& t, const torch::Tensor& like,
+                           int D) {
+  TORCH_CHECK(t.is_cuda() && t.device() == like.device() &&
+                  t.scalar_type() == torch::kBFloat16 && t.is_contiguous() &&
+                  t.numel() == D && aligned16(t),
+              fn, ": ", name,
+              " must be a contiguous, 16-byte aligned bf16 vector of ", D,
+              " elements on ", like.device());
+}
diff --git a/torchdistpackage_amd/ops/csrc/norms.hip b/torchdistpackage_amd/ops/csrc/norms.hip
--- a/torchdistpackage_amd/ops/csrc/norms.hip
+++ b/torchdistpackage_amd/ops/csrc/norms.hip
@@ -2,6 +2,7 @@
 #include <torch/extension.h>
 #include <ATen/hip/HIPContext.h>
 #include "common.h"
+#include "fused_checks.h"
 
 namespace {
 
@@ -308,11 +309,14 @@
   }
 }
 
-template <int NC>
+template <int NC, bool RES>
 __global__ void __launch_bounds__(BLOCK)
 layernorm_fwd_bf16v8(const unsigned short* __restrict__ x,
+                     const unsigned short* __restrict__ lin,
+                     const unsigned short* __restrict__ lbias,
                      const unsigned short* __restrict__ w,
                      const unsigned short* __restrict__ b,
+                     unsigned short* __restrict__ xnew,
                      unsigned short* __restrict__ y,
                      float* __restrict__ mean,
                      float* __restrict__ rstd,
@@ -329,6 +333,19 @@
       int i = threadIdx.x * 8 + c * BLOCK * 8;
       if (i < D) {
         xv[c] = load8f(xr + i);
+        if constexpr (RES) {
+          f8 t = load8f(lin + (long)row * D + i);
+          if (lbias != nullptr) {
+            f8 lb = load8f(lbias + i);
+#pragma unroll
+            for (int j = 0; j < 8; ++j)
+              t.v[j] = bf2f(f2bf(t.v[j] + lb.v[j]));
+          }
+#pragma unroll
+          for (int j = 0; j < 8; ++j)
+            xv[c].v[j] = bf2f(f2bf(xv[c].v[j] + t.v[j]));
+          store8f(xnew + (long)row * D + i, xv[c]);
+        }
 #pragma unroll
         for (int j = 0; j < 8; ++j) {
           s += xv[c].v[j];
@@ -515,22 +532,33 @@
   }
 }
 
-template <int NC>
-__global__ void layernorm_bwd_bf16_reg(const unsigned short* __restrict__ dy,
-                                       const unsigned short* __restrict__ x,
-                                       const unsigned short* __restrict__ w,
-                                       const float* __restrict__ mean,
-                                       const float* __restrict__ rstd,
-                                       unsigned short* __restrict__ dx,
-                                       float* __restrict__ dw_partial,
-                                       float* __restrict__ db_partial,
-                                       int rows, int D) {
+template <int NC, bool RES, bool COLSUM>
+__global__ void __launch_bounds__(BLOCK)
+layernorm_bwd_bf16_reg(const unsigned short* __restrict__ dy,
+                       const unsigned short* __restrict__ x,
+                       const unsigned short* __restrict__ w,
+                       const float* __restrict__ mean,
+                       const float* __restrict__ rstd,
+                       const unsigned short* __restrict__ g_res,
+                       unsigned short* __restrict__ dx,
+                       float* __restrict__ dw_partial,
+                       float* __restrict__ db_partial,
+                       float* __restrict__ dc_partial,
+                       int rows, int D) {
+  static_assert(RES || !COLSUM, "COLSUM sums the residual-added grad");
   __shared__ float scratch[2 * BLOCK / WAVE];
   float acc_dw[NC][8], acc_db[NC][8];
+  float acc_dc[COLSUM ? NC : 1][8];
 #pragma unroll
   for (int c = 0; c < NC; ++c)
 #pragma unroll
     for (int j = 0; j < 8; ++j) { acc_dw[c][j] = 0.f; acc_db[c][j] = 0.f; }
+  if constexpr (COLSUM) {
+#pragma unroll
+    for (int c = 0; c < NC; ++c)
+#pragma unroll
+      for (int j = 0; j < 8; ++j) acc_dc[c][j] = 0.f;
+  }
 
   for (int row = blockIdx.x; row < rows; row += gridDim.x) {
     const unsigned short* dyr = dy + (long)row * D;
@@ -584,6 +612,14 @@
           acc_dw[c][j] += dyv[c].v[j] * xhat;
           acc_db[c][j] += dyv[c].v[j];
         }
+        if constexpr (RES) {
+          f8 gr = load8f(g_res + (long)row * D + i);
+#pragma unroll
+          for (int j = 0; j < 8; ++j) {
+            out.v[j] = bf2f(f2bf(out.v[j])) + gr.v[j];
+            if constexpr (COLSUM) acc_dc[c][j] += bf2f(f2bf(out.v[j]));
+          }
+        }
         store8f(dxr + i, out);
       }
     }
@@ -600,6 +636,16 @@
         dwp[i + j] = acc_dw[c][j];
         dbp[i + j] = acc_db[c][j];
       }
+  }
+  if constexpr (COLSUM) {
+    float* dcp = dc_partial + (long)blockIdx.x * D;
+#pragma unroll
+    for (int c = 0; c < NC; ++c) {
+      int i = threadIdx.x * 8 + c * BLOCK * 8;
+      if (i < D)
+#pragma unroll
+        for (int j = 0; j < 8; ++j) dcp[i + j] = acc_dc[c][j];
+    }
   }
 }
 
@@ -716,10 +762,13 @@
   if (x.scalar_type() == torch::kBFloat16 && D % 8 == 0) {
     const int nc = (D + BLOCK * 8 - 1) / (BLOCK * 8);
 #define LN_FWD(NC)                                                           \
-    hipLaunchKernelGGL(layernorm_fwd_bf16v8<NC>, grid, block, 0, stream,     \
-                       (const unsigned short*)x.data_ptr(),                  \
+    hipLaunchKernelGGL((layernorm_fwd_bf16v8<NC, false>), grid, block, 0,    \
+                       stream, (const unsigned short*)x.data_ptr(),          \
+                       (const unsigned short*)nullptr,                       \
+                       (const unsigned short*)nullptr,                       \
                        (const unsigned short*)w.data_ptr(),                  \
                        (const unsigned short*)b.data_ptr(),                  \
+                       (unsigned short*)nullptr,                             \
                        (unsigned short*)y.data_ptr(),                        \
                        mean.data_ptr<float>(), rstd.data_ptr<float>(),       \
                        (int)rows, D, (float)eps)
@@ -761,14 +810,17 @@
                                    x.options().dtype(torch::kFloat));
     int nc = (D + BLOCK * 8 - 1) / (BLOCK * 8);
 #define LN_REG(NC)                                                           \
-    hipLaunchKernelGGL(layernorm_bwd_bf16_reg<NC>, grid, block, 0, stream,   \
+    hipLaunchKernelGGL((layernorm_bwd_bf16_reg<NC, false, false>), grid,     \
+                       block, 0, stream,                                     \
                        (const unsigned short*)dy.data_ptr(),                 \
                        (const unsigned short*)x.data_ptr(),                  \
                        (const unsigned short*)w.data_ptr(),                  \
                        mean.data_ptr<float>(), rstd.data_ptr<float>(),       \
+                       (const unsigned short*)nullptr,                       \
                        (unsigned short*)dx.data_ptr(),                       \
                        dw_partial.data_ptr<float>(),                         \
-                       db_partial.data_ptr<float>(), (int)rows, D)
+                       db_partial.data_ptr<float>(), (float*)nullptr,        \
+                       (int)rows, D)
     if (nc == 1) LN_REG(1); else if (nc == 2) LN_REG(2);
     else if (nc == 3) LN_REG(3); else LN_REG(4);
 #undef LN_REG
@@ -816,3 +868,108 @@
   HIP_CHECK_LAST();
   return {dx, dw.to(w.scalar_type()), db.to(w.scalar_type())};
 }
+
+
+namespace {
+
+constexpr int FUSED_LN_MAX_D = 4 * BLOCK * 8;
+
+int fused_ln_width(const char* fn, const torch::Tensor& x) {
+  TORCH_CHECK(x.is_cuda() && x.scalar_type() == torch::kBFloat16 &&
+                  x.is_contiguous() && x.dim() >= 1 && aligned16(x),
+              fn, ": needs a contiguous, 16-byte aligned bf16 device tensor");
+  const int D = x.size(-1);
+  TORCH_CHECK(D > 0 && D % 8 == 0 && D <= FUSED_LN_MAX_D, fn,
+              ": last dim must be a multiple of 8 up to ", FUSED_LN_MAX_D,
+              ", got ", D);
+  return D;
+}
+
+}
+
+int64_t fused_ln_max_d() { return FUSED_LN_MAX_D; }
+
+std::vector<torch::Tensor> bias_residual_layernorm_fwd(
+    torch::Tensor y, c10::optional<torch::Tensor> bias, torch::Tensor x_res,
+    torch::Tensor ln_w, torch::Tensor ln_b, double eps) {
+  const char* fn = "bias_residual_layernorm_fwd";
+  const int D = fused_ln_width(fn, x_res);
+  check_bf16_rows(fn, "y", y, x_res);
+  check_bf16_vec(fn, "ln_w", ln_w, x_res, D);
+  check_bf16_vec(fn, "ln_b", ln_b, x_res, D);
+  const bool has_bias = bias.has_value() && bias->defined();
+  if (has_bias) check_bf16_vec(fn, "bias", *bias, x_res, D);
+  const long rows = x_res.numel() / D;
+  auto x_new = torch::empty_like(x_res);
+  auto h = torch::empty_like(x_res);
+  auto mean = torch::empty({rows}, x_res.options().dtype(torch::kFloat));
+  auto rstd = torch::empty({rows}, x_res.options().dtype(torch::kFloat));
+  if (rows == 0) return {x_new, h, mean, rstd};
+  auto stream = at::cuda::getCurrentHIPStream();
+  dim3 grid(pick_grid(rows)), block(BLOCK);
+  const int nc = (D + BLOCK * 8 - 1) / (BLOCK * 8);
+#define LN_FWD_RES(NC)                                                       \
+  hipLaunchKernelGGL((layernorm_fwd_bf16v8<NC, true>), grid, block, 0,       \
+                     stream, (const unsigned short*)x_res.data_ptr(),        \
+                     (const unsigned short*)y.data_ptr(),                    \
+                     has_bias ? (const unsigned short*)bias->data_ptr()      \
+                              : (const unsigned short*)nullptr,              \
+                     (const unsigned short*)ln_w.data_ptr(),                 \
+                     (const unsigned short*)ln_b.data_ptr(),                 \
+                     (unsigned short*)x_new.data_ptr(),                      \
+                     (unsigned short*)h.data_ptr(),                          \
+                     mean.data_ptr<float>(), rstd.data_ptr<float>(),         \
+                     (int)rows, D, (float)eps)
+  if (nc == 1) LN_FWD_RES(1); else if (nc == 2) LN_FWD_RES(2);
+  else LN_FWD_RES(4);
+#undef LN_FWD_RES
+  HIP_CHECK_LAST();
+  return {x_new, h, mean, rstd};
+}
+
+std::vector<torch::Tensor> layernorm_bwd_residual(
+    torch::Tensor dh, torch::Tensor x, torch::Tensor w, torch::Tensor mean,
+    torch::Tensor rstd, torch::Tensor g_res, bool want_colsum) {
+  const char* fn = "layernorm_bwd_residual";
+  const int D = fused_ln_width(fn, x);
+  check_bf16_rows(fn, "dh", dh, x);
+  check_bf16_rows(fn, "g_res", g_res, x);
+  check_bf16_vec(fn, "w", w, x, D);
+  const long rows = x.numel() / D;
+  TORCH_CHECK(mean.is_cuda() && rstd.is_cuda() &&
+                  mean.scalar_type() == torch::kFloat &&
+                  rstd.scalar_type() == torch::kFloat &&
+                  mean.is_contiguous() && rstd.is_contiguous() &&
+                  mean.numel() == rows && rstd.numel() == rows,
+              fn, ": mean and rstd must be contiguous fp32 with one value "
+              "per row (", rows, ")");
+  auto g = torch::empty_like(x);
+  dim3 grid(pick_grid(rows)), block(BLOCK);
+  const long np = want_colsum ? 3 : 2;
+  auto opts = x.options().dtype(torch::kFloat);
+  if (rows == 0) return {g, torch::zeros({np, 1, (long)D}, opts)};
+  auto partial = torch::empty({np, (long)grid.x, (long)D}, opts);
+  float* pp = partial.data_ptr<float>();
+  const long pstride = (long)grid.x * D;
+  auto stream = at::cuda::getCurrentHIPStream();
+  const int nc = (D + BLOCK * 8 - 1) / (BLOCK * 8);
+#define LN_REG_RES(NC, CS)                                                   \
+  hipLaunchKernelGGL((layernorm_bwd_bf16_reg<NC, true, CS>), grid, block, 0, \
+                     stream, (const unsigned short*)dh.data_ptr(),           \
+                     (const unsigned short*)x.data_ptr(),                    \
+                     (const unsigned short*)w.data_ptr(),                    \
+                     mean.data_ptr<float>(), rstd.data_ptr<float>(),         \
+                     (const unsigned short*)g_res.data_ptr(),                \
+                     (unsigned short*)g.data_ptr(), pp, pp + pstride,        \
+                     CS ? pp + 2 * pstride : (float*)nullptr, (int)rows, D)
+#define LN_REG_RES_NC(NC)                                                    \
+  do {                                                                       \
+    if (want_colsum) LN_REG_RES(NC, true); else LN_REG_RES(NC, false);       \
+  } while (0)
+  if (nc == 1) LN_REG_RES_NC(1); else if (nc == 2) LN_REG_RES_NC(2);
+  else if (nc == 3) LN_REG_RES_NC(3); else LN_REG_RES_NC(4);
+#undef LN_REG_RES_NC
+#undef LN_REG_RES
+  HIP_CHECK_LAST();
+  return {g, partial};
+}
diff --git a/torchdistpackage_amd/parallel/tensor/attn.py b/torchdistpackage_amd/parallel/tensor/attn.py
--- a/torchdistpackage_amd/parallel/tensor/attn.py
+++ b/torchdistpackage_amd/parallel/tensor/attn.py
@@ -65,7 +65,7 @@
                                       sequence_parallel=sequence_parallel,
                                       device=device, dtype=dtype)
 
-    def forward(self, x):
+    def forward(self, x, skip_bias: bool = False):
         if is_sequence_parallel(x):
             x = gather_from_sequence_parallel_region(x)
         else:
@@ -73,7 +73,7 @@
         from ...ops.gemm import linear as fast_linear
         qkv = fast_linear(x, self.qkv.weight, self.qkv.bias)
         o = _sdpa(qkv, self.n_head_local, self.causal)
-        return self.proj(o)
+        return self.proj(o, skip_bias=skip_bias)
 
     @torch.no_grad()
     def decode_step(self, x: torch.Tensor, k_cache: torch.Tensor,
diff --git a/torchdistpackage_amd/parallel/tensor/mlp.py b/torchdistpackage_amd/parallel/tensor/mlp.py
--- a/torchdistpackage_amd/parallel/tensor/mlp.py
+++ b/torchdistpackage_amd/parallel/tensor/mlp.py
@@ -38,7 +38,7 @@
                                      sequence_parallel=sequence_parallel,
                                      device=device, dtype=dtype)
 
-    def forward(self, x):
+    def forward(self, x, skip_bias: bool = False):
         from .tp_utils import copy_to_tp_region, \
             gather_from_sequence_parallel_region
         if is_sequence_parallel(x):
@@ -50,7 +50,7 @@
         h = bias_gelu(h, self.fc1.bias)
         if self.dropout > 0 and self.training:
             h = F.dropout(h, p=self.dropout)
-        return self.fc2(h)
+        return self.fc2(h, skip_bias=skip_bias)
 
     @torch.no_grad()
     def init_weight_from_full(self, full_mlp: Mlp):
diff --git a/torchdistpackage_amd/parallel/tensor/tp_utils.py b/torchdistpackage_amd/parallel/tensor/tp_utils.py
--- a/torchdistpackage_amd/parallel/tensor/tp_utils.py
+++ b/torchdistpackage_amd/parallel/tensor/tp_utils.py
@@ -291,13 +291,13 @@
         super().__init__(in_features // tp, out_features, bias=bias,
                          device=device, dtype=dtype)
 
-    def forward(self, x):
+    def forward(self, x, skip_bias: bool = False):
         out = fast_linear(x, self.weight)
         if self.sequence_parallel and get_tp_size() > 1:
             out = reduce_scatter_to_sequence_parallel_region(out)
         else:
             out = reduce_from_tp_region(out)
-        if self.bias is not None:
+        if self.bias is not None and not skip_bias:
             out = out + self.bias
         return out
 
diff --git a/torchdistpackage_amd/parallel/tensor/transformer.py b/torchdistpackage_amd/parallel/tensor/transformer.py
--- a/torchdistpackage_amd/parallel/tensor/transformer.py
+++ b/torchdistpackage_amd/parallel/tensor/transformer.py
@@ -4,6 +4,7 @@
 import torch
 import torch.nn as nn
 
+from ... import ops
 from ...ops import LayerNorm
 from .attn import Attention, TpAttention
 from .mlp import Mlp, TpMlp
@@ -52,6 +53,9 @@
             mark_sequence_parallel_params(self.ln_2)
 
     def forward(self, x):
+        if ops.fused_residual_enabled() and \
+                not (self.dropout > 0 and self.training):
+            return self._forward_fused(x)
         if self.sequence_parallel:
             x = maybe_split_into_sequence_parallel(x)
         h = self.ln_1(x)
@@ -66,6 +70,24 @@
         if self.sequence_parallel:
             set_sequence_parallel_attr(h)
         x = x + self.mlp(h)
+        if self.sequence_parallel:
+            set_sequence_parallel_attr(x)
+        return x
+
+    def _forward_fused(self, x):
+        if self.sequence_parallel:
+            x = maybe_split_into_sequence_parallel(x)
+        ln_1, ln_2 = self.ln_1, self.ln_2
+        x, h = ops.layer_norm_fork(x, ln_1.weight, ln_1.bias, ln_1.eps)
+        if self.sequence_parallel:
+            set_sequence_parallel_attr(h)
+        a = self.attn(h, skip_bias=True)
+        x, h = ops.bias_residual_layer_norm(a, self.attn.proj.bias, x,
+                                            ln_2.weight, ln_2.bias, ln_2.eps)
+        if self.sequence_parallel:
+            set_sequence_parallel_attr(h)
+        m = self.mlp(h, skip_bias=True)
+        x = ops.bias_residual_add(m, self.mlp.fc2.bias, x)
         if self.sequence_parallel:
             set_sequence_parallel_attr(x)
         return x
```

Result: faster. 110,700 tokens/s, median of 6 (+2.8%).
